# CortexFoundation/tachikoma

Hardware: AMD Instinct MI355X
Metric: ResNet-50 int8 op-traces/sec at 1/2/4/8 GPU; bit-exact vs CPU (higher is better)
Workload: dtype int8; 1 GPU; resnet50 int8 224x224, 64 samples per GPU (BASELINE config 4 shard), full per-op trace to pinned host memory; model=resnet50, global_batch=64, samples_per_gpu=64, parallelism=batch-shard x1, sink=memory

## Files before the change

### include/tachikoma.h

```cpp
#ifndef TACHIKOMA_H_
#define TACHIKOMA_H_

#include <stdint.h>
#include <stddef.h>

#ifdef __cplusplus
extern "C" {
#endif

#pragma GCC visibility push(default)

#define TK_ABI_VERSION 1

typedef enum {
  TK_OK = 0,
  TK_ERR_INVALID_ARG = -1,
  TK_ERR_UNSUPPORTED = -2,
  TK_ERR_SHAPE = -3,
  TK_ERR_DTYPE = -4,
  TK_ERR_HIP = -5,
  TK_ERR_IO = -6,
  TK_ERR_FORMAT = -7,
} tk_status;

// ... 78 lines not shown
  int32_t has_clip;
  int64_t clip_min, clip_max;
  int32_t has_add;
  int32_t block_is_rhs;
  const tk_tensor* residual;
  tk_qnn_add_attrs add;
  int32_t algo;
} tk_block_attrs;

int tk_conv2d_block_algos(const tk_tensor* data, const tk_tensor* weight, const tk_block_attrs* attrs,
                          int32_t* algos, int max_algos);
int tk_conv2d_block_algo_info(const tk_tensor* data, const tk_tensor* weight, const tk_block_attrs* attrs, int algo,
                              char* buf, int len);

typedef struct {
  tk_qnn_add_attrs add;
  int32_t has_clip;
  int64_t clip_min, clip_max;
} tk_add_block_attrs;

typedef struct {
  int32_t pool_size[2];
  int32_t strides[2];
  int32_t padding[4];
  int32_t dilation[2];
  int32_t count_include_pad;
} tk_pool2d_attrs;


int64_t tk_conv2d_packed_weight_bytes(const tk_tensor* weight, int groups);
int tk_conv2d_pack_weight(const tk_tensor* weight, int groups, void* packed, int32_t* weight_sums,
                          void* stream);
int64_t tk_conv2d_shadow_bytes(const tk_tensor* data);
int tk_conv2d_make_shadow(const tk_tensor* data, void* shadow, void* stream);
int tk_conv2d_make_shadow_batch(const tk_tensor* const* data, void* const* shadow, int n, void* stream);
int64_t tk_conv2d_scratch_bytes(const tk_tensor* data, const tk_tensor* weight, const tk_conv2d_attrs* attrs,
                                int block);
int tk_qnn_conv2d_prepared(const tk_tensor* data, const void* shadow, const tk_tensor* weight,
                           const void* packed, const int32_t* weight_sums, tk_tensor* out,
                           const tk_conv2d_attrs* attrs, void* scratch, void* stream);
int64_t tk_qnn_conv2d_workspace_bytes(const tk_tensor* data, const tk_tensor* weight,
                                      const tk_conv2d_attrs* attrs);
int tk_qnn_conv2d(const tk_tensor* data, const tk_tensor* weight, tk_tensor* out,
                  const tk_conv2d_attrs* attrs, void* workspace, void* stream);

int tk_qnn_conv2d_block(const tk_tensor* data, const void* shadow, const tk_tensor* weight, const void* packed,
                        const int32_t* weight_sums, const tk_tensor* bias, tk_tensor* const* outs, int n_outs,
                        const tk_block_attrs* attrs, void* scratch, void* shadow_out, void* stream);

int64_t tk_qnn_dense_workspace_bytes(const tk_tensor* data, const tk_tensor* weight);
int tk_qnn_dense(const tk_tensor* data, const tk_tensor* weight, tk_tensor* out,
                 const tk_dense_attrs* attrs, void* workspace, void* stream);
int tk_qnn_dense_block(const tk_tensor* data, const tk_tensor* weight, const tk_tensor* bias, tk_tensor* const* outs,
                       int n_outs, const tk_block_attrs* attrs, void* workspace, void* stream);

int tk_requantize(const tk_tensor* data, tk_tensor* out, const tk_requantize_attrs* attrs, void* stream);
int tk_qnn_add(const tk_tensor* lhs, const tk_tensor* rhs, tk_tensor* out, const tk_qnn_add_attrs* attrs,
               void* stream);
int tk_qnn_add_block(const tk_tensor* lhs, const tk_tensor* rhs, tk_tensor* const* outs, int n_outs,
                     const tk_add_block_attrs* attrs, void* shadow_out, void* stream);

int tk_bias_add(const tk_tensor* data, const tk_tensor* bias, tk_tensor* out, int axis, void* stream);
int tk_clip(const tk_tensor* data, tk_tensor* out, int64_t a_min, int64_t a_max, void* stream);
int tk_cast(const tk_tensor* data, tk_tensor* out, void* stream);
int tk_max_pool2d(const tk_tensor* data, tk_tensor* out, const tk_pool2d_attrs* attrs, void* stream);
int tk_max_pool2d_shadow(const tk_tensor* data, const void* data_shadow, tk_tensor* out,
                         const tk_pool2d_attrs* attrs, void* out_shadow, void* stream);
int tk_avg_pool2d(const tk_tensor* data, tk_tensor* out, const tk_pool2d_attrs* attrs, void* stream);
int tk_global_avg_pool2d(const tk_tensor* data, tk_tensor* out, void* stream);
int tk_copy(const tk_tensor* data, tk_tensor* out, void* stream);
typedef struct {
  int64_t before[6], after[6];
  int64_t value_i;
  double value_f;
} tk_pad_attrs;
int tk_pad(const tk_tensor* data, tk_tensor* out, const tk_pad_attrs* attrs, void* stream);

typedef struct {
  int32_t axis;
  int32_t n_scales;
  float clip_lo, clip_hi, act_scl, sum_scl, dst_zp;
  const float* bias;
  const float* o_scl;
} tk_postops_attrs;
int tk_tachikoma_postops(const tk_tensor* acc, const tk_tensor* sum_src, tk_tensor* out,
                         const tk_postops_attrs* attrs, void* stream);

enum {
  TK_EW_ADD = 0,
  TK_EW_MULTIPLY = 1,
  TK_EW_LEFT_SHIFT = 2,
  TK_EW_RIGHT_SHIFT = 3,
  TK_EW_ROUND = 4,
  TK_EW_CLIP = 5,
  TK_EW_RELU = 6,
  TK_EW_FIXED_POINT_MULTIPLY = 7,
};
typedef struct {
  int32_t op;
  int32_t rhs_kind;
  double scalar_f;
  int64_t scalar_i;
  double lo, hi;
  int32_t multiplier, shift;
} tk_ewise_attrs;
int tk_ewise(const tk_tensor* x, const tk_tensor* rhs, tk_tensor* out, const tk_ewise_attrs* attrs, void* stream);
int tk_conv2d_f32(const tk_tensor* data, const tk_tensor* weight, tk_tensor* out, const tk_conv2d_attrs* attrs,
                  void* stream);
int tk_dense_f32(const tk_tensor* data, const tk_tensor* weight, tk_tensor* out, void* stream);
int tk_find_scale_by_kl(const int32_t* hist, const float* edges, int num_bins, int num_quantized_bins,
                        float* threshold);


typedef struct {
  int32_t axis;
  float scale;
  const float* scales;
  int32_t zero_point;
  const int32_t* zero_points;
} tk_qparams_attrs;
int tk_qnn_quantize(const tk_tensor* data, tk_tensor* out, const tk_qparams_attrs* attrs, void* stream);
int tk_qnn_dequantize(const tk_tensor* data, tk_tensor* out, const tk_qparams_attrs* attrs, void* stream);

enum { TK_QB_ADD = 0, TK_QB_SUBTRACT = 1, TK_QB_MUL = 2 };
typedef struct {
  int32_t op;
  tk_requantize_attrs lhs, rhs;
  int32_t lhs_upcast, rhs_upcast;
  tk_requantize_attrs out;
  int32_t output_zero_point;
} tk_qnn_binary_attrs;
int tk_qnn_binary(const tk_tensor* lhs, const tk_tensor* rhs, tk_tensor* out, const tk_qnn_binary_attrs* attrs,
                  void* stream);

#define TK_CONCAT_MAX 8
typedef struct {
  int32_t axis;
  int32_t n;
  int32_t requant[TK_CONCAT_MAX];
  tk_requantize_attrs rq[TK_CONCAT_MAX];
} tk_concat_attrs;
int tk_qnn_concatenate(const tk_tensor* const* inputs, int n, tk_tensor* out, const tk_concat_attrs* attrs,
                       void* stream);

typedef struct {
  int32_t ndim;
  int32_t perm[6];
} tk_transpose_attrs;
int tk_transpose(const tk_tensor* data, tk_tensor* out, const tk_transpose_attrs* attrs, void* stream);

typedef struct {
  tk_requantize_attrs rq;
  int32_t upcast;
  int32_t input_zero_point;
  int32_t output_zero_point;
  int32_t alpha_multiplier, alpha_shift;
  int32_t zp_multiplier, zp_shift;
} tk_leaky_relu_attrs;
int tk_qnn_leaky_relu(const tk_tensor* data, tk_tensor* out, const tk_leaky_relu_attrs* attrs, void* stream);

int tk_qnn_lookup(const tk_tensor* data, tk_tensor* out, const void* table, void* stream);

int64_t tk_qnn_batch_matmul_workspace_bytes(const tk_tensor* x, const tk_tensor* y);
int tk_qnn_batch_matmul(const tk_tensor* x, const tk_tensor* y, tk_tensor* out, const tk_dense_attrs* attrs,
                        void* workspace, void* stream);

typedef struct {
  int32_t strides[2];
  int32_t padding[4];
  int32_t output_padding[2];
  int32_t groups;
  int32_t input_zero_point;
  int32_t kernel_zero_point;
  const int32_t* kernel_zero_points;
} tk_conv2d_transpose_attrs;
int tk_qnn_conv2d_transpose(const tk_tensor* data, const tk_tensor* weight, tk_tensor* out,
                            const tk_conv2d_transpose_attrs* attrs, void* stream);

typedef struct {
  int32_t axis;
  int32_t n_scales, n_zero_points;
  const int32_t* dtype_code;
  const float* scales;
  const int32_t* zero_points;
} tk_simq_attrs;
int tk_qnn_simulated_quantize(const tk_tensor* data, tk_tensor* out, const tk_simq_attrs* attrs, void* stream);
int tk_qnn_simulated_dequantize(const tk_tensor* data, tk_tensor* out, const tk_simq_attrs* attrs, void* stream);

typedef struct {
  int32_t bits;
  int32_t rounding;
  int32_t axis;
  int32_t scaled;
  double multiplier;
  const double* multipliers;
  int32_t input_zero_point;
  const int32_t* input_zero_points;
  int32_t output_zero_point;
} tk_requantize_fp_attrs;
int tk_requantize_fp(const tk_tensor* data, tk_tensor* out, const tk_requantize_fp_attrs* attrs, void* stream);

typedef struct {
  int32_t op;
  tk_requantize_fp_attrs lhs, rhs;
  int32_t lhs_upcast, rhs_upcast;
  tk_requantize_fp_attrs out;
  int32_t output_zero_point;
} tk_qnn_binary_fp_attrs;
int tk_qnn_binary_fp(const tk_tensor* lhs, const tk_tensor* rhs, tk_tensor* out, const tk_qnn_binary_fp_attrs* attrs,
                     void* stream);


enum {
  TK_NODE_CONV2D = 1,
  TK_NODE_DENSE = 2,
  TK_NODE_REQUANTIZE = 3,
  TK_NODE_BIAS_ADD = 4,
  TK_NODE_CLIP = 5,
  TK_NODE_CAST = 6,
  TK_NODE_QNN_ADD = 7,
  TK_NODE_MAX_POOL2D = 8,
  TK_NODE_AVG_POOL2D = 9,
  TK_NODE_GLOBAL_AVG_POOL2D = 10,
  TK_NODE_COPY = 11,
  TK_NODE_SHADOW = 12,
  TK_NODE_CONV_BLOCK = 13,
  TK_NODE_DENSE_BLOCK = 14,
  TK_NODE_ADD_BLOCK = 15,
  TK_NODE_POSTOPS = 16,
  TK_NODE_EWISE = 17,
  TK_NODE_CONV2D_F32 = 18,
  TK_NODE_DENSE_F32 = 19,
  TK_NODE_PAD = 20,
  TK_NODE_QUANTIZE = 21,
  TK_NODE_DEQUANTIZE = 22,
  TK_NODE_QNN_BINARY = 23,
  TK_NODE_CONCAT = 24,
  TK_NODE_TRANSPOSE = 25,
  TK_NODE_LEAKY_RELU = 26,
  TK_NODE_LOOKUP = 27,
  TK_NODE_BATCH_MATMUL = 28,
  TK_NODE_CONV2D_TRANSPOSE = 29,
  TK_NODE_SIM_QUANTIZE = 30,
  TK_NODE_SIM_DEQUANTIZE = 31,
  TK_NODE_REQUANTIZE_FP = 32,
  TK_NODE_QNN_BINARY_FP = 33,
};

#define TK_MAX_NODE_INPUTS 8
#define TK_MAX_NODE_OUTPUTS 6

typedef struct {
  int32_t kind;
  int32_t n_inputs;
  const tk_tensor* inputs[TK_MAX_NODE_INPUTS];
  int32_t n_outputs;
  tk_tensor* outputs[TK_MAX_NODE_OUTPUTS];
  void* ext[5];
  union {
    tk_conv2d_attrs conv2d;
    tk_dense_attrs dense;
    tk_requantize_attrs requantize;
    tk_qnn_add_attrs qnn_add;
    tk_pool2d_attrs pool2d;
    tk_block_attrs block;
    tk_add_block_attrs add_block;
    tk_postops_attrs postops;
    tk_ewise_attrs ewise;
    tk_pad_attrs pad;
    tk_qparams_attrs qparams;
    tk_qnn_binary_attrs qnn_binary;
    tk_concat_attrs concat;
    tk_transpose_attrs transpose;
    tk_leaky_relu_attrs leaky_relu;
    tk_conv2d_transpose_attrs conv2d_transpose;
    tk_simq_attrs simq;
    tk_requantize_fp_attrs requantize_fp;
    tk_qnn_binary_fp_attrs qnn_binary_fp;
    struct { int64_t a_min, a_max; } clip;
    struct { int32_t axis; } bias_add;
  } attrs;
} tk_node;

typedef struct tk_module tk_module;

int tk_module_create(const tk_node* nodes, int n_nodes, tk_module** out);
int tk_module_destroy(tk_module* mod);
int tk_module_num_nodes(const tk_module* mod);
int tk_module_run(tk_module* mod, void* stream, void* capture_stream, void* const* host_dst);
int tk_module_run_graph(tk_module* mod, void* stream, void* capture_stream, void* const* host_dst);
int tk_module_set_graph_copies(tk_module* mod, int copy_kernels);
int tk_module_set_trace_chunks(tk_module* mod, int chunks);
int tk_module_set_copy_trace(tk_module* mod, int enable);
int tk_module_copy_trace(tk_module* mod, double* out, int max_chunks);
int tk_module_set_trace_wire(tk_module* mod, int enable);
int tk_module_wire_stats(tk_module* mod, double* out, int max_chunks);

typedef struct {
  int64_t offset;
  int64_t n_elems;
  int32_t diff;
  int32_t kind;
} tk_wire_record;
int64_t tk_wire_bound(const tk_wire_record* recs, int n_recs);
int64_t tk_wire_encode_host(const tk_wire_record* recs, int n_recs, const void* image, int64_t image_bytes,
                            void* wire, int64_t wire_cap);
int tk_wire_decode(const tk_wire_record* recs, int n_recs, const void* wire, int64_t wire_bytes, void* image,
                   int64_t image_bytes, int threads);
int tk_wire_encode_device(const tk_wire_record* recs, int n_recs, const void* const* src, void* wire,
                          int64_t wire_cap, void* stream);
int64_t tk_wire_pack_device(const tk_wire_record* recs, int n_recs, const void* const* src, void* wire,
                            int64_t wire_cap, void* stream);
int tk_wire_pack_tile(void);
int tk_wire_threads(void);

typedef struct {
  uint64_t mismatches;
  uint64_t first;
} tk_wire_mismatch;
enum { TK_WIRE_UNPACK_STORE = 0, TK_WIRE_UNPACK_COMPARE = 1 };
int tk_wire_check(const tk_wire_record* recs, int n_recs, const void* wire, int64_t wire_bytes);
int tk_wire_unpack_device(const tk_wire_record* recs, int n_recs, const void* wire, int64_t wire_bytes,
                          void* const* dst, int mode, tk_wire_mismatch* report, void* stream);
int tk_compare_device(const void* expected, const void* got, int64_t n_elems, int elem_bytes,
                      tk_wire_mismatch* report, void* stream);
int tk_compare_device_batch(const void* const* expected, const void* const* got, const int64_t* n_elems,
                            const int32_t* elem_bytes, int n, tk_wire_mismatch* report, void* stream);

typedef struct {
  int32_t node;
  int32_t output;
} tk_chain_op;
int tk_chain_check_tile(void);
int tk_module_chain_ops(tk_module* mod, tk_chain_op* ops, int capacity);
int tk_module_check_chains(tk_module* mod, tk_wire_mismatch* report, int capacity, void* stream);
int tk_check_chain(int kind, const tk_tensor* const* records, int n_records, const tk_tensor* bias, const void* attrs,
                   tk_wire_mismatch* report, int capacity, void* stream);

typedef struct {
  uint64_t count;
  int64_t sum;
  int32_t min, max;
  uint64_t bits[33];
  uint64_t values[256];
} tk_record_stats;
typedef struct tk_stats_plan tk_stats_plan;
int tk_record_stats_tile(void);
int tk_record_stats_span(void);
int tk_record_stats_size(void);
int tk_stats_plan_create(const void* const* src, const int64_t* n_elems, const int32_t* kinds, int n,
                         tk_stats_plan** out);
int tk_stats_plan_destroy(tk_stats_plan* plan);
int tk_record_stats_reset(tk_record_stats* stats_dev, int n, void* stream);
int tk_stats_plan_run(tk_stats_plan* plan, tk_record_stats* stats_dev, void* stream);
int tk_record_stats_batch(const void* const* src, const int64_t* n_elems, const int32_t* kinds, int n,
                          tk_record_stats* out_host, void* stream);

int tk_module_wait_capture(tk_module* mod, void* stream);
int tk_module_run_range(tk_module* mod, int begin, int end, void* stream);
int tk_module_run_order(tk_module* mod, const int32_t* order, int n, void* stream);
int tk_module_run_profiled(tk_module* mod, void* stream, float* node_ms);
int tk_module_set_profiling(tk_module* mod, int enable);
int tk_module_node_times(tk_module* mod, float* node_ms);
int tk_module_tune(tk_module* mod, void* stream, int max_candidates, int reps, int32_t* algo_out, float* us_out);
int tk_module_set_node_algo(tk_module* mod, int node, int algo);


typedef struct {
  const char* name;
  int32_t ndim;
  const int64_t* shape;
  tk_dtype dtype;
} tk_array_meta;

int64_t tk_ndlist_layout(const tk_array_meta* arrays, int n, int64_t* data_offsets);
int tk_ndlist_write_headers(const tk_array_meta* arrays, int n, void* blob, int64_t blob_size);
int tk_ndlist_parse(const void* blob, int64_t blob_size, int cap, tk_array_meta* arrays,
                    int64_t* data_offsets, int64_t* shapes_storage, int shapes_cap, int* n_out);

#define TK_TRACE_MAGIC 0x0045434152544B54ULL
#define TK_TRACE_VERSION 1
#define TK_TRACE_VERSION_PACKED 2
#define TK_TRACE_ALIGN 4096
typedef struct {
  uint64_t magic, version, json_len, params_off, params_size, records_off, records_size;
} tk_trace_header;

int64_t tk_trace_layout(const char* json, const tk_array_meta* params, int n_params,
                        const tk_array_meta* records, int n_records, int64_t* param_offsets,
                        int64_t* record_offsets);
int tk_trace_write_headers(const char* json, const tk_array_meta* params, int n_params,
                           const tk_array_meta* records, int n_records, void* image, int64_t image_size);
int tk_write_file(const char* path, const void* image, int64_t size);

int tk_digest_bytes(const void* data, int64_t nbytes, uint64_t* out_device, void* stream);

#pragma GCC visibility pop

#ifdef __cplusplus
}
#endif
#endif
```

### tachikoma_amd/_lib.py

```python
from __future__ import annotations

import ctypes
import os
from typing import Optional

import numpy as np

HERE = os.path.dirname(os.path.abspath(__file__))
LIB_PATH = os.path.join(HERE, "libtachikoma.so")


class TachikomaError(RuntimeError):
    """Raised when a C-ABI call fails (carries ``tk_last_error()``)."""



class tk_device(ctypes.Structure):
    _fields_ = [("device_type", ctypes.c_int32), ("device_id", ctypes.c_int32)]


class tk_dtype(ctypes.Structure):
    _fields_ = [("code", ctypes.c_uint8), ("bits", ctypes.c_uint8), ("lanes", ctypes.c_uint16)]


class tk_tensor(ctypes.Structure):
    _fields_ = [
        ("data", ctypes.c_void_p),
        ("device", tk_device),
        ("ndim", ctypes.c_int32),
        ("dtype", tk_dtype),
        ("shape", ctypes.POINTER(ctypes.c_int64)),
        ("strides", ctypes.POINTER(ctypes.c_int64)),
        ("byte_offset", ctypes.c_uint64),
    ]


class tk_requantize_attrs(ctypes.Structure):
    _fields_ = [
        ("mode", ctypes.c_int32),
        ("axis", ctypes.c_int32),
        ("multiplier", ctypes.c_int32),
        ("shift", ctypes.c_int32),
        ("multipliers", ctypes.c_void_p),
        ("shifts", ctypes.c_void_p),
        ("input_zero_point", ctypes.c_int32),
        ("input_zero_points", ctypes.c_void_p),
        ("output_zero_point", ctypes.c_int32),
    ]


class tk_conv2d_attrs(ctypes.Structure):
    _fields_ = [
        ("strides", ctypes.c_int32 * 2),
        ("padding", ctypes.c_int32 * 4),
        ("dilation", ctypes.c_int32 * 2),
        ("groups", ctypes.c_int32),
        ("input_zero_point", ctypes.c_int32),
        ("kernel_zero_point", ctypes.c_int32),
        ("kernel_zero_points", ctypes.c_void_p),
    ]


class tk_dense_attrs(ctypes.Structure):
    _fields_ = [
        ("input_zero_point", ctypes.c_int32),
        ("kernel_zero_point", ctypes.c_int32),
        ("kernel_zero_points", ctypes.c_void_p),
    ]


class tk_qnn_add_attrs(ctypes.Structure):
    _fields_ = [
        ("lhs", tk_requantize_attrs),
        ("rhs", tk_requantize_attrs),
        ("output_zero_point", ctypes.c_int32),
        ("lhs_upcast", ctypes.c_int32),
        ("rhs_upcast", ctypes.c_int32),
    ]


class tk_block_attrs(ctypes.Structure):
    _fields_ = [
        ("conv", tk_conv2d_attrs),
        ("dense", tk_dense_attrs),
        ("requantize", tk_requantize_attrs),
        ("has_clip", ctypes.c_int32),
        ("clip_min", ctypes.c_int64),
        ("clip_max", ctypes.c_int64),
        ("has_add", ctypes.c_int32),
        ("block_is_rhs", ctypes.c_int32),
        ("residual", ctypes.POINTER(tk_tensor)),
        ("add", tk_qnn_add_attrs),
        ("algo", ctypes.c_int32),
    ]


class tk_add_block_attrs(ctypes.Structure):
    _fields_ = [
        ("add", tk_qnn_add_attrs),
        ("has_clip", ctypes.c_int32),
        ("clip_min", ctypes.c_int64),
        ("clip_max", ctypes.c_int64),
    ]


class tk_postops_attrs(ctypes.Structure):
    _fields_ = [
        ("axis", ctypes.c_int32),
        ("n_scales", ctypes.c_int32),
        ("clip_lo", ctypes.c_float),
        ("clip_hi", ctypes.c_float),
        ("act_scl", ctypes.c_float),
        ("sum_scl", ctypes.c_float),
        ("dst_zp", ctypes.c_float),
        ("bias", ctypes.c_void_p),
        ("o_scl", ctypes.c_void_p),
    ]


class tk_ewise_attrs(ctypes.Structure):
    _fields_ = [
        ("op", ctypes.c_int32),
        ("rhs_kind", ctypes.c_int32),
        ("scalar_f", ctypes.c_double),
        ("scalar_i", ctypes.c_int64),
        ("lo", ctypes.c_double),
        ("hi", ctypes.c_double),
        ("multiplier", ctypes.c_int32),
        ("shift", ctypes.c_int32),
    ]


TK_EW = {"add": 0, "multiply": 1, "left_shift": 2, "right_shift": 3, "round": 4, "clip": 5, "relu": 6,
         "fixed_point_multiply": 7}


class tk_pad_attrs(ctypes.Structure):
    _fields_ = [
        ("before", ctypes.c_int64 * 6),
        ("after", ctypes.c_int64 * 6),
        ("value_i", ctypes.c_int64),
        ("value_f", ctypes.c_double),
    ]


class tk_pool2d_attrs(ctypes.Structure):
    _fields_ = [
        ("pool_size", ctypes.c_int32 * 2),
        ("strides", ctypes.c_int32 * 2),
        ("padding", ctypes.c_int32 * 4),
        ("dilation", ctypes.c_int32 * 2),
        ("count_include_pad", ctypes.c_int32),
    ]


class tk_qparams_attrs(ctypes.Structure):
    _fields_ = [
        ("axis", ctypes.c_int32),
        ("scale", ctypes.c_float),
        ("scales", ctypes.c_void_p),
        ("zero_point", ctypes.c_int32),
        ("zero_points", ctypes.c_void_p),
    ]


class tk_qnn_binary_attrs(ctypes.Structure):
    _fields_ = [
        ("op", ctypes.c_int32),
        ("lhs", tk_requantize_attrs),
        ("rhs", tk_requantize_attrs),
        ("lhs_upcast", ctypes.c_int32),
        ("rhs_upcast", ctypes.c_int32),
        ("out", tk_requantize_attrs),
        ("output_zero_point", ctypes.c_int32),
    ]


TK_QB = {"qnn.add": 0, "qnn.subtract": 1, "qnn.mul": 2}
CONCAT_MAX = 8


class tk_concat_attrs(ctypes.Structure):
    _fields_ = [
        ("axis", ctypes.c_int32),
        ("n", ctypes.c_int32),
        ("requant", ctypes.c_int32 * CONCAT_MAX),
        ("rq", tk_requantize_attrs * CONCAT_MAX),
    ]


class tk_transpose_attrs(ctypes.Structure):
    _fields_ = [("ndim", ctypes.c_int32), ("perm", ctypes.c_int32 * 6)]


class tk_leaky_relu_attrs(ctypes.Structure):
    _fields_ = [
        ("rq", tk_requantize_attrs),
        ("upcast", ctypes.c_int32),
        ("input_zero_point", ctypes.c_int32),
        ("output_zero_point", ctypes.c_int32),
        ("alpha_multiplier", ctypes.c_int32),
        ("alpha_shift", ctypes.c_int32),
        ("zp_multiplier", ctypes.c_int32),
        ("zp_shift", ctypes.c_int32),
    ]


class tk_conv2d_transpose_attrs(ctypes.Structure):
    _fields_ = [
        ("strides", ctypes.c_int32 * 2),
        ("padding", ctypes.c_int32 * 4),
        ("output_padding", ctypes.c_int32 * 2),
        ("groups", ctypes.c_int32),
        ("input_zero_point", ctypes.c_int32),
        ("kernel_zero_point", ctypes.c_int32),
        ("kernel_zero_points", ctypes.c_void_p),
    ]


class tk_simq_attrs(ctypes.Structure):
    _fields_ = [
        ("axis", ctypes.c_int32),
        ("n_scales", ctypes.c_int32),
        ("n_zero_points", ctypes.c_int32),
        ("dtype_code", ctypes.c_void_p),
        ("scales", ctypes.c_void_p),
        ("zero_points", ctypes.c_void_p),
    ]


class tk_requantize_fp_attrs(ctypes.Structure):
    _fields_ = [
        ("bits", ctypes.c_int32),
        ("rounding", ctypes.c_int32),
        ("axis", ctypes.c_int32),
        ("scaled", ctypes.c_int32),
        ("multiplier", ctypes.c_double),
        ("multipliers", ctypes.c_void_p),
        ("input_zero_point", ctypes.c_int32),
        ("input_zero_points", ctypes.c_void_p),
        ("output_zero_point", ctypes.c_int32),
    ]


class tk_qnn_binary_fp_attrs(ctypes.Structure):
    _fields_ = [
        ("op", ctypes.c_int32),
        ("lhs", tk_requantize_fp_attrs),
        ("rhs", tk_requantize_fp_attrs),
        ("lhs_upcast", ctypes.c_int32),
        ("rhs_upcast", ctypes.c_int32),
        ("out", tk_requantize_fp_attrs),
        ("output_zero_point", ctypes.c_int32),
    ]


class _clip(ctypes.Structure):
    _fields_ = [("a_min", ctypes.c_int64), ("a_max", ctypes.c_int64)]


class _bias_add(ctypes.Structure):
    _fields_ = [("axis", ctypes.c_int32)]


class tk_node_attrs(ctypes.Union):
    _fields_ = [
        ("conv2d", tk_conv2d_attrs),
        ("dense", tk_dense_attrs),
        ("requantize", tk_requantize_attrs),
        ("qnn_add", tk_qnn_add_attrs),
        ("pool2d", tk_pool2d_attrs),
        ("block", tk_block_attrs),
        ("add_block", tk_add_block_attrs),
        ("postops", tk_postops_attrs),
        ("ewise", tk_ewise_attrs),
        ("pad", tk_pad_attrs),
        ("qparams", tk_qparams_attrs),
        ("qnn_binary", tk_qnn_binary_attrs),
        ("concat", tk_concat_attrs),
        ("transpose", tk_transpose_attrs),
        ("leaky_relu", tk_leaky_relu_attrs),
        ("conv2d_transpose", tk_conv2d_transpose_attrs),
        ("simq", tk_simq_attrs),
        ("requantize_fp", tk_requantize_fp_attrs),
        ("qnn_binary_fp", tk_qnn_binary_fp_attrs),
        ("clip", _clip),
        ("bias_add", _bias_add),
    ]


class tk_node(ctypes.Structure):
    _fields_ = [
        ("kind", ctypes.c_int32),
        ("n_inputs", ctypes.c_int32),
        ("inputs", ctypes.POINTER(tk_tensor) * 8),
        ("n_outputs", ctypes.c_int32),
        ("outputs", ctypes.POINTER(tk_tensor) * 6),
        ("ext", ctypes.c_void_p * 5),
        ("attrs", tk_node_attrs),
    ]


class tk_wire_record(ctypes.Structure):
    _fields_ = [
        ("offset", ctypes.c_int64),
        ("n_elems", ctypes.c_int64),
        ("diff", ctypes.c_int32),
        ("kind", ctypes.c_int32),
    ]


class tk_wire_mismatch(ctypes.Structure):
    _fields_ = [
        ("mismatches", ctypes.c_uint64),
        ("first", ctypes.c_uint64),
    ]


class tk_chain_op(ctypes.Structure):
    _fields_ = [
        ("node", ctypes.c_int32),
        ("output", ctypes.c_int32),
    ]


class tk_record_stats(ctypes.Structure):
    _fields_ = [
        ("count", ctypes.c_uint64),
        ("sum", ctypes.c_int64),
        ("min", ctypes.c_int32),
        ("max", ctypes.c_int32),
        ("bits", ctypes.c_uint64 * 33),
        ("values", ctypes.c_uint64 * 256),
    ]


TK_WIRE_UNPACK_STORE, TK_WIRE_UNPACK_COMPARE = 0, 1
NO_MISMATCH = 0xFFFFFFFFFFFFFFFF


class tk_array_meta(ctypes.Structure):
    _fields_ = [
        ("name", ctypes.c_char_p),
        ("ndim", ctypes.c_int32),
        ("shape", ctypes.POINTER(ctypes.c_int64)),
        ("dtype", tk_dtype),
    ]


TK_DL_INT, TK_DL_UINT, TK_DL_FLOAT = 0, 1, 2
TK_DEV_CPU, TK_DEV_ROCM = 1, 10
TK_ROUND_UPWARD, TK_ROUND_TONEAREST = 0, 1
(TK_RQ_IDENTITY, TK_RQ_TENSOR_POW2, TK_RQ_TENSOR_UPWARD, TK_RQ_TENSOR_TONEAREST, TK_RQ_AXIS_UPWARD,
 TK_RQ_AXIS_TONEAREST) = range(6)
NODE_KINDS = {
    "qnn.conv2d": 1, "qnn.dense": 2, "qnn.requantize": 3, "nn.bias_add": 4, "clip": 5, "cast": 6,
    "qnn.add": 7, "nn.max_pool2d": 8, "nn.avg_pool2d": 9, "nn.global_avg_pool2d": 10, "copy": 11, "shadow": 12,
    "conv_block": 13, "dense_block": 14, "add_block": 15, "postops": 16,
    "ewise": 17, "conv2d_f32": 18, "dense_f32": 19, "nn.pad": 20,
    "qnn.quantize": 21, "qnn.dequantize": 22, "qnn_binary": 23, "qnn.concatenate": 24, "transpose": 25,
    "qnn.leaky_relu": 26, "lookup": 27, "qnn.batch_matmul": 28, "qnn.conv2d_transpose": 29,
    "qnn.simulated_quantize": 30, "qnn.simulated_dequantize": 31, "requantize_fp": 32, "qnn_binary_fp": 33,
}
MAX_NODE_INPUTS = 8
MAX_NODE_OUTPUTS = 6

_VP, _I32, _I64, _F32, _F64 = ctypes.c_void_p, ctypes.c_int32, ctypes.c_int64, ctypes.c_float, ctypes.c_double
_PT = ctypes.POINTER(tk_tensor)
SIGNATURES = {
    "tk_last_error": (ctypes.c_char_p, []),
    "tk_abi_version": (ctypes.c_int, []),
    "tk_build_arch": (ctypes.c_char_p, []),
    "tk_build_info": (ctypes.c_char_p, []),
    "tk_fixed_point_multiplier_shift": (ctypes.c_int, [_F64, ctypes.POINTER(_I32), ctypes.POINTER(_I32)]),
    "tk_requantize_prepare": (ctypes.c_int, [ctypes.POINTER(_F32), ctypes.c_int, _F32, ctypes.c_int,
                                             ctypes.POINTER(_I32), ctypes.POINTER(_I32), ctypes.POINTER(ctypes.c_int)]),
    "tk_conv2d_packed_weight_bytes": (_I64, [_PT, ctypes.c_int]),
    "tk_conv2d_pack_weight": (ctypes.c_int, [_PT, ctypes.c_int, _VP, _VP, _VP]),
    "tk_conv2d_shadow_bytes": (_I64, [_PT]),
    "tk_conv2d_scratch_bytes": (_I64, [_PT, _PT, ctypes.POINTER(tk_conv2d_attrs), ctypes.c_int]),
    "tk_conv2d_make_shadow": (ctypes.c_int, [_PT, _VP, _VP]),
    "tk_conv2d_make_shadow_batch": (ctypes.c_int, [ctypes.POINTER(_PT), ctypes.POINTER(_VP), ctypes.c_int, _VP]),
    "tk_qnn_conv2d_prepared": (ctypes.c_int, [_PT, _VP, _PT, _VP, _VP, _PT, ctypes.POINTER(tk_conv2d_attrs), _VP,
                                              _VP]),
    "tk_qnn_conv2d_workspace_bytes": (_I64, [_PT, _PT, ctypes.POINTER(tk_conv2d_attrs)]),
    "tk_qnn_conv2d": (ctypes.c_int, [_PT, _PT, _PT, ctypes.POINTER(tk_conv2d_attrs), _VP, _VP]),
    "tk_qnn_dense_workspace_bytes": (_I64, [_PT, _PT]),
    "tk_qnn_dense": (ctypes.c_int, [_PT, _PT, _PT, ctypes.POINTER(tk_dense_attrs), _VP, _VP]),
    "tk_qnn_conv2d_block": (ctypes.c_int, [_PT, _VP, _PT, _VP, _VP, _PT, ctypes.POINTER(_PT), ctypes.c_int,
                                           ctypes.POINTER(tk_block_attrs), _VP, _VP, _VP]),
    "tk_qnn_dense_block": (ctypes.c_int, [_PT, _PT, _PT, ctypes.POINTER(_PT), ctypes.c_int,
                                          ctypes.POINTER(tk_block_attrs), _VP, _VP]),
    "tk_requantize": (ctypes.c_int, [_PT, _PT, ctypes.POINTER(tk_requantize_attrs), _VP]),
    "tk_qnn_add": (ctypes.c_int, [_PT, _PT, _PT, ctypes.POINTER(tk_qnn_add_attrs), _VP]),
    "tk_qnn_add_block": (ctypes.c_int, [_PT, _PT, ctypes.POINTER(_PT), ctypes.c_int,
                                        ctypes.POINTER(tk_add_block_attrs), _VP, _VP]),
    "tk_bias_add": (ctypes.c_int, [_PT, _PT, _PT, ctypes.c_int, _VP]),
    "tk_clip": (ctypes.c_int, [_PT, _PT, _I64, _I64, _VP]),
    "tk_cast": (ctypes.c_int, [_PT, _PT, _VP]),
    "tk_max_pool2d": (ctypes.c_int, [_PT, _PT, ctypes.POINTER(tk_pool2d_attrs), _VP]),
    "tk_max_pool2d_shadow": (ctypes.c_int, [_PT, _VP, _PT, ctypes.POINTER(tk_pool2d_attrs), _VP, _VP]),
    "tk_avg_pool2d": (ctypes.c_int, [_PT, _PT, ctypes.POINTER(tk_pool2d_attrs), _VP]),
    "tk_global_avg_pool2d": (ctypes.c_int, [_PT, _PT, _VP]),
    "tk_copy": (ctypes.c_int, [_PT, _PT, _VP]),
    "tk_pad": (ctypes.c_int, [_PT, _PT, ctypes.POINTER(tk_pad_attrs), _VP]),
    "tk_tachikoma_postops": (ctypes.c_int, [_PT, _PT, _PT, ctypes.POINTER(tk_postops_attrs), _VP]),
    "tk_ewise": (ctypes.c_int, [_PT, _PT, _PT, ctypes.POINTER(tk_ewise_attrs), _VP]),
    "tk_conv2d_f32": (ctypes.c_int, [_PT, _PT, _PT, ctypes.POINTER(tk_conv2d_attrs), _VP]),
    "tk_dense_f32": (ctypes.c_int, [_PT, _PT, _PT, _VP]),
    "tk_qnn_quantize": (ctypes.c_int, [_PT, _PT, ctypes.POINTER(tk_qparams_attrs), _VP]),
    "tk_qnn_dequantize": (ctypes.c_int, [_PT, _PT, ctypes.POINTER(tk_qparams_attrs), _VP]),
    "tk_qnn_binary": (ctypes.c_int, [_PT, _PT, _PT, ctypes.POINTER(tk_qnn_binary_attrs), _VP]),
    "tk_qnn_concatenate": (ctypes.c_int, [ctypes.POINTER(_PT), ctypes.c_int, _PT, ctypes.POINTER(tk_concat_attrs),
                                          _VP]),
    "tk_transpose": (ctypes.c_int, [_PT, _PT, ctypes.POINTER(tk_transpose_attrs), _VP]),
    "tk_qnn_leaky_relu": (ctypes.c_int, [_PT, _PT, ctypes.POINTER(tk_leaky_relu_attrs), _VP]),
    "tk_qnn_lookup": (ctypes.c_int, [_PT, _PT, _VP, _VP]),
    "tk_qnn_batch_matmul_workspace_bytes": (_I64, [_PT, _PT]),
    "tk_qnn_batch_matmul": (ctypes.c_int, [_PT, _PT, _PT, ctypes.POINTER(tk_dense_attrs), _VP, _VP]),
    "tk_qnn_conv2d_transpose": (ctypes.c_int, [_PT, _PT, _PT, ctypes.POINTER(tk_conv2d_transpose_attrs), _VP]),
    "tk_qnn_simulated_quantize": (ctypes.c_int, [_PT, _PT, ctypes.POINTER(tk_simq_attrs), _VP]),
    "tk_qnn_simulated_dequantize": (ctypes.c_int, [_PT, _PT, ctypes.POINTER(tk_simq_attrs), _VP]),
    "tk_requantize_fp": (ctypes.c_int, [_PT, _PT, ctypes.POINTER(tk_requantize_fp_attrs), _VP]),
    "tk_qnn_binary_fp": (ctypes.c_int, [_PT, _PT, _PT, ctypes.POINTER(tk_qnn_binary_fp_attrs), _VP]),
    "tk_find_scale_by_kl": (ctypes.c_int, [ctypes.POINTER(_I32), ctypes.POINTER(_F32), ctypes.c_int, ctypes.c_int,
                                           ctypes.POINTER(_F32)]),
    "tk_module_create": (ctypes.c_int, [ctypes.POINTER(tk_node), ctypes.c_int, ctypes.POINTER(_VP)]),
    "tk_module_destroy": (ctypes.c_int, [_VP]),
    "tk_module_num_nodes": (ctypes.c_int, [_VP]),
    "tk_module_run": (ctypes.c_int, [_VP, _VP, _VP, ctypes.POINTER(_VP)]),
    "tk_module_wait_capture": (ctypes.c_int, [_VP, _VP]),
    "tk_module_run_range": (ctypes.c_int, [_VP, ctypes.c_int, ctypes.c_int, _VP]),
    "tk_module_run_order": (ctypes.c_int, [_VP, ctypes.POINTER(ctypes.c_int32), ctypes.c_int, _VP]),
    "tk_module_run_profiled": (ctypes.c_int, [_VP, _VP, ctypes.POINTER(_F32)]),
    "tk_module_set_profiling": (ctypes.c_int, [_VP, ctypes.c_int]),
    "tk_module_node_times": (ctypes.c_int, [_VP, ctypes.POINTER(_F32)]),
    "tk_module_run_graph": (ctypes.c_int, [_VP, _VP, _VP, ctypes.POINTER(_VP)]),
    "tk_module_set_graph_copies": (ctypes.c_int, [_VP, ctypes.c_int]),
    "tk_module_set_trace_chunks": (ctypes.c_int, [_VP, ctypes.c_int]),
    "tk_module_set_copy_trace": (ctypes.c_int, [_VP, ctypes.c_int]),
    "tk_module_copy_trace": (ctypes.c_int, [_VP, ctypes.POINTER(_F64), ctypes.c_int]),
    "tk_module_set_trace_wire": (ctypes.c_int, [_VP, ctypes.c_int]),
    "tk_module_wire_stats": (ctypes.c_int, [_VP, ctypes.POINTER(_F64), ctypes.c_int]),
    "tk_wire_bound": (_I64, [ctypes.POINTER(tk_wire_record), ctypes.c_int]),
    "tk_wire_encode_host": (_I64, [ctypes.POINTER(tk_wire_record), ctypes.c_int, _VP, _I64, _VP, _I64]),
    "tk_wire_decode": (ctypes.c_int, [ctypes.POINTER(tk_wire_record), ctypes.c_int, _VP, _I64, _VP, _I64, ctypes.c_int]),
    "tk_wire_encode_device": (ctypes.c_int, [ctypes.POINTER(tk_wire_record), ctypes.c_int, ctypes.POINTER(_VP), _VP,
                                             _I64, _VP]),
    "tk_wire_pack_device": (_I64, [ctypes.POINTER(tk_wire_record), ctypes.c_int, ctypes.POINTER(_VP), _VP, _I64, _VP]),
    "tk_wire_pack_tile": (ctypes.c_int, []),
    "tk_wire_threads": (ctypes.c_int, []),
    "tk_wire_check": (ctypes.c_int, [ctypes.POINTER(tk_wire_record), ctypes.c_int, _VP, _I64]),
    "tk_wire_unpack_device": (ctypes.c_int, [ctypes.POINTER(tk_wire_record), ctypes.c_int, _VP, _I64,
                                             ctypes.POINTER(_VP), ctypes.c_int, ctypes.POINTER(tk_wire_mismatch), _VP]),
    "tk_compare_device": (ctypes.c_int, [_VP, _VP, _I64, ctypes.c_int, ctypes.POINTER(tk_wire_mismatch), _VP]),
    "tk_compare_device_batch": (ctypes.c_int, [ctypes.POINTER(_VP), ctypes.POINTER(_VP), ctypes.POINTER(_I64),
                                               ctypes.POINTER(ctypes.c_int32), ctypes.c_int,
                                               ctypes.POINTER(tk_wire_mismatch), _VP]),
    "tk_chain_check_tile": (ctypes.c_int, []),
    "tk_module_chain_ops": (ctypes.c_int, [_VP, ctypes.POINTER(tk_chain_op), ctypes.c_int]),
    "tk_module_check_chains": (ctypes.c_int, [_VP, ctypes.POINTER(tk_wire_mismatch), ctypes.c_int, _VP]),
    "tk_check_chain": (ctypes.c_int, [ctypes.c_int, ctypes.POINTER(ctypes.POINTER(tk_tensor)), ctypes.c_int,
                                      ctypes.POINTER(tk_tensor), _VP, ctypes.POINTER(tk_wire_mismatch), ctypes.c_int,
                                      _VP]),
    "tk_record_stats_tile": (ctypes.c_int, []),
    "tk_record_stats_span": (ctypes.c_int, []),
    "tk_record_stats_size": (ctypes.c_int, []),
    "tk_stats_plan_create": (ctypes.c_int, [ctypes.POINTER(_VP), ctypes.POINTER(_I64), ctypes.POINTER(ctypes.c_int32),
                                            ctypes.c_int, ctypes.POINTER(_VP)]),
    "tk_stats_plan_destroy": (ctypes.c_int, [_VP]),
    "tk_record_stats_reset": (ctypes.c_int, [_VP, ctypes.c_int, _VP]),
    "tk_stats_plan_run": (ctypes.c_int, [_VP, _VP, _VP]),
    "tk_record_stats_batch": (ctypes.c_int, [ctypes.POINTER(_VP), ctypes.POINTER(_I64), ctypes.POINTER(ctypes.c_int32),
                                             ctypes.c_int, _VP, _VP]),
    "tk_module_tune": (ctypes.c_int, [_VP, _VP, ctypes.c_int, ctypes.c_int, ctypes.POINTER(ctypes.c_int32),
                                      ctypes.POINTER(_F32)]),
    "tk_module_set_node_algo": (ctypes.c_int, [_VP, ctypes.c_int, ctypes.c_int]),
    "tk_conv2d_block_algos": (ctypes.c_int, [_PT, _PT, ctypes.POINTER(tk_block_attrs), ctypes.POINTER(ctypes.c_int32),
                                             ctypes.c_int]),
    "tk_conv2d_block_algo_info": (ctypes.c_int, [_PT, _PT, ctypes.POINTER(tk_block_attrs), ctypes.c_int,
                                                  ctypes.c_char_p, ctypes.c_int]),
    "tk_ndlist_layout": (_I64, [ctypes.POINTER(tk_array_meta), ctypes.c_int, ctypes.POINTER(_I64)]),
    "tk_ndlist_write_headers": (ctypes.c_int, [ctypes.POINTER(tk_array_meta), ctypes.c_int, _VP, _I64]),
    "tk_ndlist_parse": (ctypes.c_int, [_VP, _I64, ctypes.c_int, ctypes.POINTER(tk_array_meta), ctypes.POINTER(_I64),
                                       ctypes.POINTER(_I64), ctypes.c_int, ctypes.POINTER(ctypes.c_int)]),
    "tk_trace_layout": (_I64, [ctypes.c_char_p, ctypes.POINTER(tk_array_meta), ctypes.c_int,
                               ctypes.POINTER(tk_array_meta), ctypes.c_int, ctypes.POINTER(_I64),
                               ctypes.POINTER(_I64)]),
    "tk_trace_write_headers": (ctypes.c_int, [ctypes.c_char_p, ctypes.POINTER(tk_array_meta), ctypes.c_int,
                                              ctypes.POINTER(tk_array_meta), ctypes.c_int, _VP, _I64]),
    "tk_write_file": (ctypes.c_int, [ctypes.c_char_p, _VP, _I64]),
    "tk_digest_bytes": (ctypes.c_int, [_VP, _I64, _VP, _VP]),
}

_LIB: Optional[ctypes.CDLL] = None


def load(path: str = LIB_PATH) -> ctypes.CDLL:
    global _LIB
    if _LIB is not None:
        return _LIB
    override = os.environ.get("TK_LIB_PATH")
    path = override or path
    if not os.path.exists(path):
        raise TachikomaError(
            f"{path} not found: build it with `python tachikoma_amd/build.py` "
            "(the engine has no CPU fallback)")
    lib = ctypes.CDLL(path, mode=ctypes.RTLD_GLOBAL)
    for name, (res, args) in SIGNATURES.items():
        fn = getattr(lib, name)
        fn.restype = res
        fn.argtypes = args
    from .build import source_hash
    built = lib.tk_build_info().decode()
    try:
        want = source_hash()
    except OSError:
        want = None
    any_src = bool(override) and os.environ.get("TK_LIB_ANY_SOURCES") == "1"
    if want is not None and built.split("+")[0] != want and not any_src:
        raise TachikomaError(
            f"{path} was built from other sources (library {built}, tree {want}): rebuild it with "
            "`python tachikoma_amd/build.py`")
    if override:
        import sys
        sys.stderr.write(f"[tachikoma] TK_LIB_PATH: using {path} ({built})\n")
    _LIB = lib
    return lib


def build_info() -> str:
    return load().tk_build_info().decode()


def check(rc: int, what: str = "") -> None:
    if rc != 0:
        msg = load().tk_last_error().decode(errors="replace")
        raise TachikomaError(f"{what or 'tachikoma call'} failed ({rc}): {msg}")


_DT = {
    "int8": (TK_DL_INT, 8), "uint8": (TK_DL_UINT, 8), "int16": (TK_DL_INT, 16), "uint16": (TK_DL_UINT, 16),
    "int32": (TK_DL_INT, 32), "uint32": (TK_DL_UINT, 32), "int64": (TK_DL_INT, 64), "uint64": (TK_DL_UINT, 64),
    "float32": (TK_DL_FLOAT, 32), "float64": (TK_DL_FLOAT, 64),
}


def dtype_struct(dtype: str) -> tk_dtype:
    code, bits = _DT[str(np.dtype(dtype))]
    return tk_dtype(code, bits, 1)


def dtype_name(d: tk_dtype) -> str:
    for k, (c, b) in _DT.items():
        if c == d.code and b == d.bits:
            return k
    raise TachikomaError(f"unknown dtype code={d.code} bits={d.bits}")


class TensorRef:

    def __init__(self, data_ptr: int, shape, dtype: str, device_type: int = TK_DEV_ROCM, device_id: int = 0):
        self.shape_arr = (ctypes.c_int64 * max(1, len(shape)))(*[int(s) for s in shape])
        self.struct = tk_tensor()
        self.struct.data = ctypes.c_void_p(int(data_ptr))
        self.struct.device = tk_device(device_type, device_id)
        self.struct.ndim = len(shape)
        self.struct.dtype = dtype_struct(dtype)
        self.struct.shape = ctypes.cast(self.shape_arr, ctypes.POINTER(ctypes.c_int64))
        self.struct.strides = None
        self.struct.byte_offset = 0
        self.shape = tuple(int(s) for s in shape)
        self.dtype = str(np.dtype(dtype))

    @property
    def ptr(self):
        return ctypes.pointer(self.struct)

    @staticmethod
    def from_torch(t) -> "TensorRef":
        import torch
        assert t.is_contiguous(), "tensors must be compact"
        dev = TK_DEV_ROCM if t.is_cuda else TK_DEV_CPU
        return TensorRef(t.data_ptr(), tuple(t.shape), str(t.dtype).replace("torch.", ""), dev,
                         t.device.index or 0 if t.is_cuda else 0)


def stream_handle(stream=None) -> int:
    import torch
    s = stream if stream is not None else torch.cuda.current_stream()
    return int(s.cuda_stream)
```

### tachikoma_amd/csrc/tk_runtime.cc

```cpp
#include <algorithm>
#include <atomic>
#include <cstdlib>
#include <cstring>
#include <map>
#include <memory>
#include <mutex>
#include <string>
#include <vector>

#include "tk_chain.h"
#include "tk_common.h"
#include "tk_wire.h"

namespace tk {
int requantize_impl(const tk_tensor* x, tk_tensor* y, const tk_requantize_attrs* a, hipStream_t s);
int bias_add_impl(const tk_tensor* x, const tk_tensor* b, tk_tensor* y, int axis, hipStream_t s);
int clip_impl(const tk_tensor* x, tk_tensor* y, int64_t lo, int64_t hi, hipStream_t s);
int cast_impl(const tk_tensor* x, tk_tensor* y, hipStream_t s);
int qnn_add_impl(const tk_tensor* a, const tk_tensor* b, tk_tensor* y, const tk_qnn_add_attrs* at, hipStream_t s);
int add_block_impl(const tk_tensor* a, const tk_tensor* b, tk_tensor* const* outs, int n_outs,
                   const tk_add_block_attrs* at, void* shadow, hipStream_t s);
int max_pool_impl(const tk_tensor* x, tk_tensor* y, const tk_pool2d_attrs* a, hipStream_t s);
int max_pool_shadow_impl(const tk_tensor* x, const void* x_shadow, tk_tensor* y, const tk_pool2d_attrs* a,
                         void* y_shadow, hipStream_t s);
int avg_pool_impl(const tk_tensor* x, tk_tensor* y, const tk_pool2d_attrs* a, hipStream_t s);
int global_avg_pool_impl(const tk_tensor* x, tk_tensor* y, hipStream_t s);
int copy_impl(const tk_tensor* x, tk_tensor* y, hipStream_t s);
int pad_impl(const tk_tensor* x, tk_tensor* y, const tk_pad_attrs* a, hipStream_t s);
int postops_impl(const tk_tensor* acc, const tk_tensor* sum_src, tk_tensor* y, const tk_postops_attrs* a,
                 hipStream_t s);
int host_copy_impl(const void* const* src, void* const* dst, const int64_t* bytes, int n, hipStream_t s);
int pack_records_impl(const void* table, int nrec, int64_t blocks, void* mirror, hipStream_t s);
int wire_encode_impl(const WireSegDev* segs, int64_t n_seg, uint32_t* cursor, void* wire, int64_t wire_bytes,
                     hipStream_t s);
int ewise_impl(const tk_tensor* x, const tk_tensor* r, tk_tensor* y, const tk_ewise_attrs* a, hipStream_t s);
int conv2d_f32_impl(const tk_tensor* x, const tk_tensor* w, tk_tensor* y, const tk_conv2d_attrs* a, hipStream_t s);
int dense_f32_impl(const tk_tensor* x, const tk_tensor* w, tk_tensor* y, hipStream_t s);
int64_t conv_packed_weight_bytes(const tk_tensor* weight, int groups);
int conv_pack_weight(const tk_tensor* weight, int groups, void* packed, int32_t* sums, hipStream_t s);
int64_t conv_shadow_bytes(const tk_tensor* data);
int64_t conv_scratch_bytes(const tk_tensor* data, const tk_tensor* weight, const tk_conv2d_attrs* a, int block);
int make_shadow_impl(const tk_tensor* data, void* shadow, hipStream_t s);
int conv2d_prepared_impl(const tk_tensor* data, const void* shadow, const tk_tensor* weight, const void* packed,
                         const int32_t* sums, tk_tensor* out, const tk_conv2d_attrs* a, void* scratch, hipStream_t s);
int64_t conv2d_workspace_bytes(const tk_tensor* data, const tk_tensor* weight, const tk_conv2d_attrs* a);
int conv2d_impl(const tk_tensor* data, const tk_tensor* weight, tk_tensor* out, const tk_conv2d_attrs* a,
                void* workspace, hipStream_t s);
int64_t dense_workspace_bytes(const tk_tensor* data, const tk_tensor* weight);
int dense_impl(const tk_tensor* data, const tk_tensor* weight, tk_tensor* out, const tk_dense_attrs* a,
               void* workspace, hipStream_t s);
int conv2d_block_impl(const tk_tensor* data, const void* shadow, const tk_tensor* weight, const void* packed,
                      const int32_t* sums, const tk_tensor* bias, tk_tensor* const* outs, int n_outs,
                      const tk_block_attrs* attrs, void* scratch, void* shadow_out, hipStream_t s);
int dense_block_impl(const tk_tensor* data, const tk_tensor* weight, const tk_tensor* bias, tk_tensor* const* outs,
                     int n_outs, const tk_block_attrs* attrs, void* workspace, hipStream_t s);
int qnn_quantize_impl(const tk_tensor* x, tk_tensor* y, const tk_qparams_attrs* a, hipStream_t s);
int qnn_dequantize_impl(const tk_tensor* x, tk_tensor* y, const tk_qparams_attrs* a, hipStream_t s);
int qnn_binary_impl(const tk_tensor* a, const tk_tensor* b, tk_tensor* y, const tk_qnn_binary_attrs* at,
                    hipStream_t s);
int qnn_concatenate_impl(const tk_tensor* const* xs, int n_in, tk_tensor* y, const tk_concat_attrs* a,
                         hipStream_t s);
int transpose_impl(const tk_tensor* x, tk_tensor* y, const tk_transpose_attrs* a, hipStream_t s);
int conv2d_block_algos_impl(const tk_tensor* data, const tk_tensor* weight, const tk_block_attrs* attrs,
                            int32_t* algos, int max_algos);
int qnn_leaky_relu_impl(const tk_tensor* x, tk_tensor* y, const tk_leaky_relu_attrs* a, hipStream_t s);
int qnn_simulated_impl(bool quant, const tk_tensor* x, tk_tensor* y, const tk_simq_attrs* a, hipStream_t s);
int requantize_fp_impl(const tk_tensor* x, tk_tensor* y, const tk_requantize_fp_attrs* a, hipStream_t s);
int qnn_binary_fp_impl(const tk_tensor* a, const tk_tensor* b, tk_tensor* y, const tk_qnn_binary_fp_attrs* at,
                       hipStream_t s);
int qnn_lookup_impl(const tk_tensor* x, tk_tensor* y, const void* table, hipStream_t s);
int qnn_conv2d_transpose_impl(const tk_tensor* x, const tk_tensor* w, tk_tensor* y, const tk_conv2d_transpose_attrs* a,
                              hipStream_t s);

static bool bmm_check(const tk_tensor* x, const tk_tensor* y) {
  return x && y && compact(x) && compact(y) && x->ndim == 3 && y->ndim == 3 && x->shape[2] == y->shape[2] &&
         (x->shape[0] == y->shape[0] || x->shape[0] == 1 || y->shape[0] == 1);
}
struct View2 {
  int64_t shape[2];
  tk_tensor t;
  View2(const tk_tensor* src, int64_t b) {
    t = *src;
    shape[0] = src->shape[1];
    shape[1] = src->shape[2];
    t.ndim = 2;
    t.shape = shape;
    t.strides = nullptr;
    t.byte_offset = src->byte_offset + (uint64_t)(b * shape[0] * shape[1] * elem_bytes(src));
  }
};
int64_t batch_matmul_workspace_bytes(const tk_tensor* x, const tk_tensor* y) {
  if (!bmm_check(x, y)) {
    set_error("qnn.batch_matmul: x [B, M, K], y [B', N, K] with B == B' or one of them 1");
    return TK_ERR_INVALID_ARG;
  }
  View2 xv(x, 0), yv(y, 0);
  return dense_workspace_bytes(&xv.t, &yv.t);
}
int batch_matmul_impl(const tk_tensor* x, const tk_tensor* y, tk_tensor* out, const tk_dense_attrs* a, void* ws,
                      hipStream_t s) {
  TK_CHECK_ARG(bmm_check(x, y) && out && a, "qnn.batch_matmul: x [B, M, K], y [B', N, K] (B == B' or one is 1)");
  const int64_t B = std::max(x->shape[0], y->shape[0]);
  TK_CHECK_ARG(compact(out) && out->ndim == 3 && out->shape[0] == B && out->shape[1] == x->shape[1] &&
               out->shape[2] == y->shape[1] && is_int(out, 32), "qnn.batch_matmul: int32 [B, M, N] output");
  for (int64_t b = 0; b < B; ++b) {
    View2 xv(x, x->shape[0] == 1 ? 0 : b), yv(y, y->shape[0] == 1 ? 0 : b), ov(out, b);
    const int rc = dense_impl(&xv.t, &yv.t, &ov.t, a, ws, s);
    if (rc) return rc;
  }
  return TK_OK;
}
int conv2d_block_algo_info_impl(const tk_tensor* data, const tk_tensor* weight, const tk_block_attrs* attrs, int algo,
                                char* buf, int len);

constexpr int TK_OK_RUN = 1;

struct OwnedTensor {
  tk_tensor t{};
  std::vector<int64_t> shape;
  void assign(const tk_tensor* src) {
    t = *src;
    shape.assign(src->shape, src->shape + src->ndim);
    t.shape = shape.data();
    t.strides = nullptr;
  }
  OwnedTensor() = default;
  OwnedTensor(const OwnedTensor& o) { assign(&o.t); }
  OwnedTensor& operator=(const OwnedTensor& o) {
    assign(&o.t);
    return *this;
  }
};

struct Node {
  tk_node desc{};
  OwnedTensor in[TK_MAX_NODE_INPUTS];
  OwnedTensor out[TK_MAX_NODE_OUTPUTS];
  tk_tensor* outp[TK_MAX_NODE_OUTPUTS] = {};
};

static int run_node(Node& n, hipStream_t s) {
  const tk_node& d = n.desc;
  const tk_tensor* i0 = &n.in[0].t;
  const tk_tensor* i1 = &n.in[1].t;
  const tk_tensor* i2 = &n.in[2].t;
  tk_tensor* o = &n.out[0].t;
  switch (d.kind) {
    case TK_NODE_CONV_BLOCK: {
      tk_block_attrs at = d.attrs.block;
      if (at.has_add) at.residual = &n.in[3].t;
      return conv2d_block_impl(i0, d.ext[0], i1, d.ext[1], (const int32_t*)d.ext[2], i2, n.outp, d.n_outputs, &at,
                               d.ext[3], d.ext[4], s);
    }
    case TK_NODE_DENSE_BLOCK:
      return dense_block_impl(i0, i1, i2, n.outp, d.n_outputs, &d.attrs.block, d.ext[0], s);
    case TK_NODE_CONV2D:
      return conv2d_prepared_impl(i0, d.ext[0], i1, d.ext[1], (const int32_t*)d.ext[2], o, &d.attrs.conv2d, d.ext[3], s);
    case TK_NODE_DENSE:
      return dense_impl(i0, i1, o, &d.attrs.dense, d.ext[0], s);
    case TK_NODE_REQUANTIZE:
      return requantize_impl(i0, o, &d.attrs.requantize, s);
    case TK_NODE_BIAS_ADD:
      return bias_add_impl(i0, i1, o, d.attrs.bias_add.axis, s);
    case TK_NODE_CLIP:
      return clip_impl(i0, o, d.attrs.clip.a_min, d.attrs.clip.a_max, s);
    case TK_NODE_CAST:
      return cast_impl(i0, o, s);
    case TK_NODE_QNN_ADD:
      return qnn_add_impl(i0, i1, o, &d.attrs.qnn_add, s);
    case TK_NODE_ADD_BLOCK:
      return add_block_impl(i0, i1, n.outp, d.n_outputs, &d.attrs.add_block, d.ext[4], s);
    case TK_NODE_MAX_POOL2D:
      if (d.ext[0]) return max_pool_shadow_impl(i0, d.ext[0], o, &d.attrs.pool2d, d.ext[4], s);
      if (d.ext[4]) {
        int rc = max_pool_impl(i0, o, &d.attrs.pool2d, s);
        return rc ? rc : make_shadow_impl(o, d.ext[4], s);
      }
      return max_pool_impl(i0, o, &d.attrs.pool2d, s);
    case TK_NODE_AVG_POOL2D:
      return avg_pool_impl(i0, o, &d.attrs.pool2d, s);
    case TK_NODE_GLOBAL_AVG_POOL2D:
      return global_avg_pool_impl(i0, o, s);
    case TK_NODE_COPY:
      return copy_impl(i0, o, s);
    case TK_NODE_SHADOW:
      return make_shadow_impl(i0, d.ext[0], s);
    case TK_NODE_POSTOPS:
      return postops_impl(i0, d.n_inputs > 1 ? i1 : nullptr, o, &d.attrs.postops, s);
    case TK_NODE_EWISE:
      return ewise_impl(i0, d.n_inputs > 1 ? i1 : nullptr, o, &d.attrs.ewise, s);
    case TK_NODE_CONV2D_F32:
      return conv2d_f32_impl(i0, i1, o, &d.attrs.conv2d, s);
    case TK_NODE_DENSE_F32:
      return dense_f32_impl(i0, i1, o, s);
    case TK_NODE_PAD:
      return pad_impl(i0, o, &d.attrs.pad, s);
    case TK_NODE_QUANTIZE:
      return qnn_quantize_impl(i0, o, &d.attrs.qparams, s);
    case TK_NODE_DEQUANTIZE:
      return qnn_dequantize_impl(i0, o, &d.attrs.qparams, s);
    case TK_NODE_QNN_BINARY:
      return qnn_binary_impl(i0, i1, o, &d.attrs.qnn_binary, s);
    case TK_NODE_CONCAT: {
      const tk_tensor* xs[TK_MAX_NODE_INPUTS];
      for (int k = 0; k < d.n_inputs; ++k) xs[k] = &n.in[k].t;
      return qnn_concatenate_impl(xs, d.n_inputs, o, &d.attrs.concat, s);
    }
    case TK_NODE_TRANSPOSE:
      return transpose_impl(i0, o, &d.attrs.transpose, s);
    case TK_NODE_LEAKY_RELU:
      return qnn_leaky_relu_impl(i0, o, &d.attrs.leaky_relu, s);
    case TK_NODE_LOOKUP:
      return qnn_lookup_impl(i0, o, d.ext[0], s);
    case TK_NODE_BATCH_MATMUL:
      return batch_matmul_impl(i0, i1, o, &d.attrs.dense, d.ext[0], s);
    case TK_NODE_CONV2D_TRANSPOSE:
      return qnn_conv2d_transpose_impl(i0, i1, o, &d.attrs.conv2d_transpose, s);
    case TK_NODE_SIM_QUANTIZE:
    case TK_NODE_SIM_DEQUANTIZE:
      return qnn_simulated_impl(d.kind == TK_NODE_SIM_QUANTIZE, i0, o, &d.attrs.simq, s);
    case TK_NODE_REQUANTIZE_FP:
      return requantize_fp_impl(i0, o, &d.attrs.requantize_fp, s);
    case TK_NODE_QNN_BINARY_FP:
      return qnn_binary_fp_impl(i0, i1, o, &d.attrs.qnn_binary_fp, s);
  }
  set_error("tk_module: unknown node kind " + std::to_string(d.kind));
  return TK_ERR_INVALID_ARG;
}

}

struct PackRecHost {
  const void* src;
  int64_t dst, bytes, first_blk;
};
struct PackPlan {
  std::vector<void*> dst;
  char* host_lo = nullptr;
  int64_t span = 0;
  void* mirror[2] = {nullptr, nullptr};
  struct Chunk {
    int after_node;
    int64_t off, len;
    int64_t table_off;
    int n_rec;
    int64_t blocks;
  };
  std::vector<Chunk> chunks;
  void* table = nullptr;
  std::vector<hipEvent_t> ev[2];
  hipEvent_t mirror_done[2] = {nullptr, nullptr};
  bool mirror_used[2] = {false, false};
  std::vector<hipGraph_t> g[2];
  std::vector<hipGraphExec_t> ge[2];
  int next = 0;
  bool wire = false;
  struct Range {
    int64_t off, len;
  };
  struct WireCall {
    tk::WireJob job;
    std::atomic<int>* failed = nullptr;
  };
  struct WireChunk {
    std::vector<Range> raw;
    int64_t seg_off = 0;
    int64_t coded_bytes = 0, bound = 0;
    std::vector<tk::WireSegHost> segs;
    std::vector<tk::WireUnit> units;
    std::unique_ptr<WireCall[]> calls;
    hipEvent_t landed = nullptr;
    int last_slot = -1;
  };
  std::vector<WireChunk> wchunks;
  void* wire_segs = nullptr;
  std::vector<void*> slots;
  uint32_t* cursors = nullptr;
  std::vector<hipEvent_t> slot_done;
  std::vector<char> slot_used;
  int slot_next = 0;
  ~PackPlan() {
    for (auto& w : wchunks)
      if (w.landed) (void)hipEventDestroy(w.landed);
    for (auto e : slot_done) (void)hipEventDestroy(e);
    for (void* p : slots) (void)hipHostFree(p);
    if (wire_segs) (void)hipFree(wire_segs);
    if (cursors) (void)hipFree(cursors);
    for (int m = 0; m < 2; ++m) {
      for (auto x : ge[m]) (void)hipGraphExecDestroy(x);
      for (auto x : g[m]) (void)hipGraphDestroy(x);
      for (auto e : ev[m]) (void)hipEventDestroy(e);
      if (mirror_done[m]) (void)hipEventDestroy(mirror_done[m]);
      if (mirror[m]) (void)hipFree(mirror[m]);
    }
    if (table) (void)hipFree(table);
  }
};

struct tk_module {
  std::vector<tk::Node> nodes;
  std::vector<hipEvent_t> done;
  std::vector<hipEvent_t> prof;
  hipEvent_t capture_done = nullptr;
  bool capture_recorded = false;
  bool capture_plain = false;
  bool profiling = false;
  bool have_times = false;
  struct Graph {
    hipGraph_t g = nullptr;
    hipGraphExec_t ge = nullptr;
    hipStream_t s = nullptr, cs = nullptr;
    std::vector<void*> dst;
  };
  std::vector<Graph> graphs;
  hipEvent_t graph_join = nullptr, graph_pre = nullptr;
  hipStream_t cap_s = nullptr, cap_cs = nullptr, cap_cx[3] = {nullptr, nullptr, nullptr};
  bool graph_copy_kernels = false;
  int graph_copy_chains = 4;
  bool graph_packed = true;
  int pack_chunks = 8;
  std::vector<std::unique_ptr<PackPlan>> packs;
  bool copy_trace = false;
  hipEvent_t ct_t0 = nullptr;
  std::vector<hipEvent_t> ct_ev;
  std::vector<int64_t> ct_bytes;
  bool trace_wire = true, wire_forced_off = false, wire_clamp = true;
  hipStream_t wire_s = nullptr, dec_s = nullptr;
  hipEvent_t wire_tail = nullptr, decode_tail = nullptr;
  bool wire_tail_used = false;
  std::atomic<int> wire_failed{0};
  PackPlan* last_wire_plan = nullptr;
  struct Chains {
    bool built = false;
    std::vector<tk_chain_op> ops;
    int n_chains = 0;
    int64_t blocks = 0;
    void* dev = nullptr;
    tk_wire_mismatch* report = nullptr;
  } chains;
  void drop_graph() {
    last_wire_plan = nullptr;
    for (Graph& x : graphs) {
      if (x.ge) (void)hipGraphExecDestroy(x.ge);
      if (x.g) (void)hipGraphDestroy(x.g);
    }
    graphs.clear();
    if (!packs.empty()) (void)hipDeviceSynchronize();
    packs.clear();
  }
  ~tk_module() {
    drop_graph();
    if (chains.dev) (void)hipFree(chains.dev);
    for (auto e : done) (void)hipEventDestroy(e);
    for (auto e : prof) (void)hipEventDestroy(e);
    if (capture_done) (void)hipEventDestroy(capture_done);
    if (graph_join) (void)hipEventDestroy(graph_join);
    if (graph_pre) (void)hipEventDestroy(graph_pre);
    if (ct_t0) (void)hipEventDestroy(ct_t0);
    for (auto e : ct_ev) (void)hipEventDestroy(e);
    if (wire_tail) (void)hipEventDestroy(wire_tail);
    if (decode_tail) (void)hipEventDestroy(decode_tail);
    if (wire_s) (void)hipStreamDestroy(wire_s);
    if (dec_s) (void)hipStreamDestroy(dec_s);
    if (cap_s) (void)hipStreamDestroy(cap_s);
    if (cap_cs) (void)hipStreamDestroy(cap_cs);
    for (hipStream_t x : cap_cx)
      if (x) (void)hipStreamDestroy(x);
  }
};

static int wait_capture(tk_module* mod, hipStream_t s) {
  if (mod->capture_recorded) TK_HIP(hipStreamWaitEvent(s, mod->capture_done, 0));
  return TK_OK;
}

extern "C" {

int64_t tk_conv2d_packed_weight_bytes(const tk_tensor* weight, int groups) {
  return tk::conv_packed_weight_bytes(weight, groups);
}
int tk_conv2d_pack_weight(const tk_tensor* weight, int groups, void* packed, int32_t* weight_sums, void* stream) {
  return tk::conv_pack_weight(weight, groups, packed, weight_sums, tk::as_stream(stream));
}
int64_t tk_conv2d_shadow_bytes(const tk_tensor* data) { return tk::conv_shadow_bytes(data); }
int64_t tk_conv2d_scratch_bytes(const tk_tensor* data, const tk_tensor* weight, const tk_conv2d_attrs* attrs,
                                int block) {
  return tk::conv_scratch_bytes(data, weight, attrs, block);
}
int tk_conv2d_make_shadow(const tk_tensor* data, void* shadow, void* stream) {
  return tk::make_shadow_impl(data, shadow, tk::as_stream(stream));
}
int tk_qnn_conv2d_prepared(const tk_tensor* data, const void* shadow, const tk_tensor* weight, const void* packed,
                           const int32_t* weight_sums, tk_tensor* out, const tk_conv2d_attrs* attrs, void* scratch,
                           void* stream) {
  return tk::conv2d_prepared_impl(data, shadow, weight, packed, weight_sums, out, attrs, scratch,
                                  tk::as_stream(stream));
}
int64_t tk_qnn_conv2d_workspace_bytes(const tk_tensor* data, const tk_tensor* weight, const tk_conv2d_attrs* attrs) {
  return tk::conv2d_workspace_bytes(data, weight, attrs);
}
int tk_qnn_conv2d(const tk_tensor* data, const tk_tensor* weight, tk_tensor* out, const tk_conv2d_attrs* attrs,
                  void* workspace, void* stream) {
  return tk::conv2d_impl(data, weight, out, attrs, workspace, tk::as_stream(stream));
}
int64_t tk_qnn_dense_workspace_bytes(const tk_tensor* data, const tk_tensor* weight) {
  return tk::dense_workspace_bytes(data, weight);
}
int tk_qnn_dense(const tk_tensor* data, const tk_tensor* weight, tk_tensor* out, const tk_dense_attrs* attrs,
                 void* workspace, void* stream) {
  return tk::dense_impl(data, weight, out, attrs, workspace, tk::as_stream(stream));
}
int tk_qnn_conv2d_block(const tk_tensor* data, const void* shadow, const tk_tensor* weight, const void* packed,
                        const int32_t* weight_sums, const tk_tensor* bias, tk_tensor* const* outs, int n_outs,
                        const tk_block_attrs* attrs, void* scratch, void* shadow_out, void* stream) {
  return tk::conv2d_block_impl(data, shadow, weight, packed, weight_sums, bias, outs, n_outs, attrs, scratch,
                               shadow_out, tk::as_stream(stream));
}
int tk_conv2d_block_algos(const tk_tensor* data, const tk_tensor* weight, const tk_block_attrs* attrs,
                          int32_t* algos, int max_algos) {
  return tk::conv2d_block_algos_impl(data, weight, attrs, algos, max_algos);
}
int tk_conv2d_block_algo_info(const tk_tensor* data, const tk_tensor* weight, const tk_block_attrs* attrs, int algo,
                              char* buf, int len) {
  return tk::conv2d_block_algo_info_impl(data, weight, attrs, algo, buf, len);
}
int tk_qnn_dense_block(const tk_tensor* data, const tk_tensor* weight, const tk_tensor* bias, tk_tensor* const* outs,
                       int n_outs, const tk_block_attrs* attrs, void* workspace, void* stream) {
  return tk::dense_block_impl(data, weight, bias, outs, n_outs, attrs, workspace, tk::as_stream(stream));
}
int tk_requantize(const tk_tensor* data, tk_tensor* out, const tk_requantize_attrs* attrs, void* stream) {
  return tk::requantize_impl(data, out, attrs, tk::as_stream(stream));
}
int tk_qnn_add_block(const tk_tensor* lhs, const tk_tensor* rhs, tk_tensor* const* outs, int n_outs,
                     const tk_add_block_attrs* attrs, void* shadow_out, void* stream) {
  return tk::add_block_impl(lhs, rhs, outs, n_outs, attrs, shadow_out, tk::as_stream(stream));
}
int tk_qnn_add(const tk_tensor* lhs, const tk_tensor* rhs, tk_tensor* out, const tk_qnn_add_attrs* attrs,
               void* stream) {
  return tk::qnn_add_impl(lhs, rhs, out, attrs, tk::as_stream(stream));
}
int tk_bias_add(const tk_tensor* data, const tk_tensor* bias, tk_tensor* out, int axis, void* stream) {
  return tk::bias_add_impl(data, bias, out, axis, tk::as_stream(stream));
}
int tk_clip(const tk_tensor* data, tk_tensor* out, int64_t a_min, int64_t a_max, void* stream) {
  return tk::clip_impl(data, out, a_min, a_max, tk::as_stream(stream));
}
int tk_cast(const tk_tensor* data, tk_tensor* out, void* stream) {
  return tk::cast_impl(data, out, tk::as_stream(stream));
}
int tk_max_pool2d(const tk_tensor* data, tk_tensor* out, const tk_pool2d_attrs* attrs, void* stream) {
  return tk::max_pool_impl(data, out, attrs, tk::as_stream(stream));
}
int tk_max_pool2d_shadow(const tk_tensor* data, const void* data_shadow, tk_tensor* out,
                         const tk_pool2d_attrs* attrs, void* out_shadow, void* stream) {
  return tk::max_pool_shadow_impl(data, data_shadow, out, attrs, out_shadow, tk::as_stream(stream));
}
int tk_avg_pool2d(const tk_tensor* data, tk_tensor* out, const tk_pool2d_attrs* attrs, void* stream) {
  return tk::avg_pool_impl(data, out, attrs, tk::as_stream(stream));
}
int tk_global_avg_pool2d(const tk_tensor* data, tk_tensor* out, void* stream) {
  return tk::global_avg_pool_impl(data, out, tk::as_stream(stream));
}
int tk_copy(const tk_tensor* data, tk_tensor* out, void* stream) {
  return tk::copy_impl(data, out, tk::as_stream(stream));
}
int tk_pad(const tk_tensor* data, tk_tensor* out, const tk_pad_attrs* attrs, void* stream) {
  return tk::pad_impl(data, out, attrs, tk::as_stream(stream));
}
int tk_tachikoma_postops(const tk_tensor* acc, const tk_tensor* sum_src, tk_tensor* out,
                         const tk_postops_attrs* attrs, void* stream) {
  return tk::postops_impl(acc, sum_src, out, attrs, tk::as_stream(stream));
}
int tk_ewise(const tk_tensor* x, const tk_tensor* rhs, tk_tensor* out, const tk_ewise_attrs* attrs, void* stream) {
  return tk::ewise_impl(x, rhs, out, attrs, tk::as_stream(stream));
}
int tk_conv2d_f32(const tk_tensor* data, const tk_tensor* weight, tk_tensor* out, const tk_conv2d_attrs* attrs,
                  void* stream) {
  return tk::conv2d_f32_impl(data, weight, out, attrs, tk::as_stream(stream));
}
int tk_dense_f32(const tk_tensor* data, const tk_tensor* weight, tk_tensor* out, void* stream) {
  return tk::dense_f32_impl(data, weight, out, tk::as_stream(stream));
}
int64_t tk_qnn_batch_matmul_workspace_bytes(const tk_tensor* x, const tk_tensor* y) {
  return tk::batch_matmul_workspace_bytes(x, y);
}
int tk_qnn_batch_matmul(const tk_tensor* x, const tk_tensor* y, tk_tensor* out, const tk_dense_attrs* attrs,
                        void* workspace, void* stream) {
  return tk::batch_matmul_impl(x, y, out, attrs, workspace, tk::as_stream(stream));
}

int tk_module_create(const tk_node* nodes, int n_nodes, tk_module** out) {
  if (!out || n_nodes < 0 || (n_nodes > 0 && !nodes)) {
    tk::set_error("tk_module_create: invalid argument");
    return TK_ERR_INVALID_ARG;
  }
  auto mod = std::make_unique<tk_module>();
  if (const char* e = std::getenv("TK_TRACE_WIRE")) mod->wire_forced_off = e[0] == '0' && e[1] == 0;
  if (const char* e = std::getenv("TK_WIRE_CLAMP")) mod->wire_clamp = !(e[0] == '0' && e[1] == 0);
  mod->nodes.resize(n_nodes);
  for (int i = 0; i < n_nodes; ++i) {
    const tk_node& src = nodes[i];
    tk::Node& dst = mod->nodes[i];
    dst.desc = src;
    if (src.n_inputs < 0 || src.n_inputs > TK_MAX_NODE_INPUTS) {
      tk::set_error("tk_module_create: node " + std::to_string(i) + " has a bad input count");
      return TK_ERR_INVALID_ARG;
    }
    if (src.kind == TK_NODE_CONV_BLOCK && src.attrs.block.has_add && src.n_inputs != 4) {
      tk::set_error("tk_module_create: node " + std::to_string(i) + ": a residual block takes the residual as input 3");
      return TK_ERR_INVALID_ARG;
    }
    for (int k = 0; k < src.n_inputs; ++k) {
      if (!src.inputs[k]) {
        tk::set_error("tk_module_create: node " + std::to_string(i) + " has a null input");
        return TK_ERR_INVALID_ARG;
      }
      dst.in[k].assign(src.inputs[k]);
    }
    if (src.n_outputs < 0 || src.n_outputs > TK_MAX_NODE_OUTPUTS || (src.kind != TK_NODE_SHADOW && src.n_outputs < 1)) {
      tk::set_error("tk_module_create: node " + std::to_string(i) + " has a bad output count");
      return TK_ERR_INVALID_ARG;
    }
    for (int k = 0; k < src.n_outputs; ++k) {
      if (!src.outputs[k]) {
        tk::set_error("tk_module_create: node " + std::to_string(i) + " has a null output");
        return TK_ERR_INVALID_ARG;
      }
      dst.out[k].assign(src.outputs[k]);
    }
    for (int k = 0; k < TK_MAX_NODE_INPUTS; ++k) dst.desc.inputs[k] = nullptr;
    for (int k = 0; k < TK_MAX_NODE_OUTPUTS; ++k) dst.desc.outputs[k] = nullptr;
  }
  for (auto& n : mod->nodes)
    for (int k = 0; k < TK_MAX_NODE_OUTPUTS; ++k) n.outp[k] = &n.out[k].t;
  mod->done.resize(n_nodes);
  for (int i = 0; i < n_nodes; ++i) {
    hipError_t e = hipEventCreateWithFlags(&mod->done[i], hipEventDisableTiming);
    if (e != hipSuccess) {
      mod->done.resize(i);
      tk::set_error(std::string("tk_module_create: hipEventCreate failed: ") + hipGetErrorString(e));
      return TK_ERR_HIP;
    }
  }
  {
    hipError_t e = hipEventCreateWithFlags(&mod->capture_done, hipEventDisableTiming);
    if (e != hipSuccess) {
      mod->capture_done = nullptr;
      tk::set_error(std::string("tk_module_create: hipEventCreate failed: ") + hipGetErrorString(e));
      return TK_ERR_HIP;
    }
  }
  *out = mod.release();
  return TK_OK;
}

int tk_module_destroy(tk_module* mod) {
  delete mod;
  return TK_OK;
}

int tk_module_num_nodes(const tk_module* mod) { return mod ? (int)mod->nodes.size() : 0; }

static int ensure_prof_events(tk_module* mod) {
  while (mod->prof.size() < mod->nodes.size() + 1) {
    hipEvent_t e;
    TK_HIP(hipEventCreate(&e));
    mod->prof.push_back(e);
  }
  return TK_OK;
}

int tk_module_set_profiling(tk_module* mod, int enable) {
  if (!mod) {
    tk::set_error("tk_module_set_profiling: null module");
    return TK_ERR_INVALID_ARG;
  }
  mod->profiling = enable != 0;
  mod->have_times = false;
  return mod->profiling ? ensure_prof_events(mod) : TK_OK;
}

int tk_module_node_times(tk_module* mod, float* node_ms) {
  if (!mod || !node_ms || !mod->have_times) {
    tk::set_error("tk_module_node_times: no profiled run recorded");
    return TK_ERR_INVALID_ARG;
  }
  size_t n = mod->nodes.size();
  TK_HIP(hipEventSynchronize(mod->prof[n]));
  for (size_t i = 0; i < n; ++i) TK_HIP(hipEventElapsedTime(&node_ms[i], mod->prof[i], mod->prof[i + 1]));
  return TK_OK;
}

static int enqueue_nodes(tk_module* mod, hipStream_t s, hipStream_t cs, void* const* host_dst, bool capture,
                         bool profiling, bool copy_kernels = false, hipStream_t const* chains = nullptr,
                         int n_chains = 1, int* n_copied = nullptr) {
  if (profiling) TK_HIP(hipEventRecord(mod->prof[0], s));
  int copied = 0;
  if (n_copied) *n_copied = 0;
  for (size_t i = 0; i < mod->nodes.size(); ++i) {
    tk::Node& n = mod->nodes[i];
    int rc = tk::run_node(n, s);
    if (rc) {
      tk::set_error("node " + std::to_string(i) + ": " + tk_last_error());
      return rc;
    }
    if (profiling) TK_HIP(hipEventRecord(mod->prof[i + 1], s));
    if (capture && n.desc.n_outputs > 0) {
      void* const* dst = host_dst + i * TK_MAX_NODE_OUTPUTS;
      bool any = false;
      for (int k = 0; k < n.desc.n_outputs; ++k) any |= dst[k] != nullptr;
      if (any) {
        if (chains) cs = chains[copied % n_chains];
        ++copied;
        if (n_copied) *n_copied = copied;
        TK_HIP(hipEventRecord(mod->done[i], s));
        TK_HIP(hipStreamWaitEvent(cs, mod->done[i], 0));
        if (copy_kernels) {
          const void* src[TK_MAX_NODE_OUTPUTS];
          int64_t nb[TK_MAX_NODE_OUTPUTS];
          for (int k = 0; k < n.desc.n_outputs; ++k) src[k] = tk::ptr(&n.out[k].t), nb[k] = tk::nbytes(&n.out[k].t);
          int rc = tk::host_copy_impl(src, dst, nb, n.desc.n_outputs, cs);
          if (rc) return rc;
        } else {
          for (int k = 0; k < n.desc.n_outputs; ++k)
            if (dst[k])
              TK_HIP(hipMemcpyAsync(dst[k], tk::ptr(&n.out[k].t), tk::nbytes(&n.out[k].t), hipMemcpyDeviceToHost, cs));
        }
      }
    }
  }
  return TK_OK;
}

int tk_module_run(tk_module* mod, void* stream, void* capture_stream, void* const* host_dst) {
  if (!mod) {
    tk::set_error("tk_module_run: null module");
    return TK_ERR_INVALID_ARG;
  }
  hipStream_t s = tk::as_stream(stream);
  hipStream_t cs = tk::as_stream(capture_stream);
  bool capture = capture_stream && host_dst;
  int rc0 = wait_capture(mod, s);
  if (rc0) return rc0;
  rc0 = enqueue_nodes(mod, s, cs, host_dst, capture, mod->profiling);
  if (rc0) return rc0;
  if (capture) {
    TK_HIP(hipEventRecord(mod->capture_done, cs));
    mod->capture_recorded = true;
    mod->capture_plain = true;
  }
  mod->have_times = mod->profiling;
  return TK_OK;
}

int tk_module_set_graph_copies(tk_module* mod, int copy_kernels) {
  if (!mod || copy_kernels < 0 || copy_kernels > 5) {
    tk::set_error("tk_module_set_graph_copies: invalid argument");
    return TK_ERR_INVALID_ARG;
  }
  const bool packed = copy_kernels == 0;
  const bool kern = copy_kernels == 1;
  const int chains = copy_kernels == 5 ? 1 : copy_kernels >= 2 ? std::min(copy_kernels, 4) : 1;
  if (mod->graph_packed != packed || mod->graph_copy_kernels != kern || mod->graph_copy_chains != chains)
    mod->drop_graph();
  mod->graph_packed = packed;
  mod->graph_copy_kernels = kern;
  mod->graph_copy_chains = chains;
  return TK_OK;
}

int tk_module_set_trace_chunks(tk_module* mod, int chunks) {
  if (!mod || chunks < 1 || chunks > 256) {
    tk::set_error("tk_module_set_trace_chunks: chunks must be 1..256");
    return TK_ERR_INVALID_ARG;
  }
  if (mod->pack_chunks != chunks) mod->drop_graph();
  mod->pack_chunks = chunks;
  return TK_OK;
}

struct PackRecord {
  char* host;
  const void* src;
  int64_t bytes;
  int node, out;
  const tk_tensor* t;
  bool wire, diff;
  bool clamp;
};

static int collect_records(const tk_module* mod, const std::vector<void*>& dst, std::vector<PackRecord>* recs) {
  for (size_t i = 0; i < mod->nodes.size(); ++i) {
    const tk::Node& n = mod->nodes[i];
    for (int k = 0; k < n.desc.n_outputs; ++k) {
      char* h = (char*)dst[i * TK_MAX_NODE_OUTPUTS + k];
      const int64_t nb = tk::nbytes(&n.out[k].t);
      if (h && nb > 0) recs->push_back({h, tk::ptr(&n.out[k].t), nb, (int)i, k, &n.out[k].t, false, false, false});
    }
  }
  std::sort(recs->begin(), recs->end(), [](const PackRecord& a, const PackRecord& b) { return a.host < b.host; });
  for (size_t r = 0; r + 1 < recs->size(); ++r)
    if ((*recs)[r].host + (*recs)[r].bytes > (*recs)[r + 1].host) {
      tk::set_error("tk_module_run_graph: overlapping record destinations");
      return TK_ERR_INVALID_ARG;
    }
  return TK_OK;
}

static const void* clip_input(const tk::Node& n, int k) {
  const tk_node& d = n.desc;
  const bool block = d.kind == TK_NODE_CONV_BLOCK || d.kind == TK_NODE_DENSE_BLOCK;
  if ((block && d.attrs.block.has_clip) || (d.kind == TK_NODE_ADD_BLOCK && d.attrs.add_block.has_clip))
    return k >= 1 && k == d.n_outputs - 1 ? tk::ptr(&n.out[k - 1].t) : nullptr;
  return d.kind == TK_NODE_CLIP && k == 0 ? tk::ptr(&n.in[0].t) : nullptr;
}

static bool decide_coding(const tk_module* mod, std::vector<PackRecord>& recs) {
  bool any = false;
  for (size_t r = 0; r < recs.size(); ++r) {
    PackRecord& c = recs[r];
    const tk_tensor* a = c.t;
    const tk_tensor* b = r ? recs[r - 1].t : nullptr;
    const bool same_shape = b && a->ndim == b->ndim && std::equal(a->shape, a->shape + a->ndim, b->shape);
    if (mod->wire_clamp && tk::is_int8ish(a) && tk::compact(a) && same_shape && tk::compact(b) &&
        a->dtype.code == b->dtype.code && b->dtype.bits == 8 && b->dtype.lanes == 1 && c.src != recs[r - 1].src &&
        clip_input(mod->nodes[c.node], c.out) == recs[r - 1].src) {
      c.wire = c.clamp = any = true;
      continue;
    }
    c.wire = tk::is_int(c.t, 32) && tk::compact(c.t) && ((uintptr_t)c.src & 3) == 0;
    any |= c.wire;
    if (!c.wire || r == 0 || !recs[r - 1].wire) continue;
    c.diff = same_shape && tk::is_int(b, 32) && c.src != recs[r - 1].src;
  }
  return any;
}

static int chunk_wire_tables(const std::vector<PackRecord>& recs, const std::vector<size_t>& coded,
                             PackPlan::WireChunk* wc, std::vector<tk::WireSegDev>& wire_segs) {
  std::vector<tk_wire_record> wrecs;
  for (size_t q = 0; q < coded.size(); ++q) {
    const PackRecord& r = recs[coded[q]];
    const bool chained = (r.diff || r.clamp) && q > 0 && coded[q - 1] == coded[q] - 1;
    const int esize = tk::elem_bytes(r.t);
    wrecs.push_back({0, r.bytes / esize, chained, esize == 4 ? tk::kWireI32 : tk::is_int(r.t, 8) ? tk::kWireI8 : tk::kWireU8});
  }
  tk::WirePlan wp;
  if (const int rc = tk::wire_plan(wrecs.data(), (int)wrecs.size(), -1, "tk_module_run_graph", &wp)) return rc;
  wc->units = std::move(wp.units);
  wc->seg_off = (int64_t)wire_segs.size();
  wc->bound = wp.bound;
  for (const tk::WireSegRef& sr : wp.segs) {
    const PackRecord& r = recs[coded[sr.rec]];
    const PackRecord* pv = r.diff || r.clamp ? &recs[coded[sr.rec] - 1] : nullptr;
    const int kind = wrecs[sr.rec].kind;
    const tk::WireSegAddr dev = tk::wire_seg_addr(sr, kind, r.src, pv ? pv->src : nullptr);
    const tk::WireSegAddr img = tk::wire_seg_addr(sr, kind, r.host, pv ? pv->host : nullptr);
    wire_segs.push_back({dev.at, dev.prev, sr.n, kind});
    wc->segs.push_back({img.at, img.prev, sr.n, kind});
  }
  for (size_t q : coded) wc->coded_bytes += recs[q].bytes;
  return TK_OK;
}

static int cut_chunks(const tk_module* mod, const std::vector<PackRecord>& recs, PackPlan* plan,
                      std::vector<PackRecHost>& table, std::vector<tk::WireSegDev>& wire_segs) {
  const int nn = (int)mod->nodes.size();
  std::vector<int64_t> complete_upto(nn);
  std::vector<int> prefix_max(recs.size());
  for (size_t q = 0; q < recs.size(); ++q) prefix_max[q] = std::max(q ? prefix_max[q - 1] : -1, recs[q].node);
  for (int i = 0, r = 0; i < nn; ++i) {
    while (r < (int)recs.size() && prefix_max[r] <= i) ++r;
    complete_upto[i] = r == (int)recs.size() ? plan->span : recs[r].host - plan->host_lo;
  }
  const int64_t target = std::max<int64_t>(1, (plan->span + mod->pack_chunks - 1) / mod->pack_chunks);
  int64_t cut = 0;
  size_t next_rec = 0;
  for (int i = 0; i < nn; ++i) {
    const int64_t upto = complete_upto[i];
    if (upto <= cut) continue;
    if (upto - cut < target && upto < plan->span) continue;
    PackPlan::Chunk c{i, cut, upto - cut, (int64_t)table.size(), 0, 0};
    int64_t blocks = 0;
    PackPlan::WireChunk wc;
    std::vector<size_t> w_rec;
    bool in_run = false;
    while (next_rec < recs.size() && recs[next_rec].host - plan->host_lo < upto) {
      const PackRecord& rc = recs[next_rec++];
      const int64_t off = rc.host - plan->host_lo;
      if (rc.wire) {
        w_rec.push_back(next_rec - 1);
        in_run = false;
        continue;
      }
      if (plan->wire) {
        if (in_run) wc.raw.back().len = off + rc.bytes - wc.raw.back().off;
        else wc.raw.push_back({off, rc.bytes});
        in_run = true;
      }
      const int64_t a0 = off & ~(int64_t)15;
      const int64_t nblk = (off + rc.bytes - a0 + 256 * 16 - 1) / (256 * 16);
      table.push_back({rc.src, off, rc.bytes, blocks});
      blocks += nblk;
      ++c.n_rec;
    }
    c.blocks = blocks;
    plan->chunks.push_back(c);
    cut = upto;
    if (!plan->wire) continue;
    if (!w_rec.empty())
      if (const int rc = chunk_wire_tables(recs, w_rec, &wc, wire_segs)) return rc;
    plan->wchunks.push_back(std::move(wc));
  }
  if (cut != plan->span || next_rec != recs.size()) {
    tk::set_error("tk_module_run_graph: pack plan does not cover every record");
    return TK_ERR_INVALID_ARG;
  }
  return TK_OK;
}

static int alloc_pack_resources(tk_module* mod, PackPlan* plan, const std::vector<PackRecHost>& table,
                                const std::vector<tk::WireSegDev>& wire_segs) {
  if (!table.empty()) {
    TK_HIP(hipMalloc(&plan->table, table.size() * sizeof(PackRecHost)));
    TK_HIP(hipMemcpy(plan->table, table.data(), table.size() * sizeof(PackRecHost), hipMemcpyHostToDevice));
  }
  if (plan->wire) {
    TK_HIP(hipMalloc(&plan->wire_segs, wire_segs.size() * sizeof(tk::WireSegDev)));
    TK_HIP(hipMemcpy(plan->wire_segs, wire_segs.data(), wire_segs.size() * sizeof(tk::WireSegDev), hipMemcpyHostToDevice));
    int64_t slot_bytes = 0;
    int coded_chunks = 0;
    for (const auto& w : plan->wchunks) slot_bytes = std::max(slot_bytes, w.bound), coded_chunks += !w.segs.empty();
    const int n_slots = std::min(3, coded_chunks);
    for (int k = 0; k < n_slots; ++k) {
      void* p = nullptr;
      TK_HIP(hipHostMalloc(&p, (size_t)slot_bytes, hipHostMallocDefault));
      plan->slots.push_back(p);
      hipEvent_t e;
      TK_HIP(hipEventCreateWithFlags(&e, hipEventDisableTiming));
      plan->slot_done.push_back(e);
    }
    plan->slot_used.assign(n_slots, 0);
    TK_HIP(hipMalloc((void**)&plan->cursors, n_slots * sizeof(uint32_t)));
    for (auto& w : plan->wchunks) {
      if (w.segs.empty()) continue;
      TK_HIP(hipEventCreateWithFlags(&w.landed, hipEventDisableTiming));
      w.calls.reset(new PackPlan::WireCall[n_slots]);
      for (int k = 0; k < n_slots; ++k) {
        tk::WireJob& j = w.calls[k].job;
        j.wire = (const char*)plan->slots[k];
        j.wire_bytes = w.bound;
        j.segs = w.segs.data(), j.n_seg = (int64_t)w.segs.size();
        j.units = w.units.data(), j.n_units = (int64_t)w.units.size();
        w.calls[k].failed = &mod->wire_failed;
      }
    }
    if (!mod->wire_s) TK_HIP(hipStreamCreateWithFlags(&mod->wire_s, hipStreamNonBlocking));
    if (!mod->dec_s) TK_HIP(hipStreamCreateWithFlags(&mod->dec_s, hipStreamNonBlocking));
    if (!mod->wire_tail) TK_HIP(hipEventCreateWithFlags(&mod->wire_tail, hipEventDisableTiming));
    if (!mod->decode_tail) TK_HIP(hipEventCreateWithFlags(&mod->decode_tail, hipEventDisableTiming));
  }
  for (int m = 0; m < 2; ++m) {
    TK_HIP(hipMalloc(&plan->mirror[m], (size_t)plan->span + 16));
    TK_HIP(hipMemcpy(plan->mirror[m], plan->host_lo, (size_t)plan->span, hipMemcpyHostToDevice));
    TK_HIP(hipEventCreateWithFlags(&plan->mirror_done[m], hipEventDisableTiming));
    plan->ev[m].resize(plan->chunks.size(), nullptr);
    for (auto& e : plan->ev[m]) TK_HIP(hipEventCreateWithFlags(&e, hipEventDisableTiming));
  }
  if (!mod->cap_s) TK_HIP(hipStreamCreateWithFlags(&mod->cap_s, hipStreamNonBlocking));
  return TK_OK;
}

static int capture_chunk_graphs(tk_module* mod, PackPlan* plan) {
  const int nn = (int)mod->nodes.size();
  const int nseg = (int)plan->chunks.size() + (plan->chunks.back().after_node < nn - 1 ? 1 : 0);
  for (int m = 0; m < 2; ++m) {
    hipStream_t qs = mod->cap_s;
    int i = 0;
    for (int seg = 0; seg < nseg; ++seg) {
      const bool has_chunk = seg < (int)plan->chunks.size();
      const int last = has_chunk ? plan->chunks[seg].after_node : nn - 1;
      TK_HIP(hipStreamBeginCapture(qs, hipStreamCaptureModeThreadLocal));
      int rc = TK_OK;
      for (; i <= last && rc == TK_OK; ++i) {
        rc = tk::run_node(mod->nodes[i], qs);
        if (rc) tk::set_error("node " + std::to_string(i) + ": " + tk_last_error());
      }
      if (rc == TK_OK && has_chunk && plan->chunks[seg].n_rec > 0) {
        const PackPlan::Chunk& ch = plan->chunks[seg];
        rc = tk::pack_records_impl((const char*)plan->table + ch.table_off * sizeof(PackRecHost), ch.n_rec, ch.blocks,
                                   plan->mirror[m], qs);
      }
      hipGraph_t g = nullptr;
      hipError_t e = hipStreamEndCapture(qs, &g);
      if (rc) {
        if (g) (void)hipGraphDestroy(g);
        return rc;
      }
      if (e != hipSuccess || !g) {
        (void)hipGetLastError();
        tk::set_error(std::string("tk_module_run_graph: stream capture failed: ") + hipGetErrorString(e));
        return TK_ERR_HIP;
      }
      plan->g[m].push_back(g);
      hipGraphExec_t ge = nullptr;
      e = hipGraphInstantiate(&ge, g, nullptr, nullptr, 0);
      if (e != hipSuccess) {
        tk::set_error(std::string("tk_module_run_graph: instantiate failed: ") + hipGetErrorString(e));
        return TK_ERR_HIP;
      }
      plan->ge[m].push_back(ge);
    }
  }
  return TK_OK;
}

static int build_pack_plan(tk_module* mod, const std::vector<void*>& dst, PackPlan** out) {
  auto plan = std::make_unique<PackPlan>();
  plan->dst = dst;
  std::vector<PackRecord> recs;
  if (const int rc = collect_records(mod, dst, &recs)) return rc;
  if (recs.empty()) {
    *out = nullptr;
    return TK_OK;
  }
  plan->wire = mod->trace_wire && !mod->wire_forced_off && decide_coding(mod, recs);
  plan->host_lo = recs.front().host;
  plan->span = recs.back().host + recs.back().bytes - plan->host_lo;
  std::vector<PackRecHost> table;
  std::vector<tk::WireSegDev> wire_segs;
  if (const int rc = cut_chunks(mod, recs, plan.get(), table, wire_segs)) return rc;
  if (const int rc = alloc_pack_resources(mod, plan.get(), table, wire_segs)) return rc;
  if (const int rc = capture_chunk_graphs(mod, plan.get())) return rc;
  *out = plan.release();
  return TK_OK;
}

static void wire_decode_call(void* p) {
  auto* call = static_cast<PackPlan::WireCall*>(p);
  if (tk::wire_decode(&call->job, 0)) call->failed->store(1);
}

static int enqueue_wire_chunk(tk_module* mod, PackPlan* plan, int m, size_t c, bool trace) {
  const PackPlan::Chunk& ch = plan->chunks[c];
  PackPlan::WireChunk& w = plan->wchunks[c];
  hipStream_t ws = mod->wire_s, ds = mod->dec_s;
  TK_HIP(hipStreamWaitEvent(ws, plan->ev[m][c], 0));
  if (trace) TK_HIP(hipEventRecord(mod->ct_ev[2 * c], ws));
  int k = -1;
  if (!w.segs.empty()) {
    k = plan->slot_next;
    plan->slot_next = (k + 1) % (int)plan->slots.size();
    if (plan->slot_used[k]) TK_HIP(hipStreamWaitEvent(ws, plan->slot_done[k], 0));
    TK_HIP(hipMemsetAsync(plan->cursors + k, 0, sizeof(uint32_t), ws));
    const int rc = tk::wire_encode_impl((const tk::WireSegDev*)plan->wire_segs + w.seg_off, (int64_t)w.segs.size(),
                                        plan->cursors + k, plan->slots[k], w.bound, ws);
    if (rc) return rc;
  }
  for (const PackPlan::Range& r : w.raw)
    TK_HIP(hipMemcpyAsync(plan->host_lo + r.off, (char*)plan->mirror[m] + r.off, (size_t)r.len, hipMemcpyDeviceToHost, ws));
  if (trace) {
    TK_HIP(hipEventRecord(mod->ct_ev[2 * c + 1], ws));
    mod->ct_bytes[c] = ch.len;
  }
  if (k >= 0) {
    TK_HIP(hipEventRecord(w.landed, ws));
    TK_HIP(hipStreamWaitEvent(ds, w.landed, 0));
    TK_HIP(hipLaunchHostFunc(ds, wire_decode_call, &w.calls[k]));
    TK_HIP(hipEventRecord(plan->slot_done[k], ds));
    plan->slot_used[k] = 1;
    w.last_slot = k;
  }
  return TK_OK;
}

static int run_packed(tk_module* mod, hipStream_t s, hipStream_t cs, void* const* host_dst) {
  const size_t nd = mod->nodes.size() * TK_MAX_NODE_OUTPUTS;
  std::vector<void*> dst(host_dst, host_dst + nd);
  PackPlan* plan = nullptr;
  for (auto& p : mod->packs)
    if (p->dst == dst) plan = p.get();
  if (!plan) {
    if (mod->packs.size() >= 2) {
      TK_HIP(hipDeviceSynchronize());
      if (mod->last_wire_plan == mod->packs.front().get()) mod->last_wire_plan = nullptr;
      mod->packs.erase(mod->packs.begin());
    }
    PackPlan* built = nullptr;
    int rc = build_pack_plan(mod, dst, &built);
    if (rc) return rc;
    if (!built) return tk::TK_OK_RUN;
    mod->packs.emplace_back(built);
    plan = built;
  }
  if (mod->capture_recorded && mod->capture_plain) TK_HIP(hipStreamWaitEvent(s, mod->capture_done, 0));
  const int m = plan->next;
  plan->next ^= 1;
  if (plan->mirror_used[m]) TK_HIP(hipStreamWaitEvent(s, plan->mirror_done[m], 0));
  if (mod->wire_failed.load()) {
    tk::set_error("tk_module_run_graph: a wire buffer of an earlier run did not decode");
    return TK_ERR_INVALID_ARG;
  }
  if (mod->wire_tail_used) TK_HIP(hipStreamWaitEvent(s, mod->wire_tail, 0));
  const bool trace = mod->copy_trace;
  if (trace) {
    if (!mod->ct_t0) TK_HIP(hipEventCreate(&mod->ct_t0));
    while (mod->ct_ev.size() < 2 * plan->chunks.size()) {
      hipEvent_t e;
      TK_HIP(hipEventCreate(&e));
      mod->ct_ev.push_back(e);
    }
    mod->ct_bytes.assign(plan->chunks.size(), 0);
    TK_HIP(hipEventRecord(mod->ct_t0, s));
  }
  for (size_t c = 0; c < plan->ge[m].size(); ++c) {
    TK_HIP(hipGraphLaunch(plan->ge[m][c], s));
    if (c >= plan->chunks.size()) break;
    const PackPlan::Chunk& ch = plan->chunks[c];
    TK_HIP(hipEventRecord(plan->ev[m][c], s));
    if (plan->wire) {
      const int rc = enqueue_wire_chunk(mod, plan, m, c, trace);
      if (rc) return rc;
      continue;
    }
    TK_HIP(hipStreamWaitEvent(cs, plan->ev[m][c], 0));
    if (trace) TK_HIP(hipEventRecord(mod->ct_ev[2 * c], cs));
    TK_HIP(hipMemcpyAsync(plan->host_lo + ch.off, (char*)plan->mirror[m] + ch.off, (size_t)ch.len,
                          hipMemcpyDeviceToHost, cs));
    if (trace) {
      TK_HIP(hipEventRecord(mod->ct_ev[2 * c + 1], cs));
      mod->ct_bytes[c] = ch.len;
    }
  }
  if (plan->wire) {
    TK_HIP(hipEventRecord(mod->wire_tail, mod->wire_s));
    TK_HIP(hipEventRecord(plan->mirror_done[m], mod->wire_s));
    TK_HIP(hipEventRecord(mod->decode_tail, mod->dec_s));
    mod->wire_tail_used = true;
    mod->last_wire_plan = plan;
    TK_HIP(hipStreamWaitEvent(cs, mod->wire_tail, 0));
    TK_HIP(hipStreamWaitEvent(cs, mod->decode_tail, 0));
  } else {
    TK_HIP(hipEventRecord(plan->mirror_done[m], cs));
    mod->last_wire_plan = nullptr;
  }
  plan->mirror_used[m] = true;
  TK_HIP(hipEventRecord(mod->capture_done, cs));
  mod->capture_recorded = true;
  mod->capture_plain = false;
  return TK_OK;
}

int tk_module_set_copy_trace(tk_module* mod, int enable) {
  if (!mod) {
    tk::set_error("tk_module_set_copy_trace: null module");
    return TK_ERR_INVALID_ARG;
  }
  mod->copy_trace = enable != 0;
  mod->ct_bytes.clear();
  return TK_OK;
}

int tk_module_set_trace_wire(tk_module* mod, int enable) {
  if (!mod || (enable != 0 && enable != 1)) {
    tk::set_error("tk_module_set_trace_wire: invalid argument");
    return TK_ERR_INVALID_ARG;
  }
  if (mod->trace_wire != (enable != 0)) mod->drop_graph();
  mod->trace_wire = enable != 0;
  return TK_OK;
}

int tk_module_wire_stats(tk_module* mod, double* out, int max_chunks) {
  if (!mod || (max_chunks > 0 && !out)) {
    tk::set_error("tk_module_wire_stats: invalid argument");
    return TK_ERR_INVALID_ARG;
  }
  PackPlan* plan = mod->last_wire_plan;
  if (!plan) return 0;
  TK_HIP(hipEventSynchronize(mod->decode_tail));
  if (mod->wire_failed.load()) {
    tk::set_error("tk_module_wire_stats: a wire buffer did not decode");
    return TK_ERR_INVALID_ARG;
  }
  const int n = (int)plan->wchunks.size();
  for (int c = 0; c < n && c < max_chunks; ++c) {
    const PackPlan::WireChunk& w = plan->wchunks[c];
    const tk::WireJob* j = w.last_slot >= 0 ? &w.calls[w.last_slot].job : nullptr;
    int64_t raw = 0;
    for (const PackPlan::Range& r : w.raw) raw += r.len;
    out[3 * c] = (double)((j ? j->used_bytes : 0) + raw);
    out[3 * c + 1] = (double)w.coded_bytes;
    out[3 * c + 2] = j ? j->ms : 0.0;
  }
  return n;
}

int tk_module_copy_trace(tk_module* mod, double* out, int max_chunks) {
  if (!mod || (max_chunks > 0 && !out)) {
    tk::set_error("tk_module_copy_trace: invalid argument");
    return TK_ERR_INVALID_ARG;
  }
  const int n = (int)mod->ct_bytes.size();
  for (int c = 0; c < n && c < max_chunks; ++c) {
    float a = 0.f, b = 0.f;
    TK_HIP(hipEventSynchronize(mod->ct_ev[2 * c + 1]));
    TK_HIP(hipEventElapsedTime(&a, mod->ct_t0, mod->ct_ev[2 * c]));
    TK_HIP(hipEventElapsedTime(&b, mod->ct_t0, mod->ct_ev[2 * c + 1]));
    out[3 * c] = (double)mod->ct_bytes[c];
    out[3 * c + 1] = a;
    out[3 * c + 2] = b;
  }
  return n;
}

int tk_module_run_graph(tk_module* mod, void* stream, void* capture_stream, void* const* host_dst) {
  if (!mod) {
    tk::set_error("tk_module_run_graph: null module");
    return TK_ERR_INVALID_ARG;
  }
  if (mod->profiling) return tk_module_run(mod, stream, capture_stream, host_dst);
  hipStream_t s = tk::as_stream(stream);
  hipStream_t cs = tk::as_stream(capture_stream);
  const bool capture = capture_stream && host_dst;
  if (capture && mod->graph_packed) {
    const int rc = run_packed(mod, s, cs, host_dst);
    if (rc != tk::TK_OK_RUN) {
      mod->have_times = false;
      return rc;
    }
  }
  const size_t nd = capture ? mod->nodes.size() * TK_MAX_NODE_OUTPUTS : 0;
  std::vector<void*> dst(nd);
  for (size_t i = 0; i < nd; ++i) dst[i] = host_dst[i];
  int gi = -1;
  for (size_t i = 0; i < mod->graphs.size(); ++i)
    if (mod->graphs[i].dst == dst && (mod->graphs[i].cs != nullptr) == capture) gi = (int)i;
  int rc0 = wait_capture(mod, s);
  if (rc0) return rc0;
  if (gi < 0) {
    if (mod->graphs.size() >= 4) {
      tk_module::Graph& old = mod->graphs.front();
      if (old.ge) (void)hipGraphExecDestroy(old.ge);
      if (old.g) (void)hipGraphDestroy(old.g);
      mod->graphs.erase(mod->graphs.begin());
    }
    if (!mod->graph_join) TK_HIP(hipEventCreateWithFlags(&mod->graph_join, hipEventDisableTiming));
    if (!mod->cap_s) TK_HIP(hipStreamCreateWithFlags(&mod->cap_s, hipStreamNonBlocking));
    if (!mod->cap_cs) TK_HIP(hipStreamCreateWithFlags(&mod->cap_cs, hipStreamNonBlocking));
    hipStream_t qs = mod->cap_s, qcs = mod->cap_cs;
    hipStream_t chains[4] = {qcs, nullptr, nullptr, nullptr};
    const int nch = capture ? mod->graph_copy_chains : 1;
    for (int c = 1; c < nch; ++c) {
      if (!mod->cap_cx[c - 1]) TK_HIP(hipStreamCreateWithFlags(&mod->cap_cx[c - 1], hipStreamNonBlocking));
      chains[c] = mod->cap_cx[c - 1];
    }
    TK_HIP(hipStreamBeginCapture(qs, hipStreamCaptureModeThreadLocal));
    int copied = 0;
    int rc = enqueue_nodes(mod, qs, qcs, host_dst, capture, false, mod->graph_copy_kernels, chains, nch, &copied);
    const int joined = std::min(copied, nch);
    for (int c = 0; c < joined && rc == TK_OK && capture; ++c) {
      if (hipEventRecord(mod->graph_join, chains[c]) != hipSuccess || hipStreamWaitEvent(qs, mod->graph_join, 0) != hipSuccess) {
        tk::set_error("tk_module_run_graph: joining the capture streams failed");
        rc = TK_ERR_HIP;
      }
    }
    hipGraph_t g = nullptr;
    hipError_t e = hipStreamEndCapture(qs, &g);
    if (rc) {
      if (g) (void)hipGraphDestroy(g);
      return rc;
    }
    if (e != hipSuccess || !g) {
      (void)hipGetLastError();
      tk::set_error(std::string("tk_module_run_graph: stream capture failed: ") + hipGetErrorString(e));
      return TK_ERR_HIP;
    }
    hipGraphExec_t ge = nullptr;
    e = hipGraphInstantiate(&ge, g, nullptr, nullptr, 0);
    if (e != hipSuccess) {
      (void)hipGraphDestroy(g);
      tk::set_error(std::string("tk_module_run_graph: instantiate failed: ") + hipGetErrorString(e));
      return TK_ERR_HIP;
    }
    tk_module::Graph x;
    x.g = g;
    x.ge = ge;
    x.s = qs;
    x.cs = capture ? qcs : nullptr;
    x.dst = std::move(dst);
    mod->graphs.push_back(std::move(x));
    gi = (int)mod->graphs.size() - 1;
  }
  if (capture) {
    if (!mod->graph_pre) TK_HIP(hipEventCreateWithFlags(&mod->graph_pre, hipEventDisableTiming));
    TK_HIP(hipEventRecord(mod->graph_pre, cs));
    TK_HIP(hipStreamWaitEvent(s, mod->graph_pre, 0));
  }
  TK_HIP(hipGraphLaunch(mod->graphs[gi].ge, s));
  if (capture) {
    TK_HIP(hipEventRecord(mod->capture_done, s));
    mod->capture_recorded = true;
    mod->capture_plain = true;
    TK_HIP(hipStreamWaitEvent(cs, mod->capture_done, 0));
  }
  mod->have_times = false;
  return TK_OK;
}

int tk_module_wait_capture(tk_module* mod, void* stream) {
  if (!mod) {
    tk::set_error("tk_module_wait_capture: null module");
    return TK_ERR_INVALID_ARG;
  }
  return wait_capture(mod, tk::as_stream(stream));
}

int tk_module_run_range(tk_module* mod, int begin, int end, void* stream) {
  if (!mod || begin < 0 || end > (int)mod->nodes.size() || begin > end) {
    tk::set_error("tk_module_run_range: bad range");
    return TK_ERR_INVALID_ARG;
  }
  hipStream_t s = tk::as_stream(stream);
  int rc0 = wait_capture(mod, s);
  if (rc0) return rc0;
  for (int i = begin; i < end; ++i) {
    int rc = tk::run_node(mod->nodes[i], s);
    if (rc) return rc;
  }
  return TK_OK;
}

int tk_module_run_order(tk_module* mod, const int32_t* order, int n, void* stream) {
// ... 302 lines not shown
```

### tachikoma_amd/csrc/tk_trace.hip

```cpp
#include <algorithm>
#include <climits>
#include <mutex>
#include <string>
#include <vector>

#include "tk_common.h"
#include "tk_wire.h"

namespace tk {

constexpr int kBlock = 256;
static inline int grid_for(int64_t work_items) {
  return (int)std::max<int64_t>(1, std::min<int64_t>((work_items + kBlock - 1) / kBlock, 256 * 8));
}

constexpr int kHostCopyMax = 6;
struct HostCopies {
  const uint8_t* src[kHostCopyMax];
  uint8_t* dst[kHostCopyMax];
  int64_t bytes[kHostCopyMax];
  int n;
};

__global__ __launch_bounds__(256) void host_copy_kernel(HostCopies c) {
  const int64_t stride = (int64_t)gridDim.x * 256;
  const int64_t t = (int64_t)blockIdx.x * 256 + threadIdx.x;
  for (int b = 0; b < c.n; ++b) {
    const uint8_t* src = c.src[b];
    uint8_t* dst = c.dst[b];
    int64_t n = c.bytes[b];
    const int64_t head = (int64_t)((16 - ((uintptr_t)dst & 15)) & 15) < n ? (int64_t)((16 - ((uintptr_t)dst & 15)) & 15) : n;
    for (int64_t i = t; i < head; i += stride) dst[i] = src[i];
    const int64_t n16 = (n - head) / 16;
    const uint64_t* s8 = reinterpret_cast<const uint64_t*>(src + head);
    tk_v4i* d16 = reinterpret_cast<tk_v4i*>(dst + head);
    if (((uintptr_t)(src + head) & 7) == 0) {
      for (int64_t i = t; i < n16; i += stride) {
        const uint64_t a = __builtin_nontemporal_load(s8 + 2 * i), bb = __builtin_nontemporal_load(s8 + 2 * i + 1);
        __builtin_nontemporal_store(tk_v4i{(int)(uint32_t)a, (int)(uint32_t)(a >> 32), (int)(uint32_t)bb, (int)(uint32_t)(bb >> 32)},
                                    d16 + i);
      }
    } else {
      for (int64_t i = t; i < n16 * 16; i += stride) dst[head + i] = src[head + i];
    }
    for (int64_t i = head + n16 * 16 + t; i < n; i += stride) dst[i] = src[i];
  }
}

int host_copy_impl(const void* const* src, void* const* dst, const int64_t* bytes, int n, hipStream_t s) {
  TK_CHECK_ARG(n >= 0 && n <= kHostCopyMax, "host copy: too many buffers");
  HostCopies c{};
  int64_t total = 0;
  int k = 0;
  for (int i = 0; i < n; ++i) {
    if (!dst[i] || bytes[i] <= 0) continue;
    c.src[k] = (const uint8_t*)src[i];
    c.dst[k] = (uint8_t*)dst[i];
    c.bytes[k] = bytes[i];
    total += bytes[i];
    ++k;
  }
  c.n = k;
  if (!k) return TK_OK;
  const int grid = (int)std::max<int64_t>(1, std::min<int64_t>(128, (total / 16 + 255) / 256));
  hipLaunchKernelGGL(host_copy_kernel, dim3(grid), dim3(256), 0, s, c);
  TK_LAUNCH_CHECK();
  return TK_OK;
}

struct PackRec {
  const uint8_t* src;
  int64_t dst;
  int64_t bytes;
  int64_t first_blk;
};

__device__ __forceinline__ uint32_t funnel(uint32_t lo, uint32_t hi, uint32_t r) {
  return r ? __builtin_amdgcn_alignbyte(hi, lo, r) : lo;
}

__global__ __launch_bounds__(256) void pack_records_kernel(const PackRec* __restrict__ recs, int nrec,
                                                           uint8_t* __restrict__ mirror) {
  int lo = 0, hi = nrec - 1;
  const int64_t b = blockIdx.x;
  while (lo < hi) {
    const int mid = (lo + hi + 1) >> 1;
    if (recs[mid].first_blk <= b) lo = mid;
    else hi = mid - 1;
  }
  const PackRec r = recs[lo];
  const int64_t a0 = r.dst & ~(int64_t)15;
  const int64_t a = a0 + ((b - r.first_blk) * 256 + threadIdx.x) * 16;
  const int64_t end = r.dst + r.bytes;
  if (a >= end) return;
  if (a >= r.dst && a + 16 <= end) {
    const int64_t so = a - r.dst;
    const int64_t base = so & ~(int64_t)15;
    const uint32_t s = (uint32_t)(so - base);
    tk_v4i v0 = __builtin_nontemporal_load(reinterpret_cast<const tk_v4i*>(r.src + base));
    tk_v4i out;
    if (s == 0) {
      out = v0;
    } else {
      tk_v4i v1 = __builtin_nontemporal_load(reinterpret_cast<const tk_v4i*>(r.src + base + 16));
      const uint32_t w[8] = {(uint32_t)v0.x, (uint32_t)v0.y, (uint32_t)v0.z, (uint32_t)v0.w,
                             (uint32_t)v1.x, (uint32_t)v1.y, (uint32_t)v1.z, (uint32_t)v1.w};
      const uint32_t q = s >> 2, rb = s & 3;
      uint32_t o[4];
#pragma unroll
      for (int k = 0; k < 4; ++k) {
        const uint32_t x0 = q == 0 ? w[k] : q == 1 ? w[k + 1] : q == 2 ? w[k + 2] : w[k + 3];
        const uint32_t x1 = q == 0 ? w[k + 1] : q == 1 ? w[k + 2] : q == 2 ? w[k + 3] : w[k + 4];
        o[k] = funnel(x0, x1, rb);
      }
      out = tk_v4i{(int)o[0], (int)o[1], (int)o[2], (int)o[3]};
    }
    *reinterpret_cast<tk_v4i*>(mirror + a) = out;
  } else {
    const int64_t from = a > r.dst ? a : r.dst;
    const int64_t to = a + 16 < end ? a + 16 : end;
    for (int64_t i = from; i < to; ++i) mirror[i] = r.src[i - r.dst];
  }
}

int pack_records_impl(const void* table, int nrec, int64_t blocks, void* mirror, hipStream_t s) {
  TK_CHECK_ARG(table && mirror && nrec > 0 && blocks > 0, "bad arguments");
  hipLaunchKernelGGL(pack_records_kernel, dim3((unsigned)blocks), dim3(256), 0, s, (const PackRec*)table, nrec,
                     (uint8_t*)mirror);
  TK_LAUNCH_CHECK();
  return TK_OK;
}

__device__ __forceinline__ uint32_t wire_byte(const uint32_t* w, int j) { return (w[j >> 2] >> (8 * (j & 3))) & 0xFFu; }

enum { kWireCursor = 0, kWireSize = 1, kWirePlace = 2 };

template <int kMode>
__global__ __launch_bounds__(256) void wire_encode_kernel(const WireSegDev* __restrict__ segs, uint32_t* cursor,
                                                          uint32_t* __restrict__ table, uint8_t* __restrict__ payload,
                                                          uint32_t cap_units) {
  __shared__ int32_t s_base[kWireSegBlocks];
  __shared__ uint32_t s_w[kWireSegBlocks];
  __shared__ uint32_t s_off[kWireSegBlocks];
  __shared__ uint32_t s_start;
  const WireSegDev sg = segs[blockIdx.x];
  const int n = sg.n;
  const int nb = (n + kWireBlock - 1) / kWireBlock;
  const int g = threadIdx.x >> 4, l = threadIdx.x & 15;
  const bool aligned = ((((uintptr_t)sg.src) | ((uintptr_t)sg.prev)) & 15) == 0;
  const bool bytes = sg.kind != kWireI32;
  const int32_t* src32 = static_cast<const int32_t*>(sg.src);
  const int32_t* prev32 = static_cast<const int32_t*>(sg.prev);
  uint32_t v[4][16];
  if (bytes) {
    const uint8_t* src8 = static_cast<const uint8_t*>(sg.src);
    const uint8_t* prev8 = static_cast<const uint8_t*>(sg.prev);
    const uint32_t flip = sg.kind == kWireI8 ? 0x80u : 0u;
#pragma unroll
    for (int p = 0; p < 4; ++p) {
      const int b = p * 16 + g;
      const int e0 = b * kWireBlock + l * 16;
      const int valid = min(16, n - e0);
      uint32_t pv[4] = {0, 0, 0, 0};
      if (aligned && valid == 16) {
        const tk_v4i a = *reinterpret_cast<const tk_v4i*>(src8 + e0);
        v[p][0] = (uint32_t)a.x, v[p][1] = (uint32_t)a.y, v[p][2] = (uint32_t)a.z, v[p][3] = (uint32_t)a.w;
        if (prev8) {
          const tk_v4i c = *reinterpret_cast<const tk_v4i*>(prev8 + e0);
          pv[0] = (uint32_t)c.x, pv[1] = (uint32_t)c.y, pv[2] = (uint32_t)c.z, pv[3] = (uint32_t)c.w;
        }
      } else {
        v[p][0] = v[p][1] = v[p][2] = v[p][3] = 0;
#pragma unroll
        for (int j = 0; j < 16; ++j)
          if (j < valid) {
            v[p][j >> 2] |= (uint32_t)src8[e0 + j] << (8 * (j & 3));
            if (prev8) pv[j >> 2] |= (uint32_t)prev8[e0 + j] << (8 * (j & 3));
          }
      }
      uint32_t lo = 0xFFu, hi = 0u;
#pragma unroll
      for (int j = 0; j < 16; ++j)
        if (j < valid) {
          const uint32_t x = wire_byte(v[p], j) ^ flip;
          lo = min(lo, x), hi = max(hi, x);
        }
#pragma unroll
      for (int m = 8; m >= 1; m >>= 1) {
        lo = min(lo, (uint32_t)__shfl_xor((int)lo, m, 16));
        hi = max(hi, (uint32_t)__shfl_xor((int)hi, m, 16));
      }
      int coded = 0;
      if (prev8) {
        coded = 1;
#pragma unroll
        for (int j = 0; j < 16; ++j)
          if (j < valid) coded &= min(max(wire_byte(pv, j) ^ flip, lo), hi) == (wire_byte(v[p], j) ^ flip);
#pragma unroll
        for (int m = 8; m >= 1; m >>= 1) coded &= __shfl_xor(coded, m, 16);
      }
      coded |= lo == hi;
      if (l == 0 && b < nb) s_base[b] = (int32_t)((lo ^ flip) | ((hi ^ flip) << 8)), s_w[b] = coded ? 0u : 1u;
    }
  } else {
#pragma unroll
    for (int p = 0; p < 4; ++p) {
      const int b = p * 16 + g;
      const int e0 = b * kWireBlock + l * 16;
      int32_t mn = INT_MAX, mx = INT_MIN;
      if (aligned && e0 + 16 <= n) {
#pragma unroll
        for (int q = 0; q < 4; ++q) {
          const tk_v4i a = *reinterpret_cast<const tk_v4i*>(src32 + e0 + 4 * q);
          v[p][4 * q] = (uint32_t)a.x, v[p][4 * q + 1] = (uint32_t)a.y, v[p][4 * q + 2] = (uint32_t)a.z,
                   v[p][4 * q + 3] = (uint32_t)a.w;
        }
        if (prev32) {
#pragma unroll
          for (int q = 0; q < 4; ++q) {
            const tk_v4i a = *reinterpret_cast<const tk_v4i*>(prev32 + e0 + 4 * q);
            v[p][4 * q] -= (uint32_t)a.x, v[p][4 * q + 1] -= (uint32_t)a.y, v[p][4 * q + 2] -= (uint32_t)a.z,
                v[p][4 * q + 3] -= (uint32_t)a.w;
          }
        }
#pragma unroll
        for (int j = 0; j < 16; ++j) mn = min(mn, (int32_t)v[p][j]), mx = max(mx, (int32_t)v[p][j]);
      } else {
#pragma unroll
        for (int j = 0; j < 16; ++j) {
          uint32_t x = 0;
          if (e0 + j < n) {
            x = (uint32_t)src32[e0 + j];
            if (prev32) x -= (uint32_t)prev32[e0 + j];
            mn = min(mn, (int32_t)x), mx = max(mx, (int32_t)x);
          }
          v[p][j] = x;
        }
      }
#pragma unroll
      for (int m = 8; m >= 1; m >>= 1) {
        mn = min(mn, __shfl_xor(mn, m, 16));
        mx = max(mx, __shfl_xor(mx, m, 16));
      }
      const uint32_t range = (uint32_t)mx - (uint32_t)mn;
      const uint32_t w = range == 0 ? 0 : range <= 0xFFu ? 1 : range <= 0xFFFFu ? 2 : range <= 0xFFFFFFu ? 3 : 4;
      if (l == 0 && b < nb) s_base[b] = mn, s_w[b] = w;
#pragma unroll
      for (int j = 0; j < 16; ++j) v[p][j] -= (uint32_t)mn;
    }
  }
  __syncthreads();
  const uint32_t base_bytes = (uint32_t)((4 * nb + 15) & ~15);
  const uint32_t hdr = base_bytes + (uint32_t)((nb + 15) & ~15);
  if (threadIdx.x == 0) {
    uint32_t off = hdr;
    for (int b = 0; b < nb; ++b) {
      s_off[b] = off;
      off += s_w[b] * (uint32_t)min(kWireBlock, n - b * kWireBlock);
    }
    const uint32_t units = (off + 63) >> 6;
    if constexpr (kMode == kWireSize) {
      table[blockIdx.x] = units;
      return;
    }
    const uint32_t start = kMode == kWirePlace ? table[blockIdx.x] : atomicAdd(cursor, units);
    if constexpr (kMode == kWireCursor) table[blockIdx.x] = start;
    s_start = start <= cap_units && units <= cap_units - start ? start : 0xFFFFFFFFu;
  }
  if constexpr (kMode == kWireSize) return;
  __syncthreads();
  if (s_start == 0xFFFFFFFFu) return;
  uint8_t* out = payload + (uint64_t)s_start * 64;
  if ((int)threadIdx.x < (int)(base_bytes >> 2))
    reinterpret_cast<int32_t*>(out)[threadIdx.x] = (int)threadIdx.x < nb ? s_base[threadIdx.x] : 0;
  if ((int)threadIdx.x < (int)((hdr - base_bytes) >> 2)) {
    uint32_t ww = 0;
#pragma unroll
    for (int j = 0; j < 4; ++j) {
      const int b = (int)threadIdx.x * 4 + j;
      if (b < nb) ww |= s_w[b] << (8 * j);
    }
    reinterpret_cast<uint32_t*>(out + base_bytes)[threadIdx.x] = ww;
  }
#pragma unroll
  for (int p = 0; p < 4; ++p) {
    const int b = p * 16 + g;
    if (b >= nb) continue;
    const int cnt = min(kWireBlock, n - b * kWireBlock);
    const uint32_t w = s_w[b];
    uint8_t* q = out + s_off[b];
    if (bytes) {
      if (w == 0) continue;
      if (cnt == kWireBlock) {
        __builtin_nontemporal_store(tk_v4i{(int)v[p][0], (int)v[p][1], (int)v[p][2], (int)v[p][3]},
                                    reinterpret_cast<tk_v4i*>(q + l * 16));
      } else {
#pragma unroll
        for (int j = 0; j < 16; ++j)
          if (l * 16 + j < cnt) q[l * 16 + j] = (uint8_t)wire_byte(v[p], j);
      }
      continue;
    }
    for (uint32_t k = 0; k < w; ++k) {
      const uint32_t sh = 8 * k;
      uint32_t o[4];
#pragma unroll
      for (int c = 0; c < 4; ++c)
        o[c] = ((v[p][4 * c] >> sh) & 0xFFu) | (((v[p][4 * c + 1] >> sh) & 0xFFu) << 8) |
               (((v[p][4 * c + 2] >> sh) & 0xFFu) << 16) | (((v[p][4 * c + 3] >> sh) & 0xFFu) << 24);
      if (cnt == kWireBlock) {
        __builtin_nontemporal_store(tk_v4i{(int)o[0], (int)o[1], (int)o[2], (int)o[3]},
                                    reinterpret_cast<tk_v4i*>(q + k * kWireBlock + l * 16));
      } else {
#pragma unroll
        for (int j = 0; j < 16; ++j)
          if (l * 16 + j < cnt) q[k * cnt + l * 16 + j] = (uint8_t)(o[j >> 2] >> (8 * (j & 3)));
      }
    }
  }
  if constexpr (kMode == kWirePlace) {
    const uint32_t end = s_off[nb - 1] + s_w[nb - 1] * (uint32_t)(n - (nb - 1) * kWireBlock);
    const uint32_t at = end + threadIdx.x;
    if (at < ((end + 63) & ~63u)) out[at] = 0;
  }
}

int wire_encode_impl(const WireSegDev* segs, int64_t n_seg, uint32_t* cursor, void* wire, int64_t wire_bytes,
                     hipStream_t s) {
  const int64_t table = wire_table_bytes(n_seg);
  TK_CHECK_ARG(segs && cursor && wire && n_seg > 0 && n_seg < ((int64_t)1 << 31) && ((uintptr_t)wire & 63) == 0 &&
               wire_bytes >= table, "bad arguments");
  const int64_t cap_units = std::min<int64_t>((wire_bytes - table) / 64, 0xFFFFFFF0ll);
  hipLaunchKernelGGL(wire_encode_kernel<kWireCursor>, dim3((unsigned)n_seg), dim3(256), 0, s, segs, cursor, (uint32_t*)wire,
                     (uint8_t*)wire + table, (uint32_t)cap_units);
  TK_LAUNCH_CHECK();
  return TK_OK;
}

constexpr int kWireScanItems = kWireScanTile / 256;

template <typename T>
__global__ __launch_bounds__(256) void wire_scan_tile_kernel(T* v, uint64_t* __restrict__ sums, int64_t n) {
  __shared__ uint64_t s_sum[256];
  const int t = threadIdx.x;
  const int64_t i0 = (int64_t)blockIdx.x * kWireScanTile + (int64_t)t * kWireScanItems;
  T x[kWireScanItems];
  uint64_t mine = 0;
#pragma unroll
  for (int j = 0; j < kWireScanItems; ++j) {
    x[j] = i0 + j < n ? v[i0 + j] : (T)0;
    mine += x[j];
  }
  s_sum[t] = mine;
  __syncthreads();
  for (int d = 1; d < 256; d <<= 1) {
    const uint64_t below = t >= d ? s_sum[t - d] : 0;
    __syncthreads();
    s_sum[t] += below;
    __syncthreads();
  }
  uint64_t at = s_sum[t] - mine;
#pragma unroll
  for (int j = 0; j < kWireScanItems; ++j) {
    if (i0 + j < n) v[i0 + j] = (T)at;
    at += x[j];
  }
  if (t == 255) sums[blockIdx.x] = s_sum[255];
}

template <typename T>
__global__ __launch_bounds__(256) void wire_scan_add_kernel(T* __restrict__ v, const uint64_t* __restrict__ offs, int64_t n) {
  const int64_t i = (int64_t)blockIdx.x * 256 + threadIdx.x;
  if (i < n) v[i] += (T)offs[i / kWireScanTile];
}

static std::vector<int64_t> wire_scan_levels(int64_t n_seg) {
  std::vector<int64_t> cnt{n_seg};
  do cnt.push_back((cnt.back() + kWireScanTile - 1) / kWireScanTile);
  while (cnt.back() > 1);
  return cnt;
}

static int64_t wire_scan_words(int64_t n_seg) {
  int64_t words = 0;
  const std::vector<int64_t> cnt = wire_scan_levels(n_seg);
  for (size_t k = 1; k < cnt.size(); ++k) words += cnt[k];
  return words;
}

static int wire_pack_plan_impl(const WireSegDev* segs, int64_t n_seg, void* wire, uint64_t* scan, hipStream_t s) {
  TK_CHECK_ARG(segs && wire && scan && n_seg > 0 && n_seg < ((int64_t)1 << 31) && ((uintptr_t)wire & 63) == 0,
               "bad arguments");
  const std::vector<int64_t> cnt = wire_scan_levels(n_seg);
  const int top = (int)cnt.size() - 1;
  std::vector<uint64_t*> lev(cnt.size(), nullptr);
  for (int k = 1; k <= top; ++k) lev[k] = k == 1 ? scan : lev[k - 1] + cnt[k - 1];
  uint32_t* table = (uint32_t*)wire;
  TK_HIP(hipMemsetAsync(wire, 0, (size_t)wire_table_bytes(n_seg), s));
  hipLaunchKernelGGL(wire_encode_kernel<kWireSize>, dim3((unsigned)n_seg), dim3(256), 0, s, segs, (uint32_t*)nullptr, table,
                     (uint8_t*)nullptr, 0u);
  TK_LAUNCH_CHECK();
  hipLaunchKernelGGL(wire_scan_tile_kernel<uint32_t>, dim3((unsigned)cnt[1]), dim3(256), 0, s, table, lev[1], n_seg);
  TK_LAUNCH_CHECK();
  for (int k = 1; k < top; ++k) {
    hipLaunchKernelGGL(wire_scan_tile_kernel<uint64_t>, dim3((unsigned)cnt[k + 1]), dim3(256), 0, s, lev[k], lev[k + 1],
                       cnt[k]);
    TK_LAUNCH_CHECK();
  }
  for (int k = top - 2; k >= 1; --k) {
    hipLaunchKernelGGL(wire_scan_add_kernel<uint64_t>, dim3((unsigned)((cnt[k] + 255) / 256)), dim3(256), 0, s, lev[k],
                       lev[k + 1], cnt[k]);
    TK_LAUNCH_CHECK();
  }
  if (top >= 2) {
    hipLaunchKernelGGL(wire_scan_add_kernel<uint32_t>, dim3((unsigned)((n_seg + 255) / 256)), dim3(256), 0, s, table,
                       lev[1], n_seg);
    TK_LAUNCH_CHECK();
  }
  return TK_OK;
}

static int wire_pack_place_impl(const WireSegDev* segs, int64_t n_seg, void* wire, int64_t wire_bytes, hipStream_t s) {
  const int64_t table = wire_table_bytes(n_seg);
  TK_CHECK_ARG(segs && wire && n_seg > 0 && n_seg < ((int64_t)1 << 31) && ((uintptr_t)wire & 63) == 0 &&
               wire_bytes >= table, "bad arguments");
  const int64_t cap_units = std::min<int64_t>((wire_bytes - table) / 64, 0xFFFFFFF0ll);
  hipLaunchKernelGGL(wire_encode_kernel<kWirePlace>, dim3((unsigned)n_seg), dim3(256), 0, s, segs, (uint32_t*)nullptr,
                     (uint32_t*)wire, (uint8_t*)wire + table, (uint32_t)cap_units);
  TK_LAUNCH_CHECK();
  return TK_OK;
}

enum { kWireStore = 0, kWireCompare = 1 };


template <int kMode>
__global__ __launch_bounds__(256) void wire_decode_kernel(const WireUnitDev* __restrict__ units,
                                                          const WireSegOut* __restrict__ segs,
                                                          const uint32_t* __restrict__ table,
                                                          const uint8_t* __restrict__ payload, int64_t payload_bytes,
                                                          tk_wire_mismatch* report, uint32_t* status) {
  __shared__ int32_t s_base[kWireSegBlocks];
  __shared__ uint32_t s_w[kWireSegBlocks];
  __shared__ uint32_t s_off[kWireSegBlocks];
  __shared__ uint32_t s_bad;
  __shared__ uint32_t s_any[4];
  __shared__ unsigned long long s_red[8];
  const WireUnitDev un = units[blockIdx.x];
  const int n = un.n;
  const int nb = (n + kWireBlock - 1) / kWireBlock;
  const int g = threadIdx.x >> 4, l = threadIdx.x & 15;
  const bool bytes = un.kind != kWireI32;
  const uint32_t max_w = bytes ? 1u : 4u;
  const uint32_t flip = un.kind == kWireI8 ? 0x80u : 0u;
  const uint32_t base_bytes = (uint32_t)((4 * nb + 15) & ~15);
  const uint32_t hdr = base_bytes + (uint32_t)((nb + 15) & ~15);
  uint32_t v[4][16];
#pragma unroll
  for (int p = 0; p < 4; ++p)
#pragma unroll
    for (int j = 0; j < 16; ++j) v[p][j] = 0;
  for (int m = 0; m < un.count; ++m) {
    const int64_t si = un.first + (int64_t)m * un.stride;
    const int64_t off = (int64_t)table[si] * 64;
    if (threadIdx.x == 0) s_bad = 0;
    __syncthreads();
    const bool head_ok = off <= payload_bytes && (int64_t)hdr <= payload_bytes - off;
    const uint8_t* seg = payload + off;
    if (head_ok && threadIdx.x < 64) {
      const int b = threadIdx.x;
      uint32_t w = 0, x = 0;
      if (b < nb) {
        w = seg[base_bytes + b];
        s_base[b] = *reinterpret_cast<const int32_t*>(seg + 4 * b);
        s_w[b] = w;
        if (w > max_w) s_bad = 1, w = 0;
        x = w * (uint32_t)min(kWireBlock, n - b * kWireBlock);
      }
      uint32_t incl = x;
#pragma unroll
      for (int d = 1; d < 64; d <<= 1) {
        const uint32_t y = (uint32_t)__shfl_up((int)incl, d, 64);
        if (b >= d) incl += y;
      }
      if (b < nb) s_off[b] = hdr + incl - x;
      if (b == 63 && (int64_t)(hdr + incl) > payload_bytes - off) s_bad = 1;
    }
    __syncthreads();
    if (!head_ok || s_bad) {
      if (threadIdx.x == 0) *status = 1;
      return;
    }
    const WireSegOut so = segs[si];
    const uint64_t e_seg = (uint64_t)un.e0;
    uint32_t mis = 0, first = 0xFFFFFFFFu;
    if (bytes) {
      uint8_t* dst8 = static_cast<uint8_t*>(so.dst);
      const bool aligned = ((uintptr_t)dst8 & 15) == 0;
#pragma unroll
      for (int p = 0; p < 4; ++p) {
        const int b = p * 16 + g;
        if (b >= nb) continue;
        const int cnt = min(kWireBlock, n - b * kWireBlock);
        const int e0 = b * kWireBlock + l * 16;
        const int valid = min(16, n - e0);
        const uint32_t lo = (uint32_t)s_base[b] & 0xFFu, hi = ((uint32_t)s_base[b] >> 8) & 0xFFu;
        if (s_w[b]) {
          const uint8_t* q = seg + s_off[b];
          if (cnt == kWireBlock) {
            const tk_v4i a = __builtin_nontemporal_load(reinterpret_cast<const tk_v4i*>(q + l * 16));
            v[p][0] = (uint32_t)a.x, v[p][1] = (uint32_t)a.y, v[p][2] = (uint32_t)a.z, v[p][3] = (uint32_t)a.w;
          } else {
            v[p][0] = v[p][1] = v[p][2] = v[p][3] = 0;
#pragma unroll
            for (int j = 0; j < 16; ++j)
              if (j < valid) v[p][j >> 2] |= (uint32_t)q[l * 16 + j] << (8 * (j & 3));
          }
        } else if (m > 0) {
#pragma unroll
          for (int c = 0; c < 4; ++c) {
            uint32_t o = 0;
#pragma unroll
            for (int k = 0; k < 4; ++k) {
              const uint32_t x = ((v[p][c] >> (8 * k)) & 0xFFu) ^ flip;
              o |= (min(max(x, lo ^ flip), hi ^ flip) ^ flip) << (8 * k);
            }
            v[p][c] = o;
          }
        } else {
          v[p][0] = v[p][1] = v[p][2] = v[p][3] = lo * 0x01010101u;
        }
        if (!dst8 || valid <= 0) continue;
        if (aligned && valid == 16) {
          tk_v4i* d = reinterpret_cast<tk_v4i*>(dst8 + e0);
          if constexpr (kMode == kWireStore) {
            *d = tk_v4i{(int)v[p][0], (int)v[p][1], (int)v[p][2], (int)v[p][3]};
          } else {
            const tk_v4i a = *d;
            const uint32_t got[4] = {(uint32_t)a.x, (uint32_t)a.y, (uint32_t)a.z, (uint32_t)a.w};
            if (got[0] != v[p][0] || got[1] != v[p][1] || got[2] != v[p][2] || got[3] != v[p][3]) {
#pragma unroll
              for (int j = 15; j >= 0; --j)
                if (wire_byte(got, j) != wire_byte(v[p], j)) ++mis, first = min(first, (uint32_t)(e0 + j));
            }
          }
        } else {
#pragma unroll
          for (int j = 15; j >= 0; --j) {
            if (j >= valid) continue;
            if constexpr (kMode == kWireStore) dst8[e0 + j] = (uint8_t)wire_byte(v[p], j);
            else if (dst8[e0 + j] != (uint8_t)wire_byte(v[p], j)) ++mis, first = min(first, (uint32_t)(e0 + j));
          }
        }
      }
    } else {
      int32_t* dst32 = static_cast<int32_t*>(so.dst);
      const bool aligned = ((uintptr_t)dst32 & 15) == 0;
#pragma unroll
      for (int p = 0; p < 4; ++p) {
        const int b = p * 16 + g;
        if (b >= nb) continue;
        const int cnt = min(kWireBlock, n - b * kWireBlock);
        const int e0 = b * kWireBlock + l * 16;
        const int valid = min(16, n - e0);
        const uint32_t w = s_w[b];
        const uint8_t* q = seg + s_off[b];
        uint32_t c[16];
#pragma unroll
        for (int j = 0; j < 16; ++j) c[j] = 0;
        for (uint32_t k = 0; k < w; ++k) {
          uint32_t o[4] = {0, 0, 0, 0};
          if (cnt == kWireBlock) {
            const tk_v4i a = __builtin_nontemporal_load(reinterpret_cast<const tk_v4i*>(q + k * kWireBlock + l * 16));
            o[0] = (uint32_t)a.x, o[1] = (uint32_t)a.y, o[2] = (uint32_t)a.z, o[3] = (uint32_t)a.w;
          } else {
#pragma unroll
            for (int j = 0; j < 16; ++j)
              if (j < valid) o[j >> 2] |= (uint32_t)q[k * cnt + l * 16 + j] << (8 * (j & 3));
          }
#pragma unroll
          for (int j = 0; j < 16; ++j) c[j] |= wire_byte(o, j) << (8 * k);
        }
        const uint32_t base = (uint32_t)s_base[b];
#pragma unroll
        for (int j = 0; j < 16; ++j) v[p][j] = (m > 0 ? v[p][j] : 0u) + base + c[j];
        if (!dst32 || valid <= 0) continue;
        if (aligned && valid == 16) {
#pragma unroll
          for (int q4 = 0; q4 < 4; ++q4) {
            tk_v4i* d = reinterpret_cast<tk_v4i*>(dst32 + e0 + 4 * q4);
            if constexpr (kMode == kWireStore) {
              *d = tk_v4i{(int)v[p][4 * q4], (int)v[p][4 * q4 + 1], (int)v[p][4 * q4 + 2], (int)v[p][4 * q4 + 3]};
            } else {
              const tk_v4i a = *d;
              const uint32_t got[4] = {(uint32_t)a.x, (uint32_t)a.y, (uint32_t)a.z, (uint32_t)a.w};
#pragma unroll
              for (int j = 3; j >= 0; --j)
                if (got[j] != v[p][4 * q4 + j])
                  ++mis, first = min(first, (uint32_t)(e0 + 4 * q4 + j));
            }
          }
        } else {
#pragma unroll
          for (int j = 15; j >= 0; --j) {
            if (j >= valid) continue;
            if constexpr (kMode == kWireStore) dst32[e0 + j] = (int32_t)v[p][j];
            else if ((uint32_t)dst32[e0 + j] != v[p][j]) ++mis, first = min(first, (uint32_t)(e0 + j));
          }
        }
      }
    }
    if constexpr (kMode == kWireCompare) {
      if (so.dst)
        wire_report_mismatches(mis, first == 0xFFFFFFFFu ? ~0ull : (unsigned long long)(e_seg + first), report + so.rec,
                               s_any, s_red);
    }
  }
}

__global__ __launch_bounds__(256) void wire_report_init_kernel(tk_wire_mismatch* report, int n) {
  const int i = blockIdx.x * 256 + threadIdx.x;
  if (i < n) report[i].mismatches = 0, report[i].first = ~0ull;
}

int wire_report_init(tk_wire_mismatch* report, int n, hipStream_t s) {
  hipLaunchKernelGGL(wire_report_init_kernel, dim3((unsigned)((n + 255) / 256)), dim3(256), 0, s, report, n);
  TK_LAUNCH_CHECK();
  return TK_OK;
}

static int wire_unpack_impl(const void* units, int64_t n_units, const void* segs, const void* wire, int64_t n_seg,
                     int64_t wire_bytes, int mode, tk_wire_mismatch* report, int n_report, uint32_t* status,
                     hipStream_t s) {
  const int64_t table = wire_table_bytes(n_seg);
  TK_CHECK_ARG(units && segs && wire && status && n_units > 0 && n_units < ((int64_t)1 << 31) &&
               ((uintptr_t)wire & 63) == 0 && wire_bytes >= table && (mode == kWireStore || (report && n_report > 0)),
               "bad arguments");
  const uint8_t* payload = (const uint8_t*)wire + table;
  if (mode == kWireStore) {
    hipLaunchKernelGGL(wire_decode_kernel<kWireStore>, dim3((unsigned)n_units), dim3(256), 0, s,
                       (const WireUnitDev*)units, (const WireSegOut*)segs, (const uint32_t*)wire, payload,
                       wire_bytes - table, (tk_wire_mismatch*)nullptr, status);
  } else {
    hipLaunchKernelGGL(wire_report_init_kernel, dim3((unsigned)((n_report + 255) / 256)), dim3(256), 0, s, report, n_report);
    TK_LAUNCH_CHECK();
    hipLaunchKernelGGL(wire_decode_kernel<kWireCompare>, dim3((unsigned)n_units), dim3(256), 0, s,
                       (const WireUnitDev*)units, (const WireSegOut*)segs, (const uint32_t*)wire, payload,
                       wire_bytes - table, report, status);
  }
  TK_LAUNCH_CHECK();
  return TK_OK;
}

__global__ __launch_bounds__(256) void compare_kernel(const ComparePair* __restrict__ pairs, int n_pairs,
                                                      tk_wire_mismatch* report) {
  __shared__ uint32_t s_any[4];
  __shared__ unsigned long long s_red[8];
  int lo = 0, hi = n_pairs - 1;
  const int64_t blk = blockIdx.x;
  while (lo < hi) {
    const int mid = (lo + hi + 1) >> 1;
    if (pairs[mid].first_blk <= blk) lo = mid;
    else hi = mid - 1;
  }
  const ComparePair pr = pairs[lo];
  const int64_t at = ((blk - pr.first_blk) * 256 + threadIdx.x) * 16;
  uint32_t mask = 0;
  if (at < pr.bytes) {
    const uint8_t* a = pr.expected + at;
    const uint8_t* b = pr.got + at;
    const uintptr_t both = (uintptr_t)a | (uintptr_t)b;
    if (at + 16 <= pr.bytes && (both & 3) == 0) {
      uint32_t x[4], y[4];
      if ((both & 15) == 0) {
        const tk_v4i p = __builtin_nontemporal_load(reinterpret_cast<const tk_v4i*>(a));
        const tk_v4i q = __builtin_nontemporal_load(reinterpret_cast<const tk_v4i*>(b));
        x[0] = (uint32_t)p.x, x[1] = (uint32_t)p.y, x[2] = (uint32_t)p.z, x[3] = (uint32_t)p.w;
        y[0] = (uint32_t)q.x, y[1] = (uint32_t)q.y, y[2] = (uint32_t)q.z, y[3] = (uint32_t)q.w;
      } else {
#pragma unroll
        for (int c = 0; c < 4; ++c)
          x[c] = reinterpret_cast<const uint32_t*>(a)[c], y[c] = reinterpret_cast<const uint32_t*>(b)[c];
      }
      if (x[0] != y[0] || x[1] != y[1] || x[2] != y[2] || x[3] != y[3]) {
#pragma unroll
        for (int j = 0; j < 16; ++j) mask |= (uint32_t)(wire_byte(x, j) != wire_byte(y, j)) << j;
      }
    } else {
      const int valid = (int)min((int64_t)16, pr.bytes - at);
#pragma unroll
      for (int j = 0; j < 16; ++j)
        if (j < valid) mask |= (uint32_t)(a[j] != b[j]) << j;
    }
  }
  uint32_t mis = 0;
  unsigned long long first = ~0ull;
  if (mask) {
    const int es = pr.elem_bytes;
    const uint32_t em = (1u << es) - 1u;
    for (int e = 16 / es - 1; e >= 0; --e)
      if ((mask >> (e * es)) & em) ++mis, first = (unsigned long long)(at / es + e);
  }
  wire_report_mismatches(mis, first, report + lo, s_any, s_red);
}

static int compare_impl(const void* pairs, int n_pairs, int64_t blocks, tk_wire_mismatch* report, hipStream_t s) {
  TK_CHECK_ARG(pairs && report && n_pairs > 0 && blocks > 0 && blocks < ((int64_t)1 << 31), "bad arguments");
  hipLaunchKernelGGL(wire_report_init_kernel, dim3((unsigned)((n_pairs + 255) / 256)), dim3(256), 0, s, report, n_pairs);
  TK_LAUNCH_CHECK();
  hipLaunchKernelGGL(compare_kernel, dim3((unsigned)blocks), dim3(256), 0, s, (const ComparePair*)pairs, n_pairs, report);
  TK_LAUNCH_CHECK();
  return TK_OK;
}

__device__ __forceinline__ uint64_t mix64(uint64_t z) {
  z = (z ^ (z >> 30)) * 0xBF58476D1CE4E5B9ULL;
  z = (z ^ (z >> 27)) * 0x94D049BB133111EBULL;
  return z ^ (z >> 31);
}

__global__ __launch_bounds__(kBlock) void digest_kernel(const uint8_t* __restrict__ p, int64_t nbytes,
                                                         unsigned long long* out) {
  int64_t nw = (nbytes + 7) / 8;
  int64_t stride = (int64_t)gridDim.x * kBlock;
  uint64_t acc = 0;
  for (int64_t i = blockIdx.x * (int64_t)kBlock + threadIdx.x; i < nw; i += stride) {
    uint64_t w = 0;
    if ((i + 1) * 8 <= nbytes) {
      __builtin_memcpy(&w, p + i * 8, 8);
    } else {
      for (int b = 0; i * 8 + b < nbytes; ++b) w |= (uint64_t)p[i * 8 + b] << (8 * b);
    }
    acc += mix64(w ^ ((uint64_t)i * 0x9E3779B97F4A7C15ULL));
  }
  for (int off = 32; off > 0; off >>= 1) acc += __shfl_xor(acc, off);
  if ((threadIdx.x & 63) == 0) atomicAdd(out, (unsigned long long)acc);
}

}

namespace {
std::vector<tk::WireSegDev> source_segs(const tk::WirePlan& plan, const tk_wire_record* recs, const void* const* src) {
  std::vector<tk::WireSegDev> segs;
  segs.reserve(plan.segs.size());
  for (const tk::WireSegRef& r : plan.segs) {
    const tk::WireSegAddr a = tk::wire_seg_addr(r, recs[r.rec].kind, src[r.rec], recs[r.rec].diff ? src[r.rec - 1] : nullptr);
    segs.push_back({a.at, a.prev, r.n, recs[r.rec].kind});
  }
  return segs;
}

struct DeviceScratch {
  std::mutex mu;
  void* dev = nullptr;
  int64_t bytes = 0;
  int device = -1;
  int reserve(int64_t need, char** out) {
    int cur = 0;
    TK_HIP(hipGetDevice(&cur));
    if (device != cur || bytes < need) {
      if (dev) (void)hipFree(dev);
      dev = nullptr, bytes = 0;
      TK_HIP(hipMalloc(&dev, (size_t)need));
      bytes = need, device = cur;
    }
    *out = (char*)dev;
    return TK_OK;
  }
};
DeviceScratch g_pack_scratch;
DeviceScratch g_unpack_scratch;
}

extern "C" {

int tk_digest_bytes(const void* data, int64_t nbytes, uint64_t* out_device, void* stream) {
  hipStream_t s = tk::as_stream(stream);
  TK_CHECK_ARG(out_device && (data || nbytes == 0), "null argument");
  TK_HIP(hipMemsetAsync(out_device, 0, 8, s));
  if (nbytes == 0) return TK_OK;
  hipLaunchKernelGGL(tk::digest_kernel, dim3(tk::grid_for((nbytes + 7) / 8)), dim3(tk::kBlock), 0, s, (const uint8_t*)data,
                     nbytes, (unsigned long long*)out_device);
  TK_LAUNCH_CHECK();
  return TK_OK;
}

int tk_wire_encode_device(const tk_wire_record* recs, int n_recs, const void* const* src, void* wire,
                          int64_t wire_cap, void* stream) {
  tk::WirePlan plan;
  if (const int rc = tk::wire_plan(recs, n_recs, -1, "tk_wire_encode_device", &plan)) return rc;
  if (!src || !wire || wire_cap < plan.bound) {
    tk::set_error("tk_wire_encode_device: the wire buffer is smaller than tk_wire_bound");
    return TK_ERR_INVALID_ARG;
  }
  const std::vector<tk::WireSegDev> segs = source_segs(plan, recs, src);
  hipStream_t s = tk::as_stream(stream);
  void* dev = nullptr;
  TK_HIP(hipMalloc(&dev, segs.size() * sizeof(tk::WireSegDev) + 64));
  uint32_t* cursor = (uint32_t*)((char*)dev + segs.size() * sizeof(tk::WireSegDev));
  int rc = TK_OK;
  if (hipMemcpyAsync(dev, segs.data(), segs.size() * sizeof(tk::WireSegDev), hipMemcpyHostToDevice, s) != hipSuccess ||
      hipMemsetAsync(cursor, 0, sizeof(uint32_t), s) != hipSuccess) {
    tk::set_error("tk_wire_encode_device: loading the segment table failed");
    rc = TK_ERR_HIP;
  }
  if (rc == TK_OK) rc = tk::wire_encode_impl((const tk::WireSegDev*)dev, (int64_t)segs.size(), cursor, wire, plan.bound, s);
  if (hipStreamSynchronize(s) != hipSuccess && rc == TK_OK) {
    tk::set_error("tk_wire_encode_device: the encode kernel failed");
    rc = TK_ERR_HIP;
  }
  (void)hipFree(dev);
  return rc;
}

int64_t tk_wire_pack_device(const tk_wire_record* recs, int n_recs, const void* const* src, void* wire,
                            int64_t wire_cap, void* stream) {
  tk::WirePlan plan;
  if (const int rc = tk::wire_plan(recs, n_recs, -1, "tk_wire_pack_device", &plan)) return rc;
  if (!src || !wire || ((uintptr_t)wire & 63) != 0 || wire_cap < plan.bound) {
    tk::set_error("tk_wire_pack_device: the wire buffer is not 64-byte aligned or smaller than tk_wire_bound");
    return TK_ERR_INVALID_ARG;
  }
  const std::vector<tk::WireSegDev> segs = source_segs(plan, recs, src);
  const int64_t n_seg = (int64_t)segs.size();
  const int64_t table = tk::wire_table_bytes(n_seg);
  const int64_t seg_bytes = tk::wire_align(n_seg * (int64_t)sizeof(tk::WireSegDev), 64);
  const int64_t words = tk::wire_scan_words(n_seg);
  hipStream_t s = tk::as_stream(stream);
  std::lock_guard<std::mutex> lock(g_pack_scratch.mu);
  char* dev = nullptr;
  int rc = g_pack_scratch.reserve(seg_bytes + 8 * words, &dev);
  if (rc != TK_OK) return rc;
  const tk::WireSegDev* dev_segs = (const tk::WireSegDev*)dev;
  uint64_t* scan = (uint64_t*)(dev + seg_bytes);
  TK_HIP(hipMemcpyAsync(dev, segs.data(), segs.size() * sizeof(tk::WireSegDev), hipMemcpyHostToDevice, s));
  rc = tk::wire_pack_plan_impl(dev_segs, n_seg, wire, scan, s);
  if (rc != TK_OK) return rc;
  uint64_t total = 0;
  TK_HIP(hipMemcpyAsync(&total, scan + words - 1, sizeof(total), hipMemcpyDeviceToHost, s));
  TK_HIP(hipStreamSynchronize(s));
  if (total > 0xFFFFFFF0ull) {
    tk::set_error("tk_wire_pack_device: the packed records do not fit the format's 32-bit segment starts");
    return TK_ERR_UNSUPPORTED;
  }
  const int64_t used = table + 64 * (int64_t)total;
  if (used > plan.bound) {
    tk::set_error("tk_wire_pack_device: the segment sizes exceed tk_wire_bound");
    return TK_ERR_HIP;
  }
  rc = tk::wire_pack_place_impl(dev_segs, n_seg, wire, used, s);
  if (rc != TK_OK) return rc;
  if (hipStreamSynchronize(s) != hipSuccess) {
    tk::set_error("tk_wire_pack_device: the place kernel failed");
    return TK_ERR_HIP;
  }
  return used;
}

int tk_wire_pack_tile(void) { return tk::kWireScanTile; }

int tk_wire_unpack_device(const tk_wire_record* recs, int n_recs, const void* wire, int64_t wire_bytes,
                          void* const* dst, int mode, tk_wire_mismatch* report, void* stream) {
  tk::WirePlan plan;
  if (const int rc = tk::wire_plan(recs, n_recs, -1, "tk_wire_unpack_device", &plan)) return rc;
  const bool compare = mode == TK_WIRE_UNPACK_COMPARE;
  if (!wire || !dst || ((uintptr_t)wire & 63) != 0 || (mode != TK_WIRE_UNPACK_STORE && !compare) ||
      (compare && !report)) {
    tk::set_error("tk_wire_unpack_device: null argument, unknown mode or a wire buffer that is not 64-byte aligned");
    return TK_ERR_INVALID_ARG;
  }
  for (int i = 0; i < n_recs; ++i)
    if (recs[i].kind == tk::kWireI32 && ((uintptr_t)dst[i] & 3) != 0) {
      tk::set_error("tk_wire_unpack_device: the buffer of int32 record " + std::to_string(i) + " is not 4-byte aligned");
      return TK_ERR_INVALID_ARG;
    }
  const std::vector<tk::WireSegRef>& refs = plan.segs;
  const std::vector<tk::WireUnit>& units = plan.units;
  const int64_t n_seg = (int64_t)refs.size(), n_units = (int64_t)units.size();
  if (wire_bytes < tk::wire_table_bytes(n_seg)) {
    tk::set_error("tk_wire_unpack_device: the segment table does not lie inside the wire buffer");
    return TK_ERR_INVALID_ARG;
  }
  std::vector<tk::WireSegOut> segs(refs.size());
  for (size_t i = 0; i < refs.size(); ++i)
    segs[i] = {tk::wire_seg_addr(refs[i], recs[refs[i].rec].kind, dst[refs[i].rec], nullptr).at, refs[i].rec, 0};
  std::vector<tk::WireUnitDev> udev(units.size());
  for (size_t u = 0; u < units.size(); ++u) {
    const tk::WireSegRef& r = refs[units[u].first];
    udev[u] = {units[u].first, units[u].stride, units[u].count, r.n, recs[r.rec].kind, 0, r.e0};
  }
  const int64_t seg_bytes = tk::wire_align(n_seg * (int64_t)sizeof(tk::WireSegOut), 64);
  const int64_t unit_bytes = tk::wire_align(n_units * (int64_t)sizeof(tk::WireUnitDev), 64);
  const int64_t rep_bytes = tk::wire_align((int64_t)n_recs * (int64_t)sizeof(tk_wire_mismatch), 64);
  hipStream_t s = tk::as_stream(stream);
  std::lock_guard<std::mutex> lock(g_unpack_scratch.mu);
  char* dev = nullptr;
  int rc = g_unpack_scratch.reserve(seg_bytes + unit_bytes + rep_bytes + 64, &dev);
  if (rc != TK_OK) return rc;
  tk_wire_mismatch* rep = (tk_wire_mismatch*)(dev + seg_bytes + unit_bytes);
  uint32_t* status = (uint32_t*)(dev + seg_bytes + unit_bytes + rep_bytes);
  TK_HIP(hipMemcpyAsync(dev, segs.data(), segs.size() * sizeof(tk::WireSegOut), hipMemcpyHostToDevice, s));
  TK_HIP(hipMemcpyAsync(dev + seg_bytes, udev.data(), udev.size() * sizeof(tk::WireUnitDev), hipMemcpyHostToDevice, s));
  TK_HIP(hipMemsetAsync(status, 0, sizeof(uint32_t), s));
  rc = tk::wire_unpack_impl(dev + seg_bytes, n_units, dev, wire, n_seg, wire_bytes, mode, rep, n_recs, status, s);
  if (rc != TK_OK) return rc;
  uint32_t bad = 0;
  if (compare) TK_HIP(hipMemcpyAsync(report, rep, (size_t)n_recs * sizeof(tk_wire_mismatch), hipMemcpyDeviceToHost, s));
  TK_HIP(hipMemcpyAsync(&bad, status, sizeof(bad), hipMemcpyDeviceToHost, s));
  if (hipStreamSynchronize(s) != hipSuccess) {
    tk::set_error("tk_wire_unpack_device: the decode kernel failed");
    return TK_ERR_HIP;
  }
  if (bad) {
    tk::set_error("tk_wire_unpack_device: a segment does not lie inside the wire buffer or states a width its kind "
                  "does not have (was the buffer checked with tk_wire_check?)");
    return TK_ERR_INVALID_ARG;
  }
  return TK_OK;
}

int tk_compare_device_batch(const void* const* expected, const void* const* got, const int64_t* n_elems,
                            const int32_t* elem_bytes, int n, tk_wire_mismatch* report, void* stream) {
  if (!expected || !got || !n_elems || !elem_bytes || !report || n < 1) {
    tk::set_error("tk_compare_device_batch: null argument or no pairs");
    return TK_ERR_INVALID_ARG;
  }
  std::vector<tk::ComparePair> pairs;
  std::vector<int> index;
  int64_t blocks = 0;
  for (int i = 0; i < n; ++i) {
    const int es = elem_bytes[i];
    if ((es != 1 && es != 2 && es != 4 && es != 8) || n_elems[i] < 0 || n_elems[i] > ((int64_t)1 << 40) ||
        (n_elems[i] > 0 && (!expected[i] || !got[i]))) {
      tk::set_error("tk_compare_device_batch: pair " + std::to_string(i) +
                    " has a null buffer, a negative count or an element size other than 1, 2, 4, 8");
      return TK_ERR_INVALID_ARG;
    }
    report[i].mismatches = 0, report[i].first = ~(uint64_t)0;
    if (n_elems[i] == 0) continue;
    const int64_t bytes = n_elems[i] * es;
    pairs.push_back({(const uint8_t*)expected[i], (const uint8_t*)got[i], bytes, blocks, es, 0});
    index.push_back(i);
    blocks += (bytes + 4095) / 4096;
  }
  if (pairs.empty()) return TK_OK;
  if (blocks >= ((int64_t)1 << 31)) {
    tk::set_error("tk_compare_device_batch: too much to compare in one launch");
    return TK_ERR_UNSUPPORTED;
  }
  const int np = (int)pairs.size();
  const int64_t pair_bytes = tk::wire_align(np * (int64_t)sizeof(tk::ComparePair), 64);
  hipStream_t s = tk::as_stream(stream);
  std::lock_guard<std::mutex> lock(g_unpack_scratch.mu);
  char* dev = nullptr;
  int rc = g_unpack_scratch.reserve(pair_bytes + np * (int64_t)sizeof(tk_wire_mismatch), &dev);
  if (rc != TK_OK) return rc;
  tk_wire_mismatch* rep = (tk_wire_mismatch*)(dev + pair_bytes);
  TK_HIP(hipMemcpyAsync(dev, pairs.data(), pairs.size() * sizeof(tk::ComparePair), hipMemcpyHostToDevice, s));
  rc = tk::compare_impl(dev, np, blocks, rep, s);
  if (rc != TK_OK) return rc;
  std::vector<tk_wire_mismatch> out(np);
  TK_HIP(hipMemcpyAsync(out.data(), rep, (size_t)np * sizeof(tk_wire_mismatch), hipMemcpyDeviceToHost, s));
  if (hipStreamSynchronize(s) != hipSuccess) {
    tk::set_error("tk_compare_device_batch: the compare kernel failed");
    return TK_ERR_HIP;
  }
  for (int k = 0; k < np; ++k) report[index[k]] = out[k];
  return TK_OK;
}

int tk_compare_device(const void* expected, const void* got, int64_t n_elems, int elem_bytes,
                      tk_wire_mismatch* report, void* stream) {
  const int32_t es = elem_bytes;
  return tk_compare_device_batch(&expected, &got, &n_elems, &es, 1, report, stream);
}

}
```

### tachikoma_amd/csrc/tk_wire.cc

```cpp
#include "tk_wire.h"

#include <sched.h>

#include <algorithm>
#include <atomic>
#include <chrono>
#include <condition_variable>
#include <cstdlib>
#include <cstring>
#include <mutex>
#include <string>
#include <thread>

namespace tk {
void set_error(const std::string& msg);

int wire_plan(const tk_wire_record* recs, int n_recs, int64_t image_bytes, const char* who, WirePlan* p) {
  if (!recs || n_recs < 1) {
    set_error(std::string(who) + ": no records");
    return TK_ERR_INVALID_ARG;
  }
  int64_t n_seg = 0;
  for (int i = 0; i < n_recs; ++i) {
    const int kind = recs[i].kind;
    const int64_t esize = wire_elem_bytes(kind);
    const bool inside = kind >= kWireI32 && kind <= kWireU8 && recs[i].offset >= 0 && recs[i].n_elems >= 1 &&
                        recs[i].n_elems <= ((int64_t)1 << 40) &&
                        (image_bytes < 0 ||
                         (recs[i].offset <= image_bytes && esize * recs[i].n_elems <= image_bytes - recs[i].offset));
    if (!inside || (recs[i].diff && (i == 0 || recs[i - 1].n_elems != recs[i].n_elems || recs[i - 1].kind != kind))) {
      set_error(std::string(who) + ": record " + std::to_string(i) +
                " is of no known kind, lies outside the image or follows (diff) a record of another size or kind");
      return TK_ERR_INVALID_ARG;
    }
    n_seg += (recs[i].n_elems + kWireSegElems - 1) / kWireSegElems;
  }
  if (n_seg >= ((int64_t)1 << 31)) {
    set_error(std::string(who) + ": too many segments");
    return TK_ERR_UNSUPPORTED;
  }
  p->segs.clear(), p->units.clear();
  p->segs.reserve((size_t)n_seg);
  p->bound = wire_table_bytes(n_seg);
  int r = 0;
  while (r < n_recs) {
    int k = 1;
    while (r + k < n_recs && recs[r + k].diff) ++k;
    const int64_t n = recs[r].n_elems;
    const int64_t S = (n + kWireSegElems - 1) / kWireSegElems;
    const int64_t first = (int64_t)p->segs.size();
    for (int m = 0; m < k; ++m)
      for (int64_t j = 0; j < S; ++j) {
        const int32_t sn = (int32_t)std::min<int64_t>(kWireSegElems, n - j * kWireSegElems);
        p->segs.push_back({r + m, sn, j * kWireSegElems});
        p->bound += wire_seg_bound(sn, wire_elem_bytes(recs[r].kind));
      }
    for (int64_t j = 0; j < S; ++j) p->units.push_back({(int32_t)(first + j), (int32_t)S, k});
    r += k;
  }
  return TK_OK;
}

namespace {
class Pool {
 public:
  static Pool& get() {
    static Pool* p = new Pool();
    return *p;
  }
  int size() const { return n_; }
  template <typename F>
  void run(int64_t count, int threads, F&& fn) {
    std::lock_guard<std::mutex> job(job_mu_);
    struct Ctx {
      F* fn;
    } ctx{&fn};
    {
      std::lock_guard<std::mutex> lk(mu_);
      call_ = [](void* c, int64_t i) { (*static_cast<Ctx*>(c)->fn)(i); };
      ctx_ = &ctx;
      count_ = count;
      next_.store(0, std::memory_order_relaxed);
      limit_ = threads > 0 ? std::min(threads, n_) : n_;
      active_ = limit_;
      ++gen_;
    }
    cv_.notify_all();
    std::unique_lock<std::mutex> lk(mu_);
    done_cv_.wait(lk, [&] { return active_ == 0; });
  }

 private:
  Pool() {
    int n = 0;
    cpu_set_t set;
    CPU_ZERO(&set);
    if (sched_getaffinity(0, sizeof(set), &set) == 0) n = CPU_COUNT(&set);
    n = std::max(1, std::min(n, 16));
    if (const char* e = std::getenv("TK_WIRE_THREADS")) {
      const int v = std::atoi(e);
      if (v >= 1 && v <= 16) n = v;
    }
    n_ = n;
    for (int t = 0; t < n_; ++t) std::thread([this, t] { worker(t); }).detach();
  }
  void worker(int id) {
    uint64_t seen = 0;
    for (;;) {
      void (*call)(void*, int64_t);
      void* ctx;
      int64_t count;
      {
        std::unique_lock<std::mutex> lk(mu_);
        cv_.wait(lk, [&] { return gen_ != seen; });
        seen = gen_;
        if (id >= limit_) continue;
        call = call_, ctx = ctx_, count = count_;
      }
      for (int64_t i; (i = next_.fetch_add(1, std::memory_order_relaxed)) < count;) call(ctx, i);
      std::lock_guard<std::mutex> lk(mu_);
      if (--active_ == 0) done_cv_.notify_all();
    }
  }
  int n_ = 1;
  std::mutex job_mu_, mu_;
  std::condition_variable cv_, done_cv_;
  uint64_t gen_ = 0;
  void (*call_)(void*, int64_t) = nullptr;
  void* ctx_ = nullptr;
  int64_t count_ = 0;
  int limit_ = 0, active_ = 0;
  std::atomic<int64_t> next_{0};
};

template <int W, bool D>
void widen(char* dst, const char* prev, const uint8_t* p, int cnt, uint32_t base) {
  for (int i = 0; i < cnt; ++i) {
    uint32_t v = base;
    if (W >= 1) v += p[i];
    if (W >= 2) v += (uint32_t)p[cnt + i] << 8;
    if (W >= 3) v += (uint32_t)p[2 * cnt + i] << 16;
    if (W >= 4) v += (uint32_t)p[3 * cnt + i] << 24;
    if (D) {
      uint32_t q;
      std::memcpy(&q, prev + 4 * (int64_t)i, 4);
      v += q;
    }
    std::memcpy(dst + 4 * (int64_t)i, &v, 4);
  }
}
template <bool D>
void widen_w(int w, char* dst, const char* prev, const uint8_t* p, int cnt, uint32_t base) {
  switch (w) {
    case 0: return widen<0, D>(dst, prev, p, cnt, base);
    case 1: return widen<1, D>(dst, prev, p, cnt, base);
    case 2: return widen<2, D>(dst, prev, p, cnt, base);
    case 3: return widen<3, D>(dst, prev, p, cnt, base);
    default: return widen<4, D>(dst, prev, p, cnt, base);
  }
}

inline uint8_t clamp_u8(uint8_t x, uint8_t lo, uint8_t hi) {
  x = x < lo ? lo : x;
  return x > hi ? hi : x;
}
void clamp_block(char* dst, const char* prev, int cnt, uint8_t lo, uint8_t hi, uint8_t flip) {
  int i = 0;
  for (; i + 32 <= cnt; i += 32) {
    uint8_t v[32];
    std::memcpy(v, prev + i, 32);
    for (int j = 0; j < 32; ++j) v[j] = (uint8_t)(clamp_u8((uint8_t)(v[j] ^ flip), lo, hi) ^ flip);
    std::memcpy(dst + i, v, 32);
  }
  for (; i < cnt; ++i) dst[i] = (char)(clamp_u8((uint8_t)((uint8_t)prev[i] ^ flip), lo, hi) ^ flip);
}

}

int64_t wire_seg_extent(int kind, int n, uint32_t start, const char* payload, int64_t payload_bytes) {
  const int64_t off = (int64_t)start * 64;
  const int nb = (n + kWireBlock - 1) / kWireBlock;
  const int64_t hdr = wire_header_bytes(nb);
  if (off > payload_bytes || hdr > payload_bytes - off) return -1;
  const uint8_t* widths = (const uint8_t*)payload + off + wire_align(4 * (int64_t)nb, 16);
  int64_t len = hdr;
  const int max_w = kind == kWireI32 ? 4 : 1;
  for (int b = 0; b < nb; ++b) {
    if (widths[b] > max_w) return -1;
    len += (int64_t)widths[b] * std::min(kWireBlock, n - b * kWireBlock);
  }
  return len > payload_bytes - off ? -1 : len;
}

namespace {
int64_t decode_seg(const WireJob& j, int64_t i, const char* payload, int64_t payload_bytes) {
  const WireSegHost& sg = j.segs[i];
  uint32_t start;
  std::memcpy(&start, j.wire + 4 * i, 4);
  const int64_t len = wire_seg_extent(sg.kind, sg.n, start, payload, payload_bytes);
  if (len < 0) return -1;
  const int nb = (sg.n + kWireBlock - 1) / kWireBlock;
  const int64_t hdr = wire_header_bytes(nb);
  const char* p = payload + (int64_t)start * 64;
  const uint8_t* widths = (const uint8_t*)p + wire_align(4 * (int64_t)nb, 16);
  const uint8_t* q = (const uint8_t*)p + hdr;
  if (sg.kind != kWireI32) {
    const uint8_t flip = sg.kind == kWireI8 ? 0x80 : 0;
    for (int b = 0; b < nb; ++b) {
      const int cnt = std::min(kWireBlock, sg.n - b * kWireBlock);
      char* dst = sg.dst + (int64_t)b * kWireBlock;
      const uint8_t lo = (uint8_t)p[4 * b], hi = (uint8_t)p[4 * b + 1];
      if (widths[b]) std::memcpy(dst, q, (size_t)cnt), q += cnt;
      else if (sg.prev) clamp_block(dst, sg.prev + (int64_t)b * kWireBlock, cnt, lo ^ flip, hi ^ flip, flip);
      else std::memset(dst, lo, (size_t)cnt);
    }
    return wire_align(len, 64);
  }
  for (int b = 0; b < nb; ++b) {
    const int cnt = std::min(kWireBlock, sg.n - b * kWireBlock);
    const int w = widths[b];
    int32_t base;
    std::memcpy(&base, p + 4 * b, 4);
    char* dst = sg.dst + 4 * (int64_t)b * kWireBlock;
    if (sg.prev) widen_w<true>(w, dst, sg.prev + 4 * (int64_t)b * kWireBlock, q, cnt, (uint32_t)base);
    else widen_w<false>(w, dst, nullptr, q, cnt, (uint32_t)base);
    q += (int64_t)w * cnt;
  }
  return wire_align(len, 64);
}
}

int wire_pool_threads() { return Pool::get().size(); }

int wire_decode(WireJob* job, int threads) {
  const auto t0 = std::chrono::steady_clock::now();
  job->status = 0;
  job->used_bytes = 0;
  const int64_t table = wire_table_bytes(job->n_seg);
  if (job->n_seg < 0 || !job->wire || job->wire_bytes < table) {
    job->status = TK_ERR_INVALID_ARG;
    return job->status;
  }
  std::atomic<int64_t> used{table};
  std::atomic<int> bad{0};
  const char* payload = job->wire + table;
  const int64_t payload_bytes = job->wire_bytes - table;
  Pool::get().run(job->n_units, threads, [&](int64_t u) {
    const WireUnit& un = job->units[u];
    int64_t sum = 0;
    for (int m = 0; m < un.count; ++m) {
      const int64_t r = decode_seg(*job, un.first + (int64_t)m * un.stride, payload, payload_bytes);
      if (r < 0) {
        bad.store(1, std::memory_order_relaxed);
        break;
      }
      sum += r;
    }
    used.fetch_add(sum, std::memory_order_relaxed);
  });
  job->used_bytes = used.load();
  job->status = bad.load() ? TK_ERR_INVALID_ARG : 0;
  job->ms = std::chrono::duration<double, std::milli>(std::chrono::steady_clock::now() - t0).count();
  return job->status;
}

namespace {
int64_t encode_seg(const char* src, const char* prev, int n, char* out) {
  const int nb = (n + kWireBlock - 1) / kWireBlock;
  const int64_t hdr = wire_header_bytes(nb);
  std::memset(out, 0, (size_t)hdr);
  uint8_t* widths = (uint8_t*)out + wire_align(4 * (int64_t)nb, 16);
  uint8_t* q = (uint8_t*)out + hdr;
  for (int b = 0; b < nb; ++b) {
    const int cnt = std::min(kWireBlock, n - b * kWireBlock);
    int32_t v[kWireBlock];
    for (int i = 0; i < cnt; ++i) {
      uint32_t a, pv = 0;
      std::memcpy(&a, src + 4 * ((int64_t)b * kWireBlock + i), 4);
      if (prev) std::memcpy(&pv, prev + 4 * ((int64_t)b * kWireBlock + i), 4);
      v[i] = (int32_t)(a - pv);
    }
    const int32_t mn = *std::min_element(v, v + cnt), mx = *std::max_element(v, v + cnt);
    const uint32_t range = (uint32_t)mx - (uint32_t)mn;
    const int w = range == 0 ? 0 : range <= 0xFFu ? 1 : range <= 0xFFFFu ? 2 : range <= 0xFFFFFFu ? 3 : 4;
    std::memcpy(out + 4 * b, &mn, 4);
    widths[b] = (uint8_t)w;
    for (int k = 0; k < w; ++k)
      for (int i = 0; i < cnt; ++i) q[k * cnt + i] = (uint8_t)(((uint32_t)v[i] - (uint32_t)mn) >> (8 * k));
    q += (int64_t)w * cnt;
  }
  return (char*)q - out;
}

int64_t encode_seg8(const char* src, const char* prev, int n, int kind, char* out) {
  const int nb = (n + kWireBlock - 1) / kWireBlock;
  const int64_t hdr = wire_header_bytes(nb);
  std::memset(out, 0, (size_t)hdr);
  uint8_t* widths = (uint8_t*)out + wire_align(4 * (int64_t)nb, 16);
  uint8_t* q = (uint8_t*)out + hdr;
  const uint8_t flip = kind == kWireI8 ? 0x80 : 0;
  for (int b = 0; b < nb; ++b) {
    const int cnt = std::min(kWireBlock, n - b * kWireBlock);
    const uint8_t* a = (const uint8_t*)src + (int64_t)b * kWireBlock;
    uint8_t lo = 0xFF, hi = 0;
    for (int i = 0; i < cnt; ++i) lo = std::min<uint8_t>(lo, a[i] ^ flip), hi = std::max<uint8_t>(hi, a[i] ^ flip);
    bool coded = lo == hi;
    if (prev && !coded) {
      const uint8_t* pv = (const uint8_t*)prev + (int64_t)b * kWireBlock;
      coded = true;
      for (int i = 0; i < cnt && coded; ++i) coded = clamp_u8((uint8_t)(pv[i] ^ flip), lo, hi) == (uint8_t)(a[i] ^ flip);
    }
    out[4 * b] = (char)(lo ^ flip), out[4 * b + 1] = (char)(hi ^ flip);
    widths[b] = coded ? 0 : 1;
    if (!coded) std::memcpy(q, a, (size_t)cnt), q += cnt;
  }
  return (char*)q - out;
}
}
}

extern "C" {

int64_t tk_wire_bound(const tk_wire_record* recs, int n_recs) {
  tk::WirePlan p;
  const int rc = tk::wire_plan(recs, n_recs, -1, "tk_wire_bound", &p);
  return rc ? rc : p.bound;
}

int64_t tk_wire_encode_host(const tk_wire_record* recs, int n_recs, const void* image, int64_t image_bytes,
                            void* wire, int64_t wire_cap) {
  tk::WirePlan p;
  if (const int rc = tk::wire_plan(recs, n_recs, image_bytes, "tk_wire_encode_host", &p)) return rc;
  if (!image || !wire || wire_cap < p.bound) {
    tk::set_error("tk_wire_encode_host: the wire buffer is smaller than tk_wire_bound");
    return TK_ERR_INVALID_ARG;
  }
  const int64_t table = tk::wire_table_bytes((int64_t)p.segs.size());
  std::memset(wire, 0, (size_t)table);
  char* payload = (char*)wire + table;
  int64_t cursor = 0;
  for (size_t i = 0; i < p.segs.size(); ++i) {
    const tk::WireSegRef& s = p.segs[i];
    const int kind = recs[s.rec].kind;
    const tk::WireSegAddr a =
        tk::wire_seg_addr(s, kind, (const char*)image + recs[s.rec].offset,
                          recs[s.rec].diff ? (const char*)image + recs[s.rec - 1].offset : nullptr);
    const uint32_t start = (uint32_t)(cursor / 64);
    std::memcpy((char*)wire + 4 * i, &start, 4);
    const int64_t len = kind == tk::kWireI32 ? tk::encode_seg(a.at, a.prev, s.n, payload + cursor)
                                             : tk::encode_seg8(a.at, a.prev, s.n, kind, payload + cursor);
    const int64_t padded = tk::wire_align(len, 64);
    std::memset(payload + cursor + len, 0, (size_t)(padded - len));
    cursor += padded;
  }
  return table + cursor;
}

int tk_wire_decode(const tk_wire_record* recs, int n_recs, const void* wire, int64_t wire_bytes, void* image,
                   int64_t image_bytes, int threads) {
  tk::WirePlan p;
  if (const int rc = tk::wire_plan(recs, n_recs, image_bytes, "tk_wire_decode", &p)) return rc;
  if (!wire || !image || wire_bytes < 0) {
    tk::set_error("tk_wire_decode: null buffer");
    return TK_ERR_INVALID_ARG;
  }
  std::vector<tk::WireSegHost> segs(p.segs.size());
  for (size_t i = 0; i < p.segs.size(); ++i) {
    const tk::WireSegRef& s = p.segs[i];
    const tk::WireSegAddr a =
        tk::wire_seg_addr(s, recs[s.rec].kind, (char*)image + recs[s.rec].offset,
                          recs[s.rec].diff ? (const char*)image + recs[s.rec - 1].offset : nullptr);
    segs[i] = {a.at, a.prev, s.n, recs[s.rec].kind};
  }
  tk::WireJob job{(const char*)wire, wire_bytes, segs.data(), (int64_t)segs.size(),
                  p.units.data(), (int64_t)p.units.size()};
  if (tk::wire_decode(&job, threads)) {
    tk::set_error("tk_wire_decode: the segment table or a segment does not lie inside the wire buffer");
    return TK_ERR_INVALID_ARG;
  }
  return TK_OK;
}

int tk_wire_check(const tk_wire_record* recs, int n_recs, const void* wire, int64_t wire_bytes) {
  tk::WirePlan p;
  if (const int rc = tk::wire_plan(recs, n_recs, -1, "tk_wire_check", &p)) return rc;
  const int64_t n_seg = (int64_t)p.segs.size();
  const int64_t table = tk::wire_table_bytes(n_seg);
  if (!wire || wire_bytes < table) {
    tk::set_error("tk_wire_check: the segment table does not lie inside the wire buffer");
    return TK_ERR_INVALID_ARG;
  }
  const char* payload = (const char*)wire + table;
  for (int64_t i = 0; i < n_seg; ++i) {
    uint32_t start;
    std::memcpy(&start, (const char*)wire + 4 * i, 4);
    if (tk::wire_seg_extent(recs[p.segs[i].rec].kind, p.segs[i].n, start, payload, wire_bytes - table) < 0) {
      tk::set_error("tk_wire_check: segment " + std::to_string(i) + " (record " + std::to_string(p.segs[i].rec) +
                    ") does not lie inside the wire buffer or states a width its kind does not have");
      return TK_ERR_INVALID_ARG;
    }
  }
  return TK_OK;
}

int tk_wire_threads(void) { return tk::wire_pool_threads(); }

}
```

### tachikoma_amd/csrc/tk_wire.h

```cpp
#pragma once

#include <stdint.h>

#include <vector>

#include "../../include/tachikoma.h"

namespace tk {

constexpr int kWireBlock = 256;
constexpr int kWireSegBlocks = 64;
constexpr int kWireSegElems = kWireBlock * kWireSegBlocks;
constexpr int kWireScanTile = 2048;

inline int64_t wire_align(int64_t x, int64_t a) { return (x + a - 1) / a * a; }
inline int64_t wire_table_bytes(int64_t n_seg) { return wire_align(4 * n_seg, 64); }
inline int64_t wire_header_bytes(int nb) { return wire_align(4 * (int64_t)nb, 16) + wire_align(nb, 16); }
enum WireKind : int32_t { kWireI32 = 0, kWireI8 = 1, kWireU8 = 2 };
inline int wire_elem_bytes(int kind) { return kind == kWireI32 ? 4 : 1; }
inline int64_t wire_seg_bound(int n, int esize = 4) {
  return wire_align(wire_header_bytes((n + kWireBlock - 1) / kWireBlock) + esize * (int64_t)n, 64);
}

struct WireSegDev {
  const void* src;
  const void* prev;
  int32_t n;
  int32_t kind;
};
struct WireSegOut {
  void* dst;
  int32_t rec;
  int32_t pad;
};
struct WireUnitDev {
  int32_t first, stride, count;
  int32_t n, kind;
  int32_t pad;
  int64_t e0;
};
struct ComparePair {
  const uint8_t* expected;
  const uint8_t* got;
  int64_t bytes;
  int64_t first_blk;
  int32_t elem_bytes;
  int32_t pad;
};
struct WireSegHost {
  char* dst;
  const char* prev;
  int32_t n;
  int32_t kind;
};
struct WireUnit {
  int32_t first, stride, count;
};
struct WireSegRef {
  int32_t rec;
  int32_t n;
  int64_t e0;
};

struct WirePlan {
  std::vector<WireSegRef> segs;
  std::vector<WireUnit> units;
  int64_t bound = 0;
};
int wire_plan(const tk_wire_record* recs, int n_recs, int64_t image_bytes, const char* who, WirePlan* plan);

struct WireSegAddr { char* at; const char* prev; };
inline WireSegAddr wire_seg_addr(const WireSegRef& s, int kind, const void* base, const void* prev_base) {
  const int64_t b0 = wire_elem_bytes(kind) * s.e0;
  return {base ? (char*)base + b0 : nullptr, prev_base ? (const char*)prev_base + b0 : nullptr};
}

int64_t wire_seg_extent(int kind, int n, uint32_t start, const char* payload, int64_t payload_bytes);

struct WireJob {
  const char* wire = nullptr;
  int64_t wire_bytes = 0;
  const WireSegHost* segs = nullptr;
  int64_t n_seg = 0;
  const WireUnit* units = nullptr;
  int64_t n_units = 0;
  int status = 0;
  int64_t used_bytes = 0;
  double ms = 0.0;
};
int wire_decode(WireJob* job, int threads);
int wire_pool_threads();

}
```

Measured before the change: 887.4 op-traces/s.

## Subtract per-channel bias from differenced int32 trace records before wire coding

Adds a bias-coded wire kind: when a traced int32 output differs from its predecessor only by a per-channel bias add (conv/dense block or bias_add), the encoder also subtracts the bias addend per channel so residuals become narrow and pack into fewer bytes. Bias values are snapshotted to device and host at plan time, and the device encoder and host decoder walk channel/plane positions to apply them. This cuts trace bytes moved to pinned host memory, at the cost of extra per-element integer div/mod and addend loads in the encode kernel, plus larger segment descriptors.

```diff
diff --git a/include/tachikoma.h b/include/tachikoma.h
--- a/include/tachikoma.h
+++ b/include/tachikoma.h
@@ -404,6 +404,10 @@
   int32_t diff;
   int32_t kind;
 } tk_wire_record;
+typedef struct {
+  int32_t plane, channels;
+  const int32_t* addend;
+} tk_wire_addend;
 int64_t tk_wire_bound(const tk_wire_record* recs, int n_recs);
 int64_t tk_wire_encode_host(const tk_wire_record* recs, int n_recs, const void* image, int64_t image_bytes,
                             void* wire, int64_t wire_cap);
@@ -415,6 +419,12 @@
                             int64_t wire_cap, void* stream);
 int tk_wire_pack_tile(void);
 int tk_wire_threads(void);
+int64_t tk_wire_encode_host_bias(const tk_wire_record* recs, const tk_wire_addend* addends, int n_recs, const void* image,
+                                 int64_t image_bytes, void* wire, int64_t wire_cap);
+int tk_wire_decode_bias(const tk_wire_record* recs, const tk_wire_addend* addends, int n_recs, const void* wire,
+                        int64_t wire_bytes, void* image, int64_t image_bytes, int threads);
+int tk_wire_encode_device_bias(const tk_wire_record* recs, const tk_wire_addend* addends, int n_recs,
+                               const void* const* src, void* wire, int64_t wire_cap, void* stream);
 
 typedef struct {
   uint64_t mismatches;
diff --git a/tachikoma_amd/_lib.py b/tachikoma_amd/_lib.py
--- a/tachikoma_amd/_lib.py
+++ b/tachikoma_amd/_lib.py
@@ -307,6 +307,14 @@
         ("n_elems", ctypes.c_int64),
         ("diff", ctypes.c_int32),
         ("kind", ctypes.c_int32),
+    ]
+
+
+class tk_wire_addend(ctypes.Structure):
+    _fields_ = [
+        ("plane", ctypes.c_int32),
+        ("channels", ctypes.c_int32),
+        ("addend", ctypes.c_void_p),
     ]
 
 
@@ -447,6 +455,12 @@
     "tk_wire_decode": (ctypes.c_int, [ctypes.POINTER(tk_wire_record), ctypes.c_int, _VP, _I64, _VP, _I64, ctypes.c_int]),
     "tk_wire_encode_device": (ctypes.c_int, [ctypes.POINTER(tk_wire_record), ctypes.c_int, ctypes.POINTER(_VP), _VP,
                                              _I64, _VP]),
+    "tk_wire_encode_host_bias": (_I64, [ctypes.POINTER(tk_wire_record), ctypes.POINTER(tk_wire_addend), ctypes.c_int, _VP,
+                                        _I64, _VP, _I64]),
+    "tk_wire_decode_bias": (ctypes.c_int, [ctypes.POINTER(tk_wire_record), ctypes.POINTER(tk_wire_addend), ctypes.c_int,
+                                           _VP, _I64, _VP, _I64, ctypes.c_int]),
+    "tk_wire_encode_device_bias": (ctypes.c_int, [ctypes.POINTER(tk_wire_record), ctypes.POINTER(tk_wire_addend),
+                                                  ctypes.c_int, ctypes.POINTER(_VP), _VP, _I64, _VP]),
     "tk_wire_pack_device": (_I64, [ctypes.POINTER(tk_wire_record), ctypes.c_int, ctypes.POINTER(_VP), _VP, _I64, _VP]),
     "tk_wire_pack_tile": (ctypes.c_int, []),
     "tk_wire_threads": (ctypes.c_int, []),
diff --git a/tachikoma_amd/csrc/tk_runtime.cc b/tachikoma_amd/csrc/tk_runtime.cc
--- a/tachikoma_amd/csrc/tk_runtime.cc
+++ b/tachikoma_amd/csrc/tk_runtime.cc
@@ -274,6 +274,8 @@
   };
   std::vector<WireChunk> wchunks;
   void* wire_segs = nullptr;
+  int32_t* addend_dev = nullptr;
+  std::vector<int32_t> addend_host;
   std::vector<void*> slots;
   uint32_t* cursors = nullptr;
   std::vector<hipEvent_t> slot_done;
@@ -285,6 +287,7 @@
     for (auto e : slot_done) (void)hipEventDestroy(e);
     for (void* p : slots) (void)hipHostFree(p);
     if (wire_segs) (void)hipFree(wire_segs);
+    if (addend_dev) (void)hipFree(addend_dev);
     if (cursors) (void)hipFree(cursors);
     for (int m = 0; m < 2; ++m) {
       for (auto x : ge[m]) (void)hipGraphExecDestroy(x);
@@ -324,7 +327,7 @@
   hipEvent_t ct_t0 = nullptr;
   std::vector<hipEvent_t> ct_ev;
   std::vector<int64_t> ct_bytes;
-  bool trace_wire = true, wire_forced_off = false, wire_clamp = true;
+  bool trace_wire = true, wire_forced_off = false, wire_clamp = true, wire_bias = true;
   hipStream_t wire_s = nullptr, dec_s = nullptr;
   hipEvent_t wire_tail = nullptr, decode_tail = nullptr;
   bool wire_tail_used = false;
@@ -497,6 +500,7 @@
   auto mod = std::make_unique<tk_module>();
   if (const char* e = std::getenv("TK_TRACE_WIRE")) mod->wire_forced_off = e[0] == '0' && e[1] == 0;
   if (const char* e = std::getenv("TK_WIRE_CLAMP")) mod->wire_clamp = !(e[0] == '0' && e[1] == 0);
+  if (const char* e = std::getenv("TK_WIRE_BIAS")) mod->wire_bias = !(e[0] == '0' && e[1] == 0);
   mod->nodes.resize(n_nodes);
   for (int i = 0; i < n_nodes; ++i) {
     const tk_node& src = nodes[i];
@@ -687,6 +691,9 @@
   const tk_tensor* t;
   bool wire, diff;
   bool clamp;
+  const tk_tensor* bias = nullptr;
+  int32_t plane = 0, channels = 0;
+  int64_t addend_at = 0;
 };
 
 static int collect_records(const tk_module* mod, const std::vector<void*>& dst, std::vector<PackRecord>* recs) {
@@ -713,6 +720,20 @@
   if ((block && d.attrs.block.has_clip) || (d.kind == TK_NODE_ADD_BLOCK && d.attrs.add_block.has_clip))
     return k >= 1 && k == d.n_outputs - 1 ? tk::ptr(&n.out[k - 1].t) : nullptr;
   return d.kind == TK_NODE_CLIP && k == 0 ? tk::ptr(&n.in[0].t) : nullptr;
+}
+
+static const tk_tensor* bias_input(const tk::Node& n, int k, const void* from, int* axis) {
+  const tk_node& d = n.desc;
+  if ((d.kind == TK_NODE_CONV_BLOCK || d.kind == TK_NODE_DENSE_BLOCK) && k == 1 && d.n_inputs >= 3 &&
+      tk::ptr(&n.out[0].t) == from) {
+    *axis = d.kind == TK_NODE_CONV_BLOCK ? 1 : n.out[1].t.ndim - 1;
+    return &n.in[2].t;
+  }
+  if (d.kind == TK_NODE_BIAS_ADD && k == 0 && d.n_inputs >= 2 && tk::ptr(&n.in[0].t) == from) {
+    *axis = d.attrs.bias_add.axis < 0 ? d.attrs.bias_add.axis + n.out[0].t.ndim : d.attrs.bias_add.axis;
+    return &n.in[1].t;
+  }
+  return nullptr;
 }
 
 static bool decide_coding(const tk_module* mod, std::vector<PackRecord>& recs) {
@@ -732,11 +753,20 @@
     any |= c.wire;
     if (!c.wire || r == 0 || !recs[r - 1].wire) continue;
     c.diff = same_shape && tk::is_int(b, 32) && c.src != recs[r - 1].src;
+    int axis = 0;
+    const tk_tensor* bias = c.diff && mod->wire_bias ? bias_input(mod->nodes[c.node], c.out, recs[r - 1].src, &axis) : nullptr;
+    if (!bias || !bias->data || axis < 0 || axis >= a->ndim || !tk::is_int(bias, 32) || !tk::compact(bias) ||
+        tk::numel(bias) != a->shape[axis] || a->shape[axis] < 1 || a->shape[axis] >= ((int64_t)1 << 31) ||
+        tk::numel(a) >= ((int64_t)1 << 31))
+      continue;
+    int64_t plane = 1;
+    for (int d = axis + 1; d < a->ndim; ++d) plane *= a->shape[d];
+    c.bias = bias, c.plane = (int32_t)plane, c.channels = (int32_t)a->shape[axis];
   }
   return any;
 }
 
-static int chunk_wire_tables(const std::vector<PackRecord>& recs, const std::vector<size_t>& coded,
+static int chunk_wire_tables(const std::vector<PackRecord>& recs, const std::vector<size_t>& coded, const PackPlan* plan,
                              PackPlan::WireChunk* wc, std::vector<tk::WireSegDev>& wire_segs) {
   std::vector<tk_wire_record> wrecs;
   for (size_t q = 0; q < coded.size(); ++q) {
@@ -758,8 +788,27 @@
     const tk::WireSegAddr img = tk::wire_seg_addr(sr, kind, r.host, pv ? pv->host : nullptr);
     wire_segs.push_back({dev.at, dev.prev, sr.n, kind});
     wc->segs.push_back({img.at, img.prev, sr.n, kind});
+    if (r.bias) {
+      tk::wire_seg_bias(&wire_segs.back(), plan->addend_dev + r.addend_at, r.plane, r.channels, sr.e0);
+      tk::wire_seg_bias(&wc->segs.back(), plan->addend_host.data() + r.addend_at, r.plane, r.channels, sr.e0);
+    }
   }
   for (size_t q : coded) wc->coded_bytes += recs[q].bytes;
+  return TK_OK;
+}
+
+static int snapshot_addends(PackPlan* plan, std::vector<PackRecord>& recs) {
+  int64_t total = 0;
+  for (PackRecord& r : recs)
+    if (r.bias) r.addend_at = total, total += r.channels;
+  if (!total) return TK_OK;
+  TK_HIP(hipMalloc((void**)&plan->addend_dev, (size_t)total * sizeof(int32_t)));
+  for (const PackRecord& r : recs)
+    if (r.bias)
+      TK_HIP(hipMemcpy(plan->addend_dev + r.addend_at, tk::ptr(r.bias), (size_t)r.channels * sizeof(int32_t),
+                       hipMemcpyDeviceToDevice));
+  plan->addend_host.resize((size_t)total);
+  TK_HIP(hipMemcpy(plan->addend_host.data(), plan->addend_dev, (size_t)total * sizeof(int32_t), hipMemcpyDeviceToHost));
   return TK_OK;
 }
 
@@ -809,7 +858,7 @@
     cut = upto;
     if (!plan->wire) continue;
     if (!w_rec.empty())
-      if (const int rc = chunk_wire_tables(recs, w_rec, &wc, wire_segs)) return rc;
+      if (const int rc = chunk_wire_tables(recs, w_rec, plan, &wc, wire_segs)) return rc;
     plan->wchunks.push_back(std::move(wc));
   }
   if (cut != plan->span || next_rec != recs.size()) {
@@ -929,6 +978,8 @@
   plan->span = recs.back().host + recs.back().bytes - plan->host_lo;
   std::vector<PackRecHost> table;
   std::vector<tk::WireSegDev> wire_segs;
+  if (plan->wire)
+    if (const int rc = snapshot_addends(plan.get(), recs)) return rc;
   if (const int rc = cut_chunks(mod, recs, plan.get(), table, wire_segs)) return rc;
   if (const int rc = alloc_pack_resources(mod, plan.get(), table, wire_segs)) return rc;
   if (const int rc = capture_chunk_graphs(mod, plan.get())) return rc;
diff --git a/tachikoma_amd/csrc/tk_trace.hip b/tachikoma_amd/csrc/tk_trace.hip
--- a/tachikoma_amd/csrc/tk_trace.hip
+++ b/tachikoma_amd/csrc/tk_trace.hip
@@ -132,6 +132,24 @@
 }
 
 __device__ __forceinline__ uint32_t wire_byte(const uint32_t* w, int j) { return (w[j >> 2] >> (8 * (j & 3))) & 0xFFu; }
+
+__device__ __forceinline__ void wire_sub_addend(uint32_t* x, const WireSegDev& sg, int e0) {
+  const uint32_t plane = (uint32_t)sg.plane, channels = (uint32_t)sg.channels;
+  const uint32_t t = (uint32_t)sg.r0 + (uint32_t)e0;
+  const uint32_t q = t / plane;
+  uint32_t r = t - q * plane;
+  uint32_t c = ((uint32_t)sg.c0 + q) % channels;
+  uint32_t a = (uint32_t)sg.addend[c];
+#pragma unroll
+  for (int j = 0; j < 16; ++j) {
+    x[j] -= a;
+    if (++r == plane) {
+      r = 0;
+      c = c + 1 == channels ? 0 : c + 1;
+      a = (uint32_t)sg.addend[c];
+    }
+  }
+}
 
 enum { kWireCursor = 0, kWireSize = 1, kWirePlace = 2 };
 
@@ -223,6 +241,7 @@
                 v[p][4 * q + 3] -= (uint32_t)a.w;
           }
         }
+        if (sg.addend) wire_sub_addend(v[p], sg, e0);
 #pragma unroll
         for (int j = 0; j < 16; ++j) mn = min(mn, (int32_t)v[p][j]), mx = max(mx, (int32_t)v[p][j]);
       } else {
@@ -232,10 +251,13 @@
           if (e0 + j < n) {
             x = (uint32_t)src32[e0 + j];
             if (prev32) x -= (uint32_t)prev32[e0 + j];
-            mn = min(mn, (int32_t)x), mx = max(mx, (int32_t)x);
           }
           v[p][j] = x;
         }
+        if (sg.addend && e0 < n) wire_sub_addend(v[p], sg, e0);
+#pragma unroll
+        for (int j = 0; j < 16; ++j)
+          if (e0 + j < n) mn = min(mn, (int32_t)v[p][j]), mx = max(mx, (int32_t)v[p][j]);
       }
 #pragma unroll
       for (int m = 8; m >= 1; m >>= 1) {
@@ -740,12 +762,16 @@
 }
 
 namespace {
-std::vector<tk::WireSegDev> source_segs(const tk::WirePlan& plan, const tk_wire_record* recs, const void* const* src) {
+std::vector<tk::WireSegDev> source_segs(const tk::WirePlan& plan, const tk_wire_record* recs, const void* const* src,
+                                        const tk_wire_addend* addends = nullptr) {
   std::vector<tk::WireSegDev> segs;
   segs.reserve(plan.segs.size());
   for (const tk::WireSegRef& r : plan.segs) {
-    const tk::WireSegAddr a = tk::wire_seg_addr(r, recs[r.rec].kind, src[r.rec], recs[r.rec].diff ? src[r.rec - 1] : nullptr);
-    segs.push_back({a.at, a.prev, r.n, recs[r.rec].kind});
+    const int kind = tk::wire_seg_kind(recs[r.rec].kind);
+    const tk::WireSegAddr a = tk::wire_seg_addr(r, kind, src[r.rec], recs[r.rec].diff ? src[r.rec - 1] : nullptr);
+    segs.push_back({a.at, a.prev, r.n, kind});
+    if (const tk_wire_addend* ad = tk::wire_addend_of(recs, addends, r.rec))
+      tk::wire_seg_bias(&segs.back(), ad->addend, ad->plane, ad->channels, r.e0);
   }
   return segs;
 }
@@ -787,13 +813,18 @@
 
 int tk_wire_encode_device(const tk_wire_record* recs, int n_recs, const void* const* src, void* wire,
                           int64_t wire_cap, void* stream) {
+  return tk_wire_encode_device_bias(recs, nullptr, n_recs, src, wire, wire_cap, stream);
+}
+
+int tk_wire_encode_device_bias(const tk_wire_record* recs, const tk_wire_addend* addends, int n_recs,
+                               const void* const* src, void* wire, int64_t wire_cap, void* stream) {
   tk::WirePlan plan;
-  if (const int rc = tk::wire_plan(recs, n_recs, -1, "tk_wire_encode_device", &plan)) return rc;
+  if (const int rc = tk::wire_plan(recs, n_recs, -1, "tk_wire_encode_device", &plan, addends)) return rc;
   if (!src || !wire || wire_cap < plan.bound) {
     tk::set_error("tk_wire_encode_device: the wire buffer is smaller than tk_wire_bound");
     return TK_ERR_INVALID_ARG;
   }
-  const std::vector<tk::WireSegDev> segs = source_segs(plan, recs, src);
+  const std::vector<tk::WireSegDev> segs = source_segs(plan, recs, src, addends);
   hipStream_t s = tk::as_stream(stream);
   void* dev = nullptr;
   TK_HIP(hipMalloc(&dev, segs.size() * sizeof(tk::WireSegDev) + 64));
diff --git a/tachikoma_amd/csrc/tk_wire.cc b/tachikoma_amd/csrc/tk_wire.cc
--- a/tachikoma_amd/csrc/tk_wire.cc
+++ b/tachikoma_amd/csrc/tk_wire.cc
@@ -15,7 +15,8 @@
 namespace tk {
 void set_error(const std::string& msg);
 
-int wire_plan(const tk_wire_record* recs, int n_recs, int64_t image_bytes, const char* who, WirePlan* p) {
+int wire_plan(const tk_wire_record* recs, int n_recs, int64_t image_bytes, const char* who, WirePlan* p,
+              const tk_wire_addend* addends, bool bias_ok) {
   if (!recs || n_recs < 1) {
     set_error(std::string(who) + ": no records");
     return TK_ERR_INVALID_ARG;
@@ -23,12 +24,27 @@
   int64_t n_seg = 0;
   for (int i = 0; i < n_recs; ++i) {
     const int kind = recs[i].kind;
+    if (kind == kWireI32Bias &&
+        (!recs[i].diff || recs[i].n_elems >= ((int64_t)1 << 31) ||
+         (addends && (!addends[i].addend || addends[i].plane < 1 || addends[i].channels < 1)))) {
+      set_error(std::string(who) + ": record " + std::to_string(i) +
+                " is bias-coded (kind 3) but is not a differenced record of fewer than 2^31 elements with an addend "
+                "and a plane and channels of at least 1");
+      return TK_ERR_INVALID_ARG;
+    }
+    if (kind == kWireI32Bias && !addends && !bias_ok) {
+      set_error(std::string(who) + ": record " + std::to_string(i) +
+                " is bias-coded (kind 3), which this entry point takes no addends for (packed trace files, format "
+                "version 2, and the device decoder do not code them)");
+      return TK_ERR_UNSUPPORTED;
+    }
     const int64_t esize = wire_elem_bytes(kind);
-    const bool inside = kind >= kWireI32 && kind <= kWireU8 && recs[i].offset >= 0 && recs[i].n_elems >= 1 &&
+    const bool inside = kind >= kWireI32 && kind <= kWireI32Bias && recs[i].offset >= 0 && recs[i].n_elems >= 1 &&
                         recs[i].n_elems <= ((int64_t)1 << 40) &&
                         (image_bytes < 0 ||
                          (recs[i].offset <= image_bytes && esize * recs[i].n_elems <= image_bytes - recs[i].offset));
-    if (!inside || (recs[i].diff && (i == 0 || recs[i - 1].n_elems != recs[i].n_elems || recs[i - 1].kind != kind))) {
+    if (!inside || (recs[i].diff && (i == 0 || recs[i - 1].n_elems != recs[i].n_elems ||
+                                     wire_seg_kind(recs[i - 1].kind) != wire_seg_kind(kind)))) {
       set_error(std::string(who) + ": record " + std::to_string(i) +
                 " is of no known kind, lies outside the image or follows (diff) a record of another size or kind");
       return TK_ERR_INVALID_ARG;
@@ -133,10 +149,10 @@
   std::atomic<int64_t> next_{0};
 };
 
-template <int W, bool D>
-void widen(char* dst, const char* prev, const uint8_t* p, int cnt, uint32_t base) {
+template <int W, bool D, bool A>
+void widen(char* dst, const char* prev, const uint8_t* p, int cnt, uint32_t base, const uint32_t* add) {
   for (int i = 0; i < cnt; ++i) {
-    uint32_t v = base;
+    uint32_t v = A ? add[i] : base;
     if (W >= 1) v += p[i];
     if (W >= 2) v += (uint32_t)p[cnt + i] << 8;
     if (W >= 3) v += (uint32_t)p[2 * cnt + i] << 16;
@@ -149,16 +165,28 @@
     std::memcpy(dst + 4 * (int64_t)i, &v, 4);
   }
 }
-template <bool D>
-void widen_w(int w, char* dst, const char* prev, const uint8_t* p, int cnt, uint32_t base) {
+template <bool D, bool A = false>
+void widen_w(int w, char* dst, const char* prev, const uint8_t* p, int cnt, uint32_t base, const uint32_t* add = nullptr) {
   switch (w) {
-    case 0: return widen<0, D>(dst, prev, p, cnt, base);
-    case 1: return widen<1, D>(dst, prev, p, cnt, base);
-    case 2: return widen<2, D>(dst, prev, p, cnt, base);
-    case 3: return widen<3, D>(dst, prev, p, cnt, base);
-    default: return widen<4, D>(dst, prev, p, cnt, base);
-  }
-}
+    case 0: return widen<0, D, A>(dst, prev, p, cnt, base, add);
+    case 1: return widen<1, D, A>(dst, prev, p, cnt, base, add);
+    case 2: return widen<2, D, A>(dst, prev, p, cnt, base, add);
+    case 3: return widen<3, D, A>(dst, prev, p, cnt, base, add);
+    default: return widen<4, D, A>(dst, prev, p, cnt, base, add);
+  }
+}
+
+struct BiasWalk {
+  const int32_t* addend;
+  int32_t plane, channels, c, r;
+  template <typename Seg>
+  explicit BiasWalk(const Seg& s) : addend(s.addend), plane(s.plane), channels(s.channels), c(s.c0), r(s.r0) {}
+  int run(int left) const { return std::min(left, plane - r); }
+  uint32_t value() const { return (uint32_t)addend[c]; }
+  void advance(int k) {
+    if ((r += k) == plane) r = 0, c = c + 1 == channels ? 0 : c + 1;
+  }
+};
 
 inline uint8_t clamp_u8(uint8_t x, uint8_t lo, uint8_t hi) {
   x = x < lo ? lo : x;
@@ -216,14 +244,40 @@
     }
     return wire_align(len, 64);
   }
+  BiasWalk walk(sg);
   for (int b = 0; b < nb; ++b) {
     const int cnt = std::min(kWireBlock, sg.n - b * kWireBlock);
     const int w = widths[b];
     int32_t base;
     std::memcpy(&base, p + 4 * b, 4);
     char* dst = sg.dst + 4 * (int64_t)b * kWireBlock;
-    if (sg.prev) widen_w<true>(w, dst, sg.prev + 4 * (int64_t)b * kWireBlock, q, cnt, (uint32_t)base);
-    else widen_w<false>(w, dst, nullptr, q, cnt, (uint32_t)base);
+    const char* prev = sg.prev ? sg.prev + 4 * (int64_t)b * kWireBlock : nullptr;
+    if (sg.addend && prev) {
+      if (walk.run(cnt) == cnt) {
+        widen_w<true>(w, dst, prev, q, cnt, (uint32_t)base + walk.value());
+        walk.advance(cnt);
+      } else if (w == 0) {
+        for (int i = 0; i < cnt;) {
+          const int k = walk.run(cnt - i);
+          widen<0, true, false>(dst + 4 * i, prev + 4 * i, q, k, (uint32_t)base + walk.value(), nullptr);
+          walk.advance(k);
+          i += k;
+        }
+      } else {
+        uint32_t add[kWireBlock];
+        for (int i = 0; i < cnt;) {
+          const int k = walk.run(cnt - i);
+          std::fill(add + i, add + i + k, (uint32_t)base + walk.value());
+          walk.advance(k);
+          i += k;
+        }
+        widen_w<true, true>(w, dst, prev, q, cnt, 0, add);
+      }
+    } else if (prev) {
+      widen_w<true>(w, dst, prev, q, cnt, (uint32_t)base);
+    } else {
+      widen_w<false>(w, dst, nullptr, q, cnt, (uint32_t)base);
+    }
     q += (int64_t)w * cnt;
   }
   return wire_align(len, 64);
@@ -265,7 +319,7 @@
 }
 
 namespace {
-int64_t encode_seg(const char* src, const char* prev, int n, char* out) {
+int64_t encode_seg(const char* src, const char* prev, int n, char* out, BiasWalk* walk) {
   const int nb = (n + kWireBlock - 1) / kWireBlock;
   const int64_t hdr = wire_header_bytes(nb);
   std::memset(out, 0, (size_t)hdr);
@@ -280,6 +334,13 @@
       if (prev) std::memcpy(&pv, prev + 4 * ((int64_t)b * kWireBlock + i), 4);
       v[i] = (int32_t)(a - pv);
     }
+    if (walk)
+      for (int i = 0; i < cnt;) {
+        const int k = walk->run(cnt - i);
+        for (int j = i; j < i + k; ++j) v[j] = (int32_t)((uint32_t)v[j] - walk->value());
+        walk->advance(k);
+        i += k;
+      }
     const int32_t mn = *std::min_element(v, v + cnt), mx = *std::max_element(v, v + cnt);
     const uint32_t range = (uint32_t)mx - (uint32_t)mn;
     const int w = range == 0 ? 0 : range <= 0xFFu ? 1 : range <= 0xFFFFu ? 2 : range <= 0xFFFFFFu ? 3 : 4;
@@ -323,14 +384,19 @@
 
 int64_t tk_wire_bound(const tk_wire_record* recs, int n_recs) {
   tk::WirePlan p;
-  const int rc = tk::wire_plan(recs, n_recs, -1, "tk_wire_bound", &p);
+  const int rc = tk::wire_plan(recs, n_recs, -1, "tk_wire_bound", &p, nullptr, true);
   return rc ? rc : p.bound;
 }
 
 int64_t tk_wire_encode_host(const tk_wire_record* recs, int n_recs, const void* image, int64_t image_bytes,
                             void* wire, int64_t wire_cap) {
+  return tk_wire_encode_host_bias(recs, nullptr, n_recs, image, image_bytes, wire, wire_cap);
+}
+
+int64_t tk_wire_encode_host_bias(const tk_wire_record* recs, const tk_wire_addend* addends, int n_recs, const void* image,
+                                 int64_t image_bytes, void* wire, int64_t wire_cap) {
   tk::WirePlan p;
-  if (const int rc = tk::wire_plan(recs, n_recs, image_bytes, "tk_wire_encode_host", &p)) return rc;
+  if (const int rc = tk::wire_plan(recs, n_recs, image_bytes, "tk_wire_encode_host", &p, addends)) return rc;
   if (!image || !wire || wire_cap < p.bound) {
     tk::set_error("tk_wire_encode_host: the wire buffer is smaller than tk_wire_bound");
     return TK_ERR_INVALID_ARG;
@@ -341,14 +407,19 @@
   int64_t cursor = 0;
   for (size_t i = 0; i < p.segs.size(); ++i) {
     const tk::WireSegRef& s = p.segs[i];
-    const int kind = recs[s.rec].kind;
+    const int kind = tk::wire_seg_kind(recs[s.rec].kind);
     const tk::WireSegAddr a =
         tk::wire_seg_addr(s, kind, (const char*)image + recs[s.rec].offset,
                           recs[s.rec].diff ? (const char*)image + recs[s.rec - 1].offset : nullptr);
     const uint32_t start = (uint32_t)(cursor / 64);
     std::memcpy((char*)wire + 4 * i, &start, 4);
-    const int64_t len = kind == tk::kWireI32 ? tk::encode_seg(a.at, a.prev, s.n, payload + cursor)
-                                             : tk::encode_seg8(a.at, a.prev, s.n, kind, payload + cursor);
+    tk::WireSegHost bias{};
+    if (const tk_wire_addend* ad = tk::wire_addend_of(recs, addends, s.rec))
+      tk::wire_seg_bias(&bias, ad->addend, ad->plane, ad->channels, s.e0);
+    tk::BiasWalk walk(bias);
+    const int64_t len = kind == tk::kWireI32
+                            ? tk::encode_seg(a.at, a.prev, s.n, payload + cursor, bias.addend ? &walk : nullptr)
+                            : tk::encode_seg8(a.at, a.prev, s.n, kind, payload + cursor);
     const int64_t padded = tk::wire_align(len, 64);
     std::memset(payload + cursor + len, 0, (size_t)(padded - len));
     cursor += padded;
@@ -358,8 +429,13 @@
 
 int tk_wire_decode(const tk_wire_record* recs, int n_recs, const void* wire, int64_t wire_bytes, void* image,
                    int64_t image_bytes, int threads) {
+  return tk_wire_decode_bias(recs, nullptr, n_recs, wire, wire_bytes, image, image_bytes, threads);
+}
+
+int tk_wire_decode_bias(const tk_wire_record* recs, const tk_wire_addend* addends, int n_recs, const void* wire,
+                        int64_t wire_bytes, void* image, int64_t image_bytes, int threads) {
   tk::WirePlan p;
-  if (const int rc = tk::wire_plan(recs, n_recs, image_bytes, "tk_wire_decode", &p)) return rc;
+  if (const int rc = tk::wire_plan(recs, n_recs, image_bytes, "tk_wire_decode", &p, addends)) return rc;
   if (!wire || !image || wire_bytes < 0) {
     tk::set_error("tk_wire_decode: null buffer");
     return TK_ERR_INVALID_ARG;
@@ -370,7 +446,9 @@
     const tk::WireSegAddr a =
         tk::wire_seg_addr(s, recs[s.rec].kind, (char*)image + recs[s.rec].offset,
                           recs[s.rec].diff ? (const char*)image + recs[s.rec - 1].offset : nullptr);
-    segs[i] = {a.at, a.prev, s.n, recs[s.rec].kind};
+    segs[i] = {a.at, a.prev, s.n, tk::wire_seg_kind(recs[s.rec].kind)};
+    if (const tk_wire_addend* ad = tk::wire_addend_of(recs, addends, s.rec))
+      tk::wire_seg_bias(&segs[i], ad->addend, ad->plane, ad->channels, s.e0);
   }
   tk::WireJob job{(const char*)wire, wire_bytes, segs.data(), (int64_t)segs.size(),
                   p.units.data(), (int64_t)p.units.size()};
diff --git a/tachikoma_amd/csrc/tk_wire.h b/tachikoma_amd/csrc/tk_wire.h
--- a/tachikoma_amd/csrc/tk_wire.h
+++ b/tachikoma_amd/csrc/tk_wire.h
@@ -16,10 +16,16 @@
 inline int64_t wire_align(int64_t x, int64_t a) { return (x + a - 1) / a * a; }
 inline int64_t wire_table_bytes(int64_t n_seg) { return wire_align(4 * n_seg, 64); }
 inline int64_t wire_header_bytes(int nb) { return wire_align(4 * (int64_t)nb, 16) + wire_align(nb, 16); }
-enum WireKind : int32_t { kWireI32 = 0, kWireI8 = 1, kWireU8 = 2 };
-inline int wire_elem_bytes(int kind) { return kind == kWireI32 ? 4 : 1; }
+enum WireKind : int32_t { kWireI32 = 0, kWireI8 = 1, kWireU8 = 2, kWireI32Bias = 3 };
+inline int wire_seg_kind(int kind) { return kind == kWireI32Bias ? (int)kWireI32 : kind; }
+inline int wire_elem_bytes(int kind) { return wire_seg_kind(kind) == kWireI32 ? 4 : 1; }
 inline int64_t wire_seg_bound(int n, int esize = 4) {
   return wire_align(wire_header_bytes((n + kWireBlock - 1) / kWireBlock) + esize * (int64_t)n, 64);
+}
+
+struct WireSegPos { int32_t c0, r0; };
+inline WireSegPos wire_seg_pos(int64_t e0, int32_t plane, int32_t channels) {
+  return {(int32_t)((e0 / plane) % channels), (int32_t)(e0 % plane)};
 }
 
 struct WireSegDev {
@@ -27,6 +33,9 @@
   const void* prev;
   int32_t n;
   int32_t kind;
+  const int32_t* addend = nullptr;
+  int32_t plane = 0, channels = 0;
+  int32_t c0 = 0, r0 = 0;
 };
 struct WireSegOut {
   void* dst;
@@ -52,6 +61,9 @@
   const char* prev;
   int32_t n;
   int32_t kind;
+  const int32_t* addend = nullptr;
+  int32_t plane = 0, channels = 0;
+  int32_t c0 = 0, r0 = 0;
 };
 struct WireUnit {
   int32_t first, stride, count;
@@ -62,17 +74,29 @@
   int64_t e0;
 };
 
+inline const tk_wire_addend* wire_addend_of(const tk_wire_record* recs, const tk_wire_addend* addends, int i) {
+  return addends && recs[i].kind == kWireI32Bias ? addends + i : nullptr;
+}
+
 struct WirePlan {
   std::vector<WireSegRef> segs;
   std::vector<WireUnit> units;
   int64_t bound = 0;
 };
-int wire_plan(const tk_wire_record* recs, int n_recs, int64_t image_bytes, const char* who, WirePlan* plan);
+int wire_plan(const tk_wire_record* recs, int n_recs, int64_t image_bytes, const char* who, WirePlan* plan,
+              const tk_wire_addend* addends = nullptr, bool bias_ok = false);
 
 struct WireSegAddr { char* at; const char* prev; };
 inline WireSegAddr wire_seg_addr(const WireSegRef& s, int kind, const void* base, const void* prev_base) {
   const int64_t b0 = wire_elem_bytes(kind) * s.e0;
   return {base ? (char*)base + b0 : nullptr, prev_base ? (const char*)prev_base + b0 : nullptr};
+}
+
+template <typename Seg>
+inline void wire_seg_bias(Seg* s, const int32_t* addend, int32_t plane, int32_t channels, int64_t e0) {
+  if (!addend) return;
+  const WireSegPos at = wire_seg_pos(e0, plane, channels);
+  s->addend = addend, s->plane = plane, s->channels = channels, s->c0 = at.c0, s->r0 = at.r0;
 }
 
 int64_t wire_seg_extent(int kind, int n, uint32_t start, const char* payload, int64_t payload_bytes);
```

New measurement: 1009 op-traces/s, median of 6. +13.7%, better.
